# bartelvdh/Navtex

Hardware: AMD Instinct MI355X
Metric: IQ Msamples/s through FIR->FSK->bitsync (higher is better)
Workload: dtype f64

## Files before the change

### navtex_amd/__init__.py

```python
from __future__ import annotations

import ctypes as C
import os
from typing import Callable, Iterable, List, Optional, Sequence, Tuple

import numpy as np

from . import _native as N
from ._native import (CHAIN_490, CHAIN_518, FRAME_BITS, FRAME_IN, FRAME_RAW, FRAME_Y3, RATE_IN, RATE_RAW,
                      SOFT_DECODE, SOFT_KEEP, NvxError, lib)

__all__ = ["Pipeline", "Group", "Capture", "Sitor", "sitor_encode", "make_stream", "synth_host", "synth_device", "device_count",
           "DeviceBuffer", "channelise", "channelise_time_stats", "Store", "wav_write", "wav_read", "NvxError", "lib",
           "CHAIN_518", "CHAIN_490", "SOFT_DECODE", "SOFT_KEEP", "FRAME_BITS", "FRAME_IN", "FRAME_RAW", "FRAME_Y3", "RATE_IN", "RATE_RAW"]


def device_count() -> int:
    return lib.nvx_device_count()


def sitor_encode(text: str, n_phasing: int = 40) -> str:
    t = text.encode("ascii")
    n = lib.nvx_sitor_encode(t, n_phasing, None, 0)
    buf = C.create_string_buffer(n + 1)
# ... 149 lines not shown
        N.check(lib.nvx_cascade_wait_stats(self._h, C.byref(a), C.byref(b), C.byref(c), int(reset)), "nvx_cascade_wait_stats")
        return a.value, b.value, c.value

    def integrity_stats(self, reset: bool = False) -> Tuple[int, int, int]:
        a, b, c = C.c_uint64(), C.c_uint64(), C.c_uint64()
        N.check(lib.nvx_cascade_integrity_stats(self._h, C.byref(a), C.byref(b), C.byref(c), int(reset)), "nvx_cascade_integrity_stats")
        return a.value, b.value, c.value

    def tie_stats(self) -> Tuple[int, int, float]:
        a, b, m = C.c_uint64(), C.c_uint64(), C.c_double()
        N.check(lib.nvx_demod_tie_stats(self._h, C.byref(a), C.byref(b), C.byref(m)), "nvx_demod_tie_stats")
        return a.value, b.value, m.value

    def enable_timing(self, on: bool = True) -> None:
        lib.nvx_enable_timing(self._h, int(on))

    def kernel_ms(self, which: int) -> float:
        return float(lib.nvx_last_kernel_ms(self._h, which))

    def kernel_time_stats(self, which: int, reset: bool = False):
        s, n = C.c_double(), C.c_uint64()
        N.check(lib.nvx_kernel_time_stats(self._h, which, C.byref(s), C.byref(n), int(reset)), "nvx_kernel_time_stats")
        return s.value, n.value

    def enable_signal_report(self, on: bool = True) -> None:
        N.check(lib.nvx_enable_signal_report(self._h, int(on)), "nvx_enable_signal_report")

    def signal_report(self, stream: int = 0, chain: int = 0, reset: bool = False) -> dict:
        r = N.SignalReport()
        N.check(lib.nvx_signal_report_read(self._h, stream, chain, C.byref(r), int(reset)), "nvx_signal_report_read")
        return {f: getattr(r, f) for f, _ in N.SignalReport._fields_}

    def enable_soft(self, mode: int = N.SOFT_DECODE, on_message: Optional[Callable[[int, int, str, str], None]] = None) -> None:
        if not hasattr(self, "soft_messages"):
            self.soft_messages: List[Tuple[int, int, str, str]] = []
        if mode:
            sink = on_message or (lambda s, f, b, t: self.soft_messages.append((s, f, b, t)))
            self._soft_cb = N.MESSAGE_FN(lambda u, s, b, m, f: sink(s, f, b.decode("latin1"), m.decode("latin1")))
            N.check(lib.nvx_set_soft_message_fn(self._h, self._soft_cb, None), "nvx_set_soft_message_fn")
        N.check(lib.nvx_enable_soft(self._h, int(mode)), "nvx_enable_soft")

    def soft_values(self, stream: int = 0, chain: int = 0) -> np.ndarray:
        parts, cap = [], 1 << 14
        while True:
            buf = np.empty(cap, dtype=np.float32)
            n = lib.nvx_poll_soft(self._h, stream, chain, N.as_ptr(buf), cap)
            parts.append(buf[:n])
            if n < cap:
                break
        return np.concatenate(parts)

    def soft_count(self, stream: int = 0, chain: int = 0) -> int:
        return int(lib.nvx_soft_count(self._h, stream, chain))

    def set_carrier(self, stream: int, chain: int, offset_hz: float) -> float:
        applied = C.c_double()
        N.check(lib.nvx_set_carrier(self._h, stream, chain, float(offset_hz), C.byref(applied)), "nvx_set_carrier")
        return applied.value

    def carrier(self, stream: int, chain: int) -> Tuple[float, bool]:
        off, ref = C.c_double(), C.c_int()
        N.check(lib.nvx_get_carrier(self._h, stream, chain, C.byref(off), C.byref(ref)), "nvx_get_carrier")
        return off.value, bool(ref.value)

    def afc_enable(self, stream: int, chain: int, cfg: Optional[N.AfcConfig] = None, **fields) -> None:
        _afc_enable(lib.nvx_afc_enable, self._h, stream, chain, cfg, fields, "nvx_afc_enable")

    def afc_disable(self, stream: int, chain: int, keep: bool = False) -> None:
        N.check(lib.nvx_afc_disable(self._h, stream, chain, int(keep)), "nvx_afc_disable")

    def afc_status(self, stream: int, chain: int) -> dict:
        return _afc_status(lib.nvx_afc_read, self._h, stream, chain, "nvx_afc_read")

    def afc_trace(self, stream: int, chain: int) -> List[int]:
        return _afc_trace(lib.nvx_afc_trace, self._h, stream, chain, "nvx_afc_trace")

    def set_forms(self, independent: int = -1, dynamic_preroll: int = -1, demod_tiles: int = -1) -> None:
        N.check(lib.nvx_debug_set_forms(self._h, independent, dynamic_preroll, demod_tiles), "nvx_debug_set_forms")

    def last_forms(self) -> Tuple[int, int, int]:
        a, b, c = C.c_int(), C.c_int(), C.c_int()
        N.check(lib.nvx_debug_last_forms(self._h, C.byref(a), C.byref(b), C.byref(c)), "nvx_debug_last_forms")
        return a.value, b.value, c.value

    def _apply_forms(self, forms: Optional[Sequence[int]]) -> None:
        if forms is None:
            if not hasattr(lib, "nvx_debug_set_forms"):
                return
            forms = tuple(int(os.environ.get(name, -1)) for name in ("NVX_INDEPENDENT", "NVX_DYNAMIC_PREROLL", "NVX_DEMOD_TILES"))
        if tuple(forms) != (-1, -1, -1):
            self.set_forms(*forms)


class Pipeline(HandleStats):

    def __init__(self, n_streams: int = 1, raw_rate: bool = False, chain_mask: int = CHAIN_518 | CHAIN_490,
                 chain_masks: Optional[Iterable[int]] = None, labels: Optional[Sequence[Sequence[int]]] = None,
                 max_frames: int = 1, char_layer: bool = True, push_mode: bool = False, device: int = 0,
                 wideband: bool = False, bit_history: int = 0, store: "Optional[Store]" = None, stage0_order: int = 1,
                 eager_launch: bool = False, stall_timeout_ms: int = 0, forms: Optional[Sequence[int]] = None):
        self.messages: List[Tuple[int, int, str, str]] = []
        cfg = N.Config()
        lib.nvx_config_default(C.byref(cfg))
        cfg.device, cfg.n_streams, cfg.raw_rate = device, n_streams, int(raw_rate)
        cfg.stage0_order = int(stage0_order)
        cfg.eager_launch = int(eager_launch)
        cfg.stall_timeout_ms = int(stall_timeout_ms)
        cfg.chain_mask, cfg.max_frames, cfg.char_layer, cfg.push_mode = chain_mask, max_frames, int(char_layer), int(push_mode)
        cfg.wideband = int(wideband)
        cfg.bit_history = int(bit_history)
        if chain_masks is not None:
            chain_masks = list(chain_masks)
            self._masks = (C.c_uint8 * len(chain_masks))(*chain_masks)
            cfg.chain_masks = self._masks
        if labels is not None:
            flat = [int(v) for pair in labels for v in pair]
            self._labels = (C.c_int * len(flat))(*flat)
            cfg.labels = self._labels
        self._cb = N.MESSAGE_FN(lambda u, s, b, m, f: self.messages.append((s, f, b.decode("latin1"), m.decode("latin1"))))
        cfg.on_message = self._cb
        if store is not None:
            cfg.on_message = C.cast(lib.nvx_store_on_message, N.MESSAGE_FN)
            cfg.user = store._s
            self._store = store
        self.n_streams, self.raw_rate, self.max_frames, self.device = n_streams, bool(raw_rate), max_frames, device
        self.wideband = bool(wideband)
        self.frame = FRAME_RAW if (raw_rate or wideband) else FRAME_IN
        h = C.c_void_p()
        N.check(lib.nvx_create(C.byref(cfg), C.byref(h)), "nvx_create")
        self._h = h
        self._bits = {}
        self._apply_forms(forms)

    def push(self, stream: int, iq: np.ndarray) -> None:
        iq = np.ascontiguousarray(iq, dtype=np.int16).reshape(-1, 2)
        N.check(lib.nvx_push_iq(self._h, stream, N.as_ptr(iq), iq.shape[0]), "nvx_push_iq")

    def push_planar(self, stream: int, xi: np.ndarray, xq: np.ndarray) -> None:
        xi = np.ascontiguousarray(xi, dtype=np.int16); xq = np.ascontiguousarray(xq, dtype=np.int16)
        N.check(lib.nvx_push_planar(self._h, stream, N.as_ptr(xi), N.as_ptr(xq), xi.size), "nvx_push_planar")

    def flush(self) -> None:
        N.check(lib.nvx_flush(self._h), "nvx_flush")

    def finish(self, stream: Optional[int] = None) -> None:
        if stream is None:
            N.check(lib.nvx_finish(self._h), "nvx_finish")
        else:
            N.check(lib.nvx_stream_finish(self._h, stream), "nvx_stream_finish")

    def poll(self) -> None:
        N.check(lib.nvx_poll(self._h), "nvx_poll")

    def set_active(self, stream: int, active: bool) -> None:
        N.check(lib.nvx_stream_set_active(self._h, stream, int(active)), "nvx_stream_set_active")

    def stream_stats(self, stream: int = 0) -> Tuple[bool, int, int]:
        a, f, p = C.c_int(), C.c_uint64(), C.c_uint64()
        N.check(lib.nvx_stream_stats(self._h, stream, C.byref(a), C.byref(f), C.byref(p)), "nvx_stream_stats")
        return bool(a.value), f.value, p.value

    def set_trace(self, on_text: Optional[Callable[[str], None]]) -> None:
        self._trace_cb = N.SITOR_TRACE_FN(lambda u, t: on_text(t.decode("latin1"))) if on_text else C.cast(None, N.SITOR_TRACE_FN)
        N.check(lib.nvx_set_trace(self._h, self._trace_cb, None), "nvx_set_trace")

    def decode_wav(self, path: str, stream: int = 0) -> int:
# ... 304 lines not shown
```

### navtex_amd/_native.py

```python
from __future__ import annotations

import ctypes as C
import os
from pathlib import Path

import numpy as np

_LIB_PATH = Path(os.environ.get("NAVTEX_AMD_LIB") or (Path(__file__).resolve().parent / "libnavtex_amd.so"))

OK, ERR_ARG, ERR_NODEV, ERR_HIP, ERR_NOMEM, ERR_STATE, ERR_IO = 0, -1, -2, -3, -4, -5, -6
RATE_RAW, RATE_IN = 2016000, 252000
FRAME_BITS, FRAME_IN, FRAME_RAW, FRAME_Y3 = 32, 80640, 645120, 288
CHAIN_518, CHAIN_490 = 1, 2
SOFT_DECODE, SOFT_KEEP = 1, 2
TUNE_N, TUNE_STEP_HZ, TUNE_MAX_HZ, TUNE_NOMINAL_K = 20160, 3.125, 25000.0, 4480

MESSAGE_FN = C.CFUNCTYPE(None, C.c_void_p, C.c_int, C.c_char_p, C.c_char_p, C.c_int)
SITOR_MSG_FN = C.CFUNCTYPE(None, C.c_void_p, C.c_char_p, C.c_char_p, C.c_int)
SITOR_TRACE_FN = C.CFUNCTYPE(None, C.c_void_p, C.c_char_p)


class Config(C.Structure):
    _fields_ = [
        ("struct_size", C.c_uint32), ("device", C.c_int), ("n_streams", C.c_int), ("raw_rate", C.c_int), ("chain_mask", C.c_uint32),
        ("chain_masks", C.POINTER(C.c_uint8)), ("labels", C.POINTER(C.c_int)), ("max_frames", C.c_int),
        ("char_layer", C.c_int), ("on_message", MESSAGE_FN), ("user", C.c_void_p), ("push_mode", C.c_int),
        ("wideband", C.c_int),
        ("bit_history", C.c_int),
        ("host_threads", C.c_int),
        ("stage0_order", C.c_int),
        ("eager_launch", C.c_int),
        ("stall_timeout_ms", C.c_int),
    ]


class Carrier(C.Structure):
    _fields_ = [
        ("freq_hz", C.c_int32), ("shift_hz", C.c_int32), ("amplitude", C.c_int32), ("phase0", C.c_uint32),
        ("bit_offset", C.c_uint32), ("n_bits", C.c_uint32), ("bits", C.c_char_p),
    ]


class SynthStream(C.Structure):
    _fields_ = [("seed", C.c_uint32), ("noise_amp", C.c_int32), ("n_carriers", C.c_int32), ("carrier", Carrier * 16)]


class SignalReport(C.Structure):
    _fields_ = [("samples", C.c_uint64), ("b_samples", C.c_uint64)] + [(f, C.c_double) for f in (
        "sum_power", "sum_dphi_b", "sum_dphi2_b", "sum_dphi_y", "sum_dphi2_y", "sum_mf_hi", "sum_mf_lo",
        "power_db", "b_hz", "y_hz", "offset_hz", "shift_hz", "eye_snr_db", "contrast")]


class AfcConfig(C.Structure):
    _fields_ = [("struct_size", C.c_uint32), ("gain_shift", C.c_int), ("max_step", C.c_int), ("range_k", C.c_int),
                ("min_samples", C.c_int), ("contrast_min", C.c_double)]


class AfcStatus(C.Structure):
    _fields_ = [("enabled", C.c_int), ("centre_k", C.c_int), ("k_last", C.c_int), ("last_step", C.c_int), ("offset_hz", C.c_double),
                ("launches", C.c_uint64), ("updates", C.c_uint64), ("held", C.c_uint64), ("clamped", C.c_uint64)]


AFC_TRACE_KEEP = 1024


def _load() -> C.CDLL:
    if not _LIB_PATH.exists():
        raise ImportError(
            f"{_LIB_PATH} is missing: build it with `python navtex_amd/build.py` "
            "(hipcc, gfx950). navtex_amd has no pure-Python or CPU fallback.")
    lib = C.CDLL(str(_LIB_PATH))
    vp, sz, i, u32 = C.c_void_p, C.c_size_t, C.c_int, C.c_uint32
    sig = {
        "nvx_last_error": (C.c_char_p, []), "nvx_version": (C.c_char_p, []), "nvx_abi_version": (i, []),
        "nvx_sample_to_int16": (i, [C.c_double, C.POINTER(C.c_int16)]), "nvx_shim_stats": (i, [C.POINTER(C.c_uint64), C.POINTER(C.c_uint64)]),
        "nvx_debug_advance_clock": (i, [vp, i, C.c_uint64]),
        "nvx_debug_set_forms": (i, [vp, i, i, i]), "nvx_debug_last_forms": (i, [vp, C.POINTER(i), C.POINTER(i), C.POINTER(i)]),
        "init_fir_filter1": (None, []), "sample_in_1": (None, [C.c_double, C.c_double]), "init_fir2_wrapper": (None, []),
        "nvx_set_trace": (i, [vp, SITOR_TRACE_FN, vp]),
        "nvx_shim_latency": (i, [C.POINTER(C.c_uint64), C.POINTER(C.c_double), C.POINTER(C.c_double), C.POINTER(C.c_double), C.POINTER(C.c_double), i]),
        "nvx_shim_flush": (i, []), "nvx_shim_finish": (i, []), "nvx_shim_bits": (sz, [i, C.c_char_p, sz]),
        "nvx_StreamACallback": (None, [vp, vp, vp, C.c_uint, C.c_uint, vp]),
        "nvx_capture_start": (i, [vp, i, C.c_double, C.POINTER(vp)]), "nvx_capture_callback": (None, [vp, vp, vp, C.c_uint, C.c_uint, vp]),
        "nvx_capture_latency": (i, [vp, C.POINTER(C.c_uint64), C.POINTER(C.c_double), C.POINTER(C.c_double), C.POINTER(C.c_double), C.POINTER(C.c_double), i]),
        "nvx_capture_stop": (i, [vp]), "nvx_capture_record": (i, [vp, C.c_char_p]), "nvx_fsm_selftest": (i, [u32, i]),
        "nvx_cascade_wait_stats": (i, [vp, C.POINTER(C.c_uint64), C.POINTER(C.c_uint64), C.POINTER(C.c_uint64), i]),
        "nvx_debug_cascade_state": (i, [vp, i, vp, sz, i]),
        "nvx_cascade_integrity_stats": (i, [vp, C.POINTER(C.c_uint64), C.POINTER(C.c_uint64), C.POINTER(C.c_uint64), i]), "nvx_capture_pause": (None, [vp, i]),
        "nvx_capture_stats": (None, [vp, C.POINTER(C.c_uint64), C.POINTER(C.c_uint64), C.POINTER(C.c_uint64)]),
        "nvx_config_default": (None, [C.POINTER(Config)]),
        "nvx_create": (i, [C.POINTER(Config), C.POINTER(vp)]), "nvx_destroy": (None, [vp]), "nvx_reset": (i, [vp]), "nvx_stream_reset": (i, [vp, i]),
        "nvx_push_iq": (i, [vp, i, vp, sz]), "nvx_push_planar": (i, [vp, i, vp, vp, sz]), "nvx_flush": (i, [vp]),
        "nvx_finish": (i, [vp]), "nvx_stream_finish": (i, [vp, i]),
        "nvx_poll_bits": (sz, [vp, i, i, C.c_char_p, sz]),
        "nvx_process_resident": (i, [vp, vp, sz, sz, i, vp]), "nvx_fetch_bits": (i, [vp]),
        "nvx_bit_count": (sz, [vp, i, i]),
        "nvx_last_kernel_ms": (C.c_float, [vp, i]), "nvx_enable_timing": (None, [vp, i]), "nvx_enable_debug": (i, [vp, i]),
        "nvx_group_create": (i, [C.POINTER(C.c_int), i, C.POINTER(Config), C.POINTER(vp)]), "nvx_group_destroy": (None, [vp]),
        "nvx_group_reset": (i, [vp]), "nvx_group_size": (i, [vp]),
        "nvx_group_member": (i, [vp, i, C.POINTER(i), C.POINTER(i), C.POINTER(i), C.POINTER(vp)]), "nvx_group_member_of": (i, [vp, i]),
        "nvx_group_process_resident": (i, [vp, C.POINTER(vp), sz, sz, i]), "nvx_group_fetch_bits": (i, [vp]),
        "nvx_group_push_iq": (i, [vp, i, vp, sz]), "nvx_group_flush": (i, [vp]), "nvx_group_finish": (i, [vp]),
        "nvx_group_poll_bits": (sz, [vp, i, i, C.c_char_p, sz]), "nvx_group_bit_count": (sz, [vp, i, i]),
        "nvx_bind_thread_to_device": (i, [i]),
        "nvx_demod_tie_stats": (i, [vp, C.POINTER(C.c_uint64), C.POINTER(C.c_uint64), C.POINTER(C.c_double)]),
        "nvx_capture_error": (i, [vp]),
        "nvx_capture_stalled": (i, [vp, C.POINTER(C.c_uint64)]), "nvx_capture_set_stall_timeout": (None, [vp, C.c_double]),
        "nvx_stream_set_active": (i, [vp, i, i]), "nvx_poll": (i, [vp]),
        "nvx_stream_stats": (i, [vp, i, C.POINTER(i), C.POINTER(C.c_uint64), C.POINTER(C.c_uint64)]),
        "nvx_kernel_time_stats": (i, [vp, i, C.POINTER(C.c_double), C.POINTER(C.c_uint64), i]),
        "nvx_debug_y3": (sz, [vp, i, i, vp, sz]), "nvx_debug_dphi": (sz, [vp, i, i, vp, sz]),
        "nvx_debug_timing": (sz, [vp, i, i, vp, vp, vp, sz]),
        "nvx_enable_signal_report": (i, [vp, i]), "nvx_signal_report_read": (i, [vp, i, i, C.POINTER(SignalReport), i]),
        "nvx_enable_soft": (i, [vp, i]), "nvx_set_soft_message_fn": (i, [vp, MESSAGE_FN, vp]),
        "nvx_poll_soft": (sz, [vp, i, i, vp, sz]), "nvx_soft_count": (C.c_uint64, [vp, i, i]),
        "nvx_sitor_set_soft": (None, [vp, i]), "nvx_sitor_receive_soft": (None, [vp, vp, sz]),
        "nvx_set_carrier": (i, [vp, i, i, C.c_double, C.POINTER(C.c_double)]),
        "nvx_get_carrier": (i, [vp, i, i, C.POINTER(C.c_double), C.POINTER(i)]),
        "nvx_group_set_carrier": (i, [vp, i, i, C.c_double, C.POINTER(C.c_double)]),
        "nvx_group_get_carrier": (i, [vp, i, i, C.POINTER(C.c_double), C.POINTER(i)]),
        "nvx_afc_config_default": (None, [C.POINTER(AfcConfig)]),
        "nvx_afc_enable": (i, [vp, i, i, C.POINTER(AfcConfig)]), "nvx_afc_disable": (i, [vp, i, i, i]),
        "nvx_afc_read": (i, [vp, i, i, C.POINTER(AfcStatus)]), "nvx_afc_trace": (i, [vp, i, i, C.POINTER(C.c_int32), sz]),
        "nvx_group_afc_enable": (i, [vp, i, i, C.POINTER(AfcConfig)]), "nvx_group_afc_disable": (i, [vp, i, i, i]),
        "nvx_group_afc_read": (i, [vp, i, i, C.POINTER(AfcStatus)]), "nvx_group_afc_trace": (i, [vp, i, i, C.POINTER(C.c_int32), sz]),
        "nvx_afc_step_host": (i, [i, i, i, i, C.c_double, i, i, i, C.c_uint, C.c_uint, C.c_double, C.c_double, C.c_double, C.c_double, C.POINTER(C.c_uint)]),
        "nvx_device_count": (i, []), "nvx_device_alloc": (vp, [i, sz]), "nvx_device_free": (None, [i, vp]),
        "nvx_memcpy_h2d": (i, [i, vp, vp, sz]), "nvx_memcpy_d2h": (i, [i, vp, vp, sz]), "nvx_device_sync": (i, [i]),
        "nvx_stream_create": (vp, [i]), "nvx_stream_destroy": (None, [i, vp]),
        "nvx_sitor_new": (vp, [i, SITOR_MSG_FN, vp]), "nvx_sitor_set_trace": (None, [vp, SITOR_TRACE_FN, vp]),
        "nvx_sitor_free": (None, [vp]), "nvx_sitor_reset": (None, [vp]),
        "nvx_sitor_receive_bit": (None, [vp, C.c_char]), "nvx_sitor_receive_bits": (None, [vp, C.c_char_p, sz]),
        "nvx_wav_open": (vp, [C.c_char_p, u32]), "nvx_wav_close": (i, [vp]),
        "nvx_wav_read": (sz, [vp, vp, sz]), "nvx_wav_write": (sz, [vp, vp, sz]),
        "nvx_wav_set_format": (None, [vp, C.c_uint16]), "nvx_wav_set_num_channels": (None, [vp, C.c_uint16]),
        "nvx_wav_set_sample_rate": (None, [vp, u32]), "nvx_wav_set_sample_size": (None, [vp, sz]),
        "nvx_wav_get_format": (C.c_uint16, [vp]), "nvx_wav_get_num_channels": (C.c_uint16, [vp]),
        "nvx_wav_get_sample_rate": (u32, [vp]), "nvx_wav_get_sample_size": (sz, [vp]), "nvx_wav_get_length": (sz, [vp]),
        "nvx_wav_err": (C.c_char_p, []), "nvx_decode_wav": (i, [vp, i, C.c_char_p]),
        "nvx_sitor_encode": (sz, [C.c_char_p, i, C.c_char_p, sz]),
        "nvx_synth_host": (i, [C.POINTER(SynthStream), u32, C.c_uint64, sz, vp]),
        "nvx_synth_device": (i, [i, C.POINTER(SynthStream), i, u32, sz, vp, sz]),
        "nvx_atan2_host": (C.c_double, [C.c_double, C.c_double]),
        "nvx_channelise_resident": (i, [i, vp, sz, sz, i, sz, vp, vp, vp, sz, sz, vp]),
        "nvx_handle_stream": (vp, [vp]), "nvx_channelise_timing": (None, [i]),
        "nvx_channelise_time_stats": (i, [C.POINTER(C.c_double), C.POINTER(C.c_uint64), i]),
        "nvx_store_open": (i, [C.c_char_p, i, C.POINTER(vp)]), "nvx_store_close": (None, [vp]),
        "nvx_store_add_message": (i, [vp, C.c_char_p, C.c_char_p, i]),
        "nvx_store_on_message": (None, [vp, i, C.c_char_p, C.c_char_p, i]),
        "nvx_store_purge": (i, [vp, C.c_long]), "nvx_store_set_time": (None, [vp, C.c_int64]),
        "nvx_store_stats": (None, [vp, C.POINTER(C.c_uint64), C.POINTER(C.c_uint64)]),
    }
    for name, (res, args) in sig.items():
        fn = getattr(lib, name, None)
        if fn is None:
            if os.environ.get("NAVTEX_AMD_LIB"):
                continue
            raise ImportError(f"{_LIB_PATH} does not export {name}: rebuild it (python navtex_amd/build.py)")
        fn.restype, fn.argtypes = res, args
    return lib
# ... 21 lines not shown
```

### navtex_amd/build.py

```python
from __future__ import annotations

import os
import shutil
import subprocess
import sys
from pathlib import Path

PKG = Path(__file__).resolve().parent
ROOT = PKG.parent
CSRC = PKG / "csrc"
OBJ = PKG / "_obj"
LIB = PKG / "libnavtex_amd.so"
ARCH = "gfx950"

C_SOURCES = ["nvx_sitor.c", "nvx_wav.c", "nvx_synth_host.c", "nvx_store.c"]
HIP_SOURCES = ["nvx_cascade.hip", "nvx_fir3.hip", "nvx_demod.hip", "nvx_channelise.hip", "nvx_wideband_fused.hip", "nvx_synth.hip"]
SCAN = PKG / "scan"
SCAN_LIB = PKG / "libnavtex_amd_scan.so"
SCAN_C_SOURCES = ["nvx_scan_find.c"]
SCAN_HIP_SOURCES = ["nvx_scan.hip"]
SCAN_CXX_SOURCES = ["nvx_scan_host.cpp"]
RESAMPLE = PKG / "resample"
RESAMPLE_LIB = PKG / "libnavtex_amd_resample.so"
RESAMPLE_C_SOURCES = ["nvx_resample_design.c"]
RESAMPLE_HIP_SOURCES = ["nvx_resample.hip"]
RESAMPLE_CXX_SOURCES = ["nvx_resample_host.cpp"]
DDC = PKG / "ddc"
DDC_LIB = PKG / "libnavtex_amd_ddc.so"
DDC_HIP_SOURCES = ["nvx_ddc.hip"]
DDC_CXX_SOURCES = ["nvx_ddc_host.cpp"]
DDC_SHARED_C_SOURCES = ["nvx_resample_design.c"]
BLANK = PKG / "blank"
BLANK_LIB = PKG / "libnavtex_amd_blank.so"
BLANK_HIP_SOURCES = ["nvx_blank.hip"]
BLANK_CXX_SOURCES = ["nvx_blank_host.cpp"]
IQC = PKG / "iqc"
IQC_LIB = PKG / "libnavtex_amd_iqc.so"
IQC_HIP_SOURCES = ["nvx_iqc.hip"]
IQC_CXX_SOURCES = ["nvx_iqc_host.cpp"]
REAL = PKG / "real"
REAL_LIB = PKG / "libnavtex_amd_real.so"
REAL_HIP_SOURCES = ["nvx_real.hip"]
REAL_CXX_SOURCES = ["nvx_real_host.cpp"]
NARROW = PKG / "narrow"
NARROW_LIB = PKG / "libnavtex_amd_narrow.so"
NARROW_C_SOURCES = ["nvx_narrow_design.c"]
NARROW_HIP_SOURCES = ["nvx_narrow.hip"]
NARROW_CXX_SOURCES = ["nvx_narrow_host.cpp"]
TAP = PKG / "tap"
TAP_LIB = PKG / "libnavtex_amd_tap.so"
TAP_C_SOURCES = ["nvx_tap_design.c"]
TAP_HIP_SOURCES = ["nvx_tap.hip"]
TAP_CXX_SOURCES = ["nvx_tap_host.cpp"]
ANC = PKG / "anc"
ANC_LIB = PKG / "libnavtex_amd_anc.so"
ANC_HIP_SOURCES = ["nvx_anc.hip"]
ANC_CXX_SOURCES = ["nvx_anc_host.cpp"]
CXX_SOURCES = ["nvx_api.cpp", "nvx_push.cpp", "nvx_shim.cpp", "nvx_capture.cpp", "nvx_wideband.cpp", "nvx_synth_dev.cpp", "nvx_fsm_host.cpp", "nvx_group.cpp",
               "nvx_tune.cpp", "nvx_afc.cpp"]
AFC = PKG / "afc"
AFC_HIP_SOURCES = ["nvx_afc.hip"]

COMMON = ["-O3", "-fPIC", "-ffp-contract=off", "-fvisibility=hidden",
          f"-I{ROOT / 'include'}", f"-I{CSRC}"] + os.environ.get("NVX_EXTRA_CFLAGS", "").split()


def _hipcc() -> str:
    for cand in (os.environ.get("HIPCC"), shutil.which("hipcc"), "/opt/rocm/bin/hipcc"):
        if cand and Path(cand).exists():
            return cand
    raise RuntimeError("hipcc not found: the HIP toolchain is required (there is no CPU build of this library)")


def _run(cmd):
    print(" ".join(str(c) for c in cmd), file=sys.stderr, flush=True)
    subprocess.run([str(c) for c in cmd], check=True, stdout=sys.stderr)


def _stale(out: Path, deps) -> bool:
    if not out.exists():
        return True
    t = out.stat().st_mtime
    return any(Path(d).stat().st_mtime > t for d in deps)


def _companion_jobs(hipcc: str, force: bool, src_dir: Path, c_sources, hip_sources, cxx_sources, also=()):
    headers = list(src_dir.glob("*.h")) + list(CSRC.glob("*.h")) + list((ROOT / "include").glob("*.h")) + [Path(__file__)]
    flags = [*COMMON, f"-I{src_dir}"]
    for d in also:
        headers += list(d.glob("*.h"))
        flags.append(f"-I{d}")
    objs, jobs = [], []
    for srcs, cmd in ((c_sources, [hipcc, "-x", "c", "-std=gnu11", "-Wall", "-Wextra"]),
                      (hip_sources, [hipcc, f"--offload-arch={ARCH}", "-std=c++17"]),
                      (cxx_sources, [hipcc, "-x", "hip", "--offload-arch=" + ARCH, "-std=c++17", "-Wall"])):
        for src in srcs:
            o = OBJ / (src + ".o")
            if force or _stale(o, [src_dir / src] + headers):
                jobs.append([*cmd, *flags, "-c", src_dir / src, "-o", o])
            objs.append(o)
    return objs, jobs


def _scan_jobs(hipcc: str, force: bool):
    return _companion_jobs(hipcc, force, SCAN, SCAN_C_SOURCES, SCAN_HIP_SOURCES, SCAN_CXX_SOURCES)


def _resample_jobs(hipcc: str, force: bool):
    return _companion_jobs(hipcc, force, RESAMPLE, RESAMPLE_C_SOURCES, RESAMPLE_HIP_SOURCES, RESAMPLE_CXX_SOURCES)


def _ddc_jobs(hipcc: str, force: bool):
    objs, jobs = _companion_jobs(hipcc, force, DDC, [], DDC_HIP_SOURCES, DDC_CXX_SOURCES, also=(RESAMPLE,))
    return objs + [OBJ / (src + ".o") for src in DDC_SHARED_C_SOURCES], jobs


def _blank_jobs(hipcc: str, force: bool):
    return _companion_jobs(hipcc, force, BLANK, [], BLANK_HIP_SOURCES, BLANK_CXX_SOURCES, also=(RESAMPLE,))


def _iqc_jobs(hipcc: str, force: bool):
    return _companion_jobs(hipcc, force, IQC, [], IQC_HIP_SOURCES, IQC_CXX_SOURCES, also=(RESAMPLE,))


def _real_jobs(hipcc: str, force: bool):
    return _companion_jobs(hipcc, force, REAL, [], REAL_HIP_SOURCES, REAL_CXX_SOURCES, also=(RESAMPLE,))


def _narrow_jobs(hipcc: str, force: bool):
    return _companion_jobs(hipcc, force, NARROW, NARROW_C_SOURCES, NARROW_HIP_SOURCES, NARROW_CXX_SOURCES, also=(RESAMPLE,))


def _tap_jobs(hipcc: str, force: bool):
    return _companion_jobs(hipcc, force, TAP, TAP_C_SOURCES, TAP_HIP_SOURCES, TAP_CXX_SOURCES, also=(RESAMPLE, DDC))


def _anc_jobs(hipcc: str, force: bool):
    return _companion_jobs(hipcc, force, ANC, [], ANC_HIP_SOURCES, ANC_CXX_SOURCES, also=(RESAMPLE,))


def _link(hipcc: str, lib: Path, objs, libs=()) -> None:
    tmp = lib.with_name(lib.name + f".tmp{os.getpid()}")
    _run([hipcc, "-shared", "-fPIC", f"--offload-arch={ARCH}", *objs, "-o", tmp, *libs])
    os.replace(tmp, lib)


def build_lib(force: bool = False) -> Path:
    from concurrent.futures import ThreadPoolExecutor
    hipcc = _hipcc()
    OBJ.mkdir(exist_ok=True)
    headers = list(CSRC.glob("*.h")) + list((ROOT / "include").glob("*.h")) + [Path(__file__)]
    objs, jobs = [], []
    scan_objs, scan_jobs = _scan_jobs(hipcc, force)
    jobs += scan_jobs
    resample_objs, resample_jobs = _resample_jobs(hipcc, force)
    jobs += resample_jobs
    ddc_objs, ddc_jobs = _ddc_jobs(hipcc, force)
    jobs += ddc_jobs
    blank_objs, blank_jobs = _blank_jobs(hipcc, force)
    jobs += blank_jobs
    iqc_objs, iqc_jobs = _iqc_jobs(hipcc, force)
    jobs += iqc_jobs
    real_objs, real_jobs = _real_jobs(hipcc, force)
    jobs += real_jobs
    narrow_objs, narrow_jobs = _narrow_jobs(hipcc, force)
    jobs += narrow_jobs
    tap_objs, tap_jobs = _tap_jobs(hipcc, force)
    jobs += tap_jobs
    anc_objs, anc_jobs = _anc_jobs(hipcc, force)
    jobs += anc_jobs
    for src in C_SOURCES:
        o = OBJ / (src + ".o")
        if force or _stale(o, [CSRC / src] + headers):
            jobs.append([hipcc, "-x", "c", "-std=gnu11", "-Wall", "-Wextra", *COMMON, "-c", CSRC / src, "-o", o])
        objs.append(o)
    for src in HIP_SOURCES:
        o = OBJ / (src + ".o")
        if force or _stale(o, [CSRC / src] + headers):
            jobs.append([hipcc, f"--offload-arch={ARCH}", "-std=c++17", *COMMON, "-c", CSRC / src, "-o", o])
        objs.append(o)
    for src in AFC_HIP_SOURCES:
        o = OBJ / (src + ".o")
        if force or _stale(o, [AFC / src] + headers):
            jobs.append([hipcc, f"--offload-arch={ARCH}", "-std=c++17", *COMMON, "-c", AFC / src, "-o", o])
        objs.append(o)
    for src in CXX_SOURCES:
        o = OBJ / (src + ".o")
        if force or _stale(o, [CSRC / src] + headers):
            jobs.append([hipcc, "-x", "hip", "--offload-arch=" + ARCH, "-std=c++17", "-Wall", "-Wno-unused-value", "-Wno-unused-result", *COMMON, "-c", CSRC / src, "-o", o])
        objs.append(o)
    with ThreadPoolExecutor(max_workers=min(8, os.cpu_count() or 1)) as pool:
        list(pool.map(_run, jobs))
    if force or _stale(LIB, objs):
        _link(hipcc, LIB, objs, ["-lpthread", "-ldl"])
    if force or _stale(SCAN_LIB, scan_objs):
        _link(hipcc, SCAN_LIB, scan_objs, ["-lpthread", "-lm"])
    if force or _stale(RESAMPLE_LIB, resample_objs):
        _link(hipcc, RESAMPLE_LIB, resample_objs, ["-lpthread", "-lm"])
    if force or _stale(DDC_LIB, ddc_objs):
        _link(hipcc, DDC_LIB, ddc_objs, ["-lpthread", "-lm"])
    if force or _stale(BLANK_LIB, blank_objs):
        _link(hipcc, BLANK_LIB, blank_objs, ["-lpthread"])
    if force or _stale(IQC_LIB, iqc_objs):
        _link(hipcc, IQC_LIB, iqc_objs, ["-lpthread"])
    if force or _stale(REAL_LIB, real_objs):
        _link(hipcc, REAL_LIB, real_objs, ["-lpthread"])
    if force or _stale(NARROW_LIB, narrow_objs):
        _link(hipcc, NARROW_LIB, narrow_objs, ["-lpthread", "-lm"])
    if force or _stale(TAP_LIB, tap_objs):
        _link(hipcc, TAP_LIB, tap_objs, ["-lpthread", "-lm"])
    if force or _stale(ANC_LIB, anc_objs):
        _link(hipcc, ANC_LIB, anc_objs, ["-lpthread"])
    return LIB


def build_variant(name: str, flags, sources=("nvx_cascade.hip", "nvx_wideband_fused.hip")) -> Path:
    hipcc = _hipcc()
    build_lib()
    out_dir = ROOT / "tests" / "_variants"
    out_dir.mkdir(exist_ok=True)
    headers = list(CSRC.glob("*.h")) + list((ROOT / "include").glob("*.h")) + [Path(__file__)]
    objs, jobs = [], []
    for src in C_SOURCES + HIP_SOURCES + CXX_SOURCES:
        if src in sources:
            o = out_dir / f"{src}.{name}.o"
            if _stale(o, [CSRC / src] + headers):
                lang = ["-x", "c", "-std=gnu11"] if src in C_SOURCES else (["-x", "hip"] if src in CXX_SOURCES else []) + [f"--offload-arch={ARCH}", "-std=c++17"]
                jobs.append([hipcc, *lang, *COMMON, *flags, "-c", CSRC / src, "-o", o])
            objs.append(o)
        else:
            objs.append(OBJ / (src + ".o"))
    objs += [OBJ / (src + ".o") for src in AFC_HIP_SOURCES]
    from concurrent.futures import ThreadPoolExecutor
    with ThreadPoolExecutor(max_workers=2) as pool:
        list(pool.map(_run, jobs))
    lib = out_dir / f"libnavtex_amd_{name}.so"
    if _stale(lib, objs):
        tmp = lib.with_name(lib.name + f".tmp{os.getpid()}")
        _run([hipcc, "-shared", "-fPIC", f"--offload-arch={ARCH}", *objs, "-o", tmp, "-lpthread", "-ldl"])
        os.replace(tmp, lib)
    return lib


INJECT_FLAGS = ["-DNVX_INJECT_STALE=5"]


def build_oracle() -> None:
    _run(["make", "-s", "-C", ROOT / "oracle", "oracle"])
    if os.path.isdir("/root/reference/receiver"):
        _run(["make", "-s", "-C", ROOT / "oracle", "ref"])


if __name__ == "__main__":
    build_lib(force="--force" in sys.argv)
    if "--oracle" in sys.argv:
        build_oracle()
    if "--inject" in sys.argv or (ROOT / "tests" / "_variants" / "libnavtex_amd_inject.so").exists():
        build_variant("inject", INJECT_FLAGS)
    if "--variant" in sys.argv:
        rest = sys.argv[sys.argv.index("--variant") + 1:]
        srcs = ("nvx_cascade.hip", "nvx_wideband_fused.hip")
        if "--sources" in rest:
            k = rest.index("--sources"); srcs = tuple(rest[k + 1].split(",")); rest = rest[:k] + rest[k + 2:]
        print(build_variant(rest[0], rest[1:], srcs))
```

### navtex_amd/csrc/nvx_api.cpp

```cpp
#include "nvx_handle.h"
#include <chrono>
#include <cmath>
#include "navtex_amd_afc.h"
#include "navtex_amd_signal.h"
#include "navtex_amd_soft.h"
#include "navtex_amd_tune.h"
#include "nvx_fsm.h"

extern "C" hipError_t nvx_launch_afc_update(const nvx_afc_args *a, hipStream_t s) __attribute__((weak));
static_assert(NVX_AFC_LAW_C == NVX_AFC_C && NVX_AFC_K_MAX * NVX_TUNE_STEP_HZ == NVX_TUNE_MAX_HZ, "the law's constants are the header's");
static_assert(sizeof(nvx_afc_note) == 8 && sizeof(nvx_afc_par) == 32, "layouts of nvx_afc_law.h");

static thread_local char g_err[512] = "";
extern "C" void nvx_set_error(const char *fmt, ...)
{
    va_list ap; va_start(ap, fmt);
    vsnprintf(g_err, sizeof g_err, fmt, ap);
    va_end(ap);
}
extern "C" const char *nvx_last_error(void) { return g_err; }
int64_t nvx_now_ns()
{
    return std::chrono::duration_cast<std::chrono::nanoseconds>(std::chrono::steady_clock::now().time_since_epoch()).count();
}
#define NVX_STR2(x) #x
#define NVX_STR(x) NVX_STR2(x)
extern "C" const char *nvx_version(void) { return "navtex_amd " NVX_STR(NVX_ABI_VERSION) ".0 (gfx950)"; }
extern "C" int nvx_abi_version(void) { return NVX_ABI_VERSION; }

int nvx_select_device(int device)
{
    int n = 0;
    hipError_t e = hipGetDeviceCount(&n);
    if (e != hipSuccess || n == 0) {
        nvx_set_error("no HIP device available (%s); libnavtex_amd has no CPU path",
                      e == hipSuccess ? "device count 0" : hipGetErrorString(e));
        return NVX_ERR_NODEV;
    }
    if (device < 0 || device >= n) { nvx_set_error("device %d out of range (0..%d)", device, n - 1); return NVX_ERR_ARG; }
    HIP_TRY(hipSetDevice(device));
    return NVX_OK;
}


int nvx_check_device_span(const void *p, size_t bytes, const char *what)
{
    hipDeviceptr_t base = nullptr; size_t size = 0;
    if (hipMemGetAddressRange(&base, &size, (hipDeviceptr_t)p) != hipSuccess) { (void)hipGetLastError(); return NVX_OK; }
    const size_t off = (size_t)((const char *)p - (const char *)base);
    if (off > size || bytes > size - off) {
        nvx_set_error("%s: %zu bytes from %p leave the allocation they lie in (%zu bytes from %p): the launch would fault", what, bytes, p, size, (void *)base);
        return NVX_ERR_ARG;
    }
    return NVX_OK;
}

static void sitor_sink(void *user, const char *bbbb, const char *message, int freq);

static void deliver_outbox(nvx_handle *h, int stream, Slot &s);

static void sitor_sink_impl(nvx_handle *h, int slot, const char *bbbb, const char *message, int freq);

static void sitor_sink(void *user, const char *bbbb, const char *message, int freq)
{
    SinkCtx *c = (SinkCtx *)user;
    if (c->soft) c->h->slots[c->slot].soft_outbox.push_back(Message{ bbbb, message, freq });
    else sitor_sink_impl(c->h, c->slot, bbbb, message, freq);
}

extern "C" void nvx_config_default(nvx_config *c)
{
    memset(c, 0, sizeof *c);
    c->struct_size = (uint32_t)sizeof *c;
    c->device = 0; c->n_streams = 1; c->raw_rate = 0;
    c->chain_mask = NVX_CHAIN_518 | NVX_CHAIN_490;
    c->max_frames = 1; c->char_layer = 1; c->push_mode = 0;
}

static int drain(nvx_handle *h)
{
    if (h->launch_done_valid) HIP_TRY(hipEventSynchronize(h->launch_done));
    if (h->stream) HIP_TRY(hipStreamSynchronize(h->stream));
    if (h->stream2) HIP_TRY(hipStreamSynchronize(h->stream2));
    return NVX_OK;
}

// ... 326 lines not shown
    return NVX_OK;
}

int nvx_launch_locked(nvx_handle *h, const void *d_iq, size_t pitch, size_t first_sample, int n_frames, hipStream_t st,
                      const int *part, int n_part, const int *tail_n3)
{
    if (h->poisoned) return nvx_poisoned_error(h);
    if (n_frames < 1 || n_frames > h->cfg.max_frames) { nvx_set_error("n_frames %d outside 1..max_frames %d", n_frames, h->cfg.max_frames); return NVX_ERR_ARG; }
    if ((pitch & 3) || (first_sample & 3)) { nvx_set_error("pitch and first sample must be multiples of 4 samples"); return NVX_ERR_ARG; }
    if (part && (n_part < 1 || n_part > h->n_in)) { nvx_set_error("launch with %d of %d streams", n_part, h->n_in); return NVX_ERR_ARG; }
    if (part && n_part == h->n_in && !tail_n3) part = nullptr;
    for (int i = 0; part && i < n_part; i++)
        if (part[i] < 0 || part[i] >= h->n_in || (i > 0 && part[i] <= part[i - 1])) { nvx_set_error("launch list: stream %d out of order or range", part[i]); return NVX_ERR_ARG; }
    const int n_named = part ? n_part : h->n_in;
    for (int i = 0; i < n_named; i++) {
        const int s = part ? part[i] : i;
        if (h->ended[s]) { nvx_set_error("stream %d has ended (nvx_finish): nvx_stream_reset or nvx_reset starts a new one", s); return NVX_ERR_STATE; }
        if (tail_n3 && (tail_n3[i] < 1 || tail_n3[i] >= n_frames * NVX_FRAME_Y3)) { nvx_set_error("launch list: %d samples at 900 S/s in the tail of stream %d", tail_n3[i], s); return NVX_ERR_ARG; }
    }
    Result &r = h->res[h->launched % RESULT_SLOTS];
    if (r.pending) { int rc = nvx_collect_locked(h, h->launched - RESULT_SLOTS + 1); if (rc != NVX_OK) return rc; }
    { int rc = nvx_collect_ready_locked(h); if (rc != NVX_OK) return rc; }

    if (h->launch_done_valid && st != h->last_launch_stream) HIP_TRY(hipStreamWaitEvent(st, h->launch_done, 0));

    const bool fused = h->cfg.wideband != 0;
    const int yb = (int)(h->launched & 1);
    hipStream_t sd = h->stream2;
    const int n3_full = n_frames * NVX_FRAME_Y3;
    const bool with_list = h->diverged || part != nullptr || tail_n3 != nullptr;
    r.n_part = 0;
    const nvx_part *d_list = nullptr;
    if (with_list) {
        r.n_part = n_named;
        for (int i = 0; i < r.n_part; i++) {
            const int s = part ? part[i] : i;
            r.h_part[i] = nvx_part{ s, (int)h->parity[s], h->g0s[s], tail_n3 ? tail_n3[i] : n3_full, 0 };
        }
        HIP_TRY(hipMemcpyAsync(r.d_part, r.h_part, (size_t)r.n_part * sizeof(nvx_part), hipMemcpyHostToDevice, st));
        d_list = r.d_part;
    }
    const int n_here = with_list ? r.n_part : h->n_in;
    const int p0 = d_list ? 0 : (int)h->parity[0];
    const unsigned third0 = (unsigned)(h->g0s[0] / (NVX_FRAME_Y3 / 3));
    double2 *const y2_bufs[2] = { h->d_y2[d_list ? 0 : p0], h->d_y2[d_list ? 1 : p0 ^ 1] };
    nvx_demod_args da{};
    da.y3 = h->d_y3[yb]; da.y3_cap = (size_t)h->y3_cap; da.y3_base = 0; da.n3 = n3_full;
    da.n_slots = h->n_slots; da.slot_active = h->d_active;
    da.g0 = h->g0s[0]; da.part = d_list; da.n_part = r.n_part; da.per_part = h->per_in;
    da.dstate[0] = h->d_dd[p0]; da.dstate[1] = h->d_dd[p0 ^ 1];
    da.state_i = h->d_di; da.fsm_table = h->d_fsm_tab; da.words = h->d_words;
    da.bits = r.d_bits; da.bits_cap = h->bits_cap; da.nbits = r.d_nbits; da.dphi = h->d_dphi; da.ties = h->d_ties;
    da.corr = h->d_corr; da.csum = h->d_csum;
    const bool afc = h->afc_tracking > 0;
    da.sig = (h->sig_on || afc) ? r.d_sig : nullptr; da.sig_part = h->d_sig_part; da.sig_stride = h->sig_stride;
    da.soft = h->soft_mode ? r.d_soft : nullptr; da.soft_cap = std::min(h->soft_cap, n3_full / 8 + 8); da.soft_pos = h->d_soft_pos;
    nvx_forms forms = h->forms_req;
    forms.demod_tiles = nvx_front_tile_wgs(&da, forms.demod_tiles);
    da.sig_parts = 1 + forms.demod_tiles;

    if (h->demod_pending[yb]) HIP_TRY(hipStreamWaitEvent(st, h->demod_done[yb], 0));
    r.timed = h->timing;
    if (r.timed) HIP_TRY(hipEventRecord(r.ev[0], st));
    if (fused) {
        nvx_wideband_args wa{};
        wa.raw = (const uint32_t *)d_iq; wa.pitch = pitch; wa.first_sample = first_sample;
        wa.n_wide = n_here; wa.n_frames = n_frames; wa.chain_masks = h->d_masks;
        wa.part = d_list;
        wa.state[0] = h->d_cstate[p0]; wa.state[1] = h->d_cstate[p0 ^ 1];
        wa.hist[0] = h->d_whist[p0]; wa.hist[1] = h->d_whist[p0 ^ 1];
        wa.y3 = h->d_y3[yb]; wa.y3_cap = (size_t)h->y3_cap; wa.y3_base = 0;
        wa.queue = h->d_ctrl; wa.status = h->d_ctrl + 1; wa.done = h->d_ctrl + NVX_CASCADE_CTRL_INTS; wa.third0 = third0;
        wa.y2[0] = y2_bufs[0]; wa.y2[1] = y2_bufs[1]; wa.y2_pitch = h->y2_pitch; wa.y2_row = h->d_y2row;
        HIP_TRY(nvx_launch_wideband_fused(&wa, &forms, st));
    } else {
        nvx_cascade_args ca{};
        ca.iq = (const uint32_t *)d_iq; ca.pitch = pitch; ca.first_sample = first_sample;
        ca.n_frames = n_frames; ca.n_streams = n_here; ca.chain_masks = h->d_masks;
        ca.part = d_list;
        ca.state[0] = h->d_cstate[p0]; ca.state[1] = h->d_cstate[p0 ^ 1]; ca.y3 = h->d_y3[yb]; ca.y3_cap = (size_t)h->y3_cap; ca.y3_base = 0;
        ca.queue = h->d_ctrl; ca.status = h->d_ctrl + 1; ca.done = h->d_ctrl + NVX_CASCADE_CTRL_INTS;
        ca.stage0_order = h->cfg.stage0_order;
        ca.third0 = third0;
        ca.tune_k = afc ? h->d_afc_k[h->launched & 1] : h->d_tune_k;
        ca.max_waves_per_cu = -1;
        HIP_TRY(nvx_launch_cascade(&ca, h->cascade_raw, h->nch, &forms, st));
    }
    if (r.timed) HIP_TRY(hipEventRecord(r.ev[1], st));
    HIP_TRY(hipMemcpyAsync(h->h_status + NVX_STATUS_INTS * (h->launched % RESULT_SLOTS), h->d_ctrl + 1, NVX_STATUS_INTS * sizeof(int), hipMemcpyDeviceToHost, st));
    HIP_TRY(hipEventRecord(h->casc_done[yb], st));
    HIP_TRY(hipStreamWaitEvent(sd, h->casc_done[yb], 0));
    if (fused) {
        nvx_fir3_args fa{};
        fa.y2[0] = y2_bufs[0]; fa.y2[1] = y2_bufs[1]; fa.y2_pitch = h->y2_pitch; fa.y2_row = h->d_y2row;
        fa.y3 = h->d_y3[yb]; fa.y3_cap = (size_t)h->y3_cap; fa.y3_base = 0; fa.n_frames = n_frames; fa.n_slots = h->n_slots;
        fa.part = d_list; fa.n_part = r.n_part; fa.per_part = h->per_in;
        if (r.timed) HIP_TRY(hipEventRecord(r.ev[6], sd));
        HIP_TRY(nvx_launch_fir3(&fa, sd));
        if (r.timed) HIP_TRY(hipEventRecord(r.ev[7], sd));
    }
    if (r.timed) HIP_TRY(hipEventRecord(r.ev[2], sd));
    HIP_TRY(nvx_launch_demod_front(&da, sd));
    if (r.timed) HIP_TRY(hipEventRecord(r.ev[3], sd));
    if (!da.soft && !afc) HIP_TRY(hipEventRecord(h->demod_done[yb], sd));
    h->demod_pending[yb] = true;
    if (r.timed) HIP_TRY(hipEventRecord(r.ev[4], sd));
    HIP_TRY(nvx_launch_demod_fsm(&da, sd));
    if (r.timed) HIP_TRY(hipEventRecord(r.ev[5], sd));
    if (afc) {
        nvx_afc_args aa{};
        aa.sig = r.d_sig; aa.par = h->d_afc_par; aa.k_rw = h->d_afc_k[h->launched & 1]; aa.k_next = h->d_afc_k[(h->launched + 1) & 1];
        aa.note = r.d_note; aa.n_slots = h->n_slots; aa.part = d_list; aa.n_part = r.n_part;
        if (r.timed) HIP_TRY(hipEventRecord(r.ev[8], sd));
        HIP_TRY(nvx_launch_afc_update(&aa, sd));
        if (r.timed) HIP_TRY(hipEventRecord(r.ev[9], sd));
    }
    if (da.soft || afc) HIP_TRY(hipEventRecord(h->demod_done[yb], sd));
    HIP_TRY(hipMemcpyAsync(h->h_ties, h->d_ties, sizeof(nvx_tie_stats), hipMemcpyDeviceToHost, sd));
    HIP_TRY(hipMemcpyAsync(r.h_nbits, r.d_nbits, (size_t)h->n_slots * sizeof(int), hipMemcpyDeviceToHost, sd));
    HIP_TRY(hipMemcpyAsync(r.h_bits, r.d_bits, (size_t)h->n_slots * h->bits_cap, hipMemcpyDeviceToHost, sd));
    if (h->sig_on) HIP_TRY(hipMemcpyAsync(r.h_sig, r.d_sig, (size_t)h->n_slots * sizeof(nvx_sig_rec), hipMemcpyDeviceToHost, sd));
    r.sig = h->sig_on;
    if (afc) HIP_TRY(hipMemcpyAsync(r.h_note, r.d_note, (size_t)h->n_slots * sizeof(nvx_afc_note), hipMemcpyDeviceToHost, sd));
    r.afc = afc;
    if (da.soft) HIP_TRY(hipMemcpyAsync(r.h_soft, r.d_soft, (size_t)h->n_slots * da.soft_cap * sizeof(float), hipMemcpyDeviceToHost, sd));
    r.soft_pitch = da.soft_cap;
    r.soft = da.soft != nullptr;
    HIP_TRY(hipEventRecord(r.done, sd));
    HIP_TRY(hipEventRecord(h->launch_done, sd));
    h->launch_done_valid = true; h->last_launch_stream = st;
    r.pending = true;
    r.n3 = n3_full;
    r.g0_all = h->g0s[0];
    h->launched++;
    h->last_n3 = n3_full;
    h->forms_last = forms; h->forms_known = true;
    for (int i = 0; i < n_here; i++) {
        const int s = with_list ? r.h_part[i].stream : i;
        h->parity[s] ^= 1; h->g0s[s] += (unsigned long long)(tail_n3 ? tail_n3[i] : n3_full);
        if (tail_n3) h->ended[s] = 1;
    }
    if (part) h->partial_launches++;
    h->diverged = with_list && !streams_together(h);
    return NVX_OK;
}

int nvx_collect_ready_locked(nvx_handle *h)
{
    while (h->collected < h->launched) {
        Result &o = h->res[h->collected % RESULT_SLOTS];
        if (o.pending) {
            const hipError_t q = hipEventQuery(o.done);
            if (q == hipErrorNotReady) { (void)hipGetLastError(); break; }
            if (q != hipSuccess) { nvx_set_error("hipEventQuery: %s", hipGetErrorString(q)); return NVX_ERR_HIP; }
        }
        int rc = nvx_collect_locked(h, h->collected + 1);
        if (rc != NVX_OK) return rc;
    }
    return NVX_OK;
}

int nvx_poisoned_error(nvx_handle *h)
{
    nvx_set_error("a launch of this handle failed (%s): nvx_reset it", h->poison_why.c_str());
    return NVX_ERR_STATE;
}

// ... 287 lines not shown
extern "C" int nvx_enable_signal_report(nvx_handle *h, int on)
{
    if (!h) { nvx_set_error("nvx_enable_signal_report: null handle"); return NVX_ERR_ARG; }
    std::lock_guard<std::mutex> lk(h->mu);
    HIP_TRY(hipSetDevice(h->cfg.device));
    { int rc = drain(h); if (rc != NVX_OK) return rc; }
    if (!on) { free_signal(h); return NVX_OK; }
    if (h->sig_on) return NVX_OK;
    { int rc = make_signal_buffers(h, "nvx_enable_signal_report"); if (rc != NVX_OK) return rc; }
    h->sig_on = true;
    return NVX_OK;
}

extern "C" int nvx_enable_soft(nvx_handle *h, int mode)
{
    if (!h) { nvx_set_error("nvx_enable_soft: null handle"); return NVX_ERR_ARG; }
    if (mode != 0 && mode != NVX_SOFT_DECODE && mode != (NVX_SOFT_DECODE | NVX_SOFT_KEEP)) { nvx_set_error("nvx_enable_soft: mode %d (0, NVX_SOFT_DECODE, NVX_SOFT_DECODE | NVX_SOFT_KEEP)", mode); return NVX_ERR_ARG; }
    std::lock_guard<std::mutex> lk(h->mu);
    if (h->poisoned) return nvx_poisoned_error(h);
    HIP_TRY(hipSetDevice(h->cfg.device));
    { int rc = drain(h); if (rc != NVX_OK) return rc; }
    if (!mode) { free_soft(h); return NVX_OK; }
    if (!h->soft_mode) {
        const int cap = h->bits_cap * 8;
        const size_t row_bytes = (size_t)h->n_slots * cap * sizeof(float);
        hipError_t e = hipMalloc(&h->d_soft_pos, (size_t)(h->y3_cap / 9) * h->n_slots * sizeof(unsigned short));
        for (auto &r : h->res) {
            if (e == hipSuccess) e = hipMalloc(&r.d_soft, row_bytes);
            if (e == hipSuccess) e = hipHostMalloc((void **)&r.h_soft, row_bytes, hipHostMallocDefault);
        }
        if (e != hipSuccess) {
            free_soft(h);
            nvx_set_error("nvx_enable_soft: allocation failed: %s", hipGetErrorString(e));
            return e == hipErrorOutOfMemory ? NVX_ERR_NOMEM : NVX_ERR_HIP;
        }
        h->soft_cap = cap;
        if (h->cfg.char_layer)
            for (int i = 0; i < h->n_slots; i++) {
                Slot &s = h->slots[i];
                if (!s.active) continue;
                SinkCtx *ctx = new SinkCtx{ h, i / 2, i, true };
                h->sinks.push_back(ctx);
                s.soft_sitor = nvx_sitor_new(s.label, sitor_sink, ctx);
                nvx_sitor_set_soft(s.soft_sitor, 1);
            }
    }
    if (!(mode & NVX_SOFT_KEEP))
        for (auto &s : h->slots) { s.soft_base += s.soft.size(); std::vector<float>().swap(s.soft); }
    else if (!(h->soft_mode & NVX_SOFT_KEEP))
        for (auto &s : h->slots) { s.soft_base = (size_t)s.soft_count; s.soft_polled = s.soft_base; }
    h->soft_mode = mode;
    return NVX_OK;
}

extern "C" int nvx_set_soft_message_fn(nvx_handle *h, nvx_message_fn fn, void *user)
{
    if (!h) { nvx_set_error("nvx_set_soft_message_fn: null handle"); return NVX_ERR_ARG; }
    std::lock_guard<std::mutex> lk(h->mu);
    if (h->poisoned) return nvx_poisoned_error(h);
    h->soft_fn = fn; h->soft_user = user;
    return NVX_OK;
}

extern "C" size_t nvx_poll_soft(nvx_handle *h, int stream, int chain, float *out, size_t cap)
{
    if (!h || !out || stream < 0 || stream >= h->n_streams || chain < 0 || chain > 1) return 0;
    std::lock_guard<std::mutex> lk(h->mu);
    if (!(h->soft_mode & NVX_SOFT_KEEP)) return 0;
    Slot &s = h->slots[2 * stream + chain];
    if (s.soft_polled < s.soft_base) s.soft_polled = s.soft_base;
    const size_t n = std::min(cap, s.soft_base + s.soft.size() - s.soft_polled);
    if (n) memcpy(out, s.soft.data() + (s.soft_polled - s.soft_base), n * sizeof(float));
    s.soft_polled += n;
    return n;
}

extern "C" uint64_t nvx_soft_count(nvx_handle *h, int stream, int chain)
{
    if (!h || stream < 0 || stream >= h->n_streams || chain < 0 || chain > 1) return 0;
    std::lock_guard<std::mutex> lk(h->mu);
    return h->slots[2 * stream + chain].soft_count;
}

static int afc_write_centre(nvx_handle *h, int slot, int k)
{
    for (int i = 0; i < 2; i++) HIP_TRY(hipMemcpy(h->d_afc_k[i] + slot, &k, sizeof(int), hipMemcpyHostToDevice));
    h->slots[slot].afc.par.kc = k;
    HIP_TRY(hipMemcpy(h->d_afc_par + slot, &h->slots[slot].afc.par, sizeof(nvx_afc_par), hipMemcpyHostToDevice));
    return NVX_OK;
}

extern "C" int nvx_set_carrier(nvx_handle *h, int stream, int chain, double offset_hz, double *applied_hz)
{
    if (!h) { nvx_set_error("nvx_set_carrier: null handle"); return NVX_ERR_ARG; }
    if (h->cfg.wideband) { nvx_set_error("nvx_set_carrier: not for wideband handles (the channeliser fixes their sub-bands)"); return NVX_ERR_STATE; }
    if (stream < 0 || stream >= h->n_streams || chain < 0 || chain > 1) { nvx_set_error("nvx_set_carrier: bad stream or chain"); return NVX_ERR_ARG; }
    if (!((h->masks[stream] >> chain) & 1)) { nvx_set_error("nvx_set_carrier: chain %d is not in stream %d's mask", chain, stream); return NVX_ERR_ARG; }
    if (!std::isfinite(offset_hz) || std::fabs(offset_hz) > NVX_TUNE_MAX_HZ) { nvx_set_error("nvx_set_carrier: offset %g Hz outside +-%g Hz", offset_hz, NVX_TUNE_MAX_HZ); return NVX_ERR_ARG; }
    const int k = (int)std::rint(offset_hz / NVX_TUNE_STEP_HZ);
    std::lock_guard<std::mutex> lk(h->mu);
    HIP_TRY(hipSetDevice(h->cfg.device));
    const int slot = 2 * stream + chain;
    if (h->slots[slot].afc.on) { int rc = nvx_collect_locked(h); if (rc != NVX_OK) return rc; }
    { int rc = drain(h); if (rc != NVX_OK) return rc; }
    HIP_TRY(hipMemcpyAsync(h->d_tune_k + slot, &k, sizeof(int), hipMemcpyHostToDevice, h->stream));
    if (h->afc_tracking) { int rc = afc_write_centre(h, slot, k); if (rc != NVX_OK) return rc; }
    HIP_TRY(hipStreamSynchronize(h->stream));
    h->tune_k[slot] = k;
    afc_restart(h, slot);
    if (applied_hz) *applied_hz = k * NVX_TUNE_STEP_HZ;
    return NVX_OK;
}

extern "C" int nvx_get_carrier(nvx_handle *h, int stream, int chain, double *offset_hz, int *reference_mixer)
{
    if (!h) { nvx_set_error("nvx_get_carrier: null handle"); return NVX_ERR_ARG; }
    if (h->cfg.wideband) { nvx_set_error("nvx_get_carrier: not for wideband handles"); return NVX_ERR_STATE; }
    if (stream < 0 || stream >= h->n_streams || chain < 0 || chain > 1) { nvx_set_error("nvx_get_carrier: bad stream or chain"); return NVX_ERR_ARG; }
    std::lock_guard<std::mutex> lk(h->mu);
    const int k = h->tune_k[2 * stream + chain];
    if (offset_hz) *offset_hz = k * NVX_TUNE_STEP_HZ;
    if (reference_mixer) *reference_mixer = k == (chain ? -NVX_TUNE_NOMINAL_K : NVX_TUNE_NOMINAL_K);
    return NVX_OK;
}

extern "C" void nvx_afc_config_default(nvx_afc_config *c)
{
    if (!c) return;
    memset(c, 0, sizeof *c);
    c->struct_size = (uint32_t)sizeof *c;
    c->gain_shift = 1; c->max_step = 8; c->range_k = 48; c->min_samples = 256; c->contrast_min = 0.7;
}

static int afc_args(nvx_handle *h, int stream, int chain, const char *what, int *slot)
{
    if (!h) { nvx_set_error("%s: null handle", what); return NVX_ERR_ARG; }
    if (h->cfg.wideband) { nvx_set_error("%s: not for wideband handles (the channeliser fixes their sub-bands)", what); return NVX_ERR_STATE; }
    if (stream < 0 || stream >= h->n_streams || chain < 0 || chain > 1) { nvx_set_error("%s: bad stream or chain", what); return NVX_ERR_ARG; }
    if (!((h->masks[stream] >> chain) & 1)) { nvx_set_error("%s: chain %d is not in stream %d's mask", what, chain, stream); return NVX_ERR_ARG; }
    *slot = 2 * stream + chain;
    return NVX_OK;
}

static int make_afc(nvx_handle *h)
{
    if (h->d_afc_par) return NVX_OK;
    const size_t n = (size_t)h->n_slots;
    hipError_t e = hipMalloc(&h->d_afc_par, n * sizeof(nvx_afc_par));
    if (e != hipSuccess) h->d_afc_par = nullptr;
    for (int i = 0; i < 2; i++) if (e == hipSuccess) e = hipMalloc(&h->d_afc_k[i], n * sizeof(int));
    for (auto &r : h->res) {
        if (e == hipSuccess) e = hipMalloc(&r.d_note, n * sizeof(nvx_afc_note));
        if (e == hipSuccess) e = hipHostMalloc((void **)&r.h_note, n * sizeof(nvx_afc_note), hipHostMallocDefault);
    }
    if (e == hipSuccess) {
        std::vector<nvx_afc_par> par(n);
        for (size_t i = 0; i < n; i++) { par[i] = h->slots[i].afc.par; par[i].track = 0; par[i].kc = h->tune_k[i]; }
        e = hipMemcpy(h->d_afc_par, par.data(), n * sizeof(nvx_afc_par), hipMemcpyHostToDevice);
    }
    if (e != hipSuccess) {
        free_afc(h);
        nvx_set_error("nvx_afc_enable: allocation failed: %s", hipGetErrorString(e));
        return e == hipErrorOutOfMemory ? NVX_ERR_NOMEM : NVX_ERR_HIP;
    }
    return NVX_OK;
}

extern "C" int nvx_afc_enable(nvx_handle *h, int stream, int chain, const nvx_afc_config *cfg)
{
    int slot = 0;
    { int rc = afc_args(h, stream, chain, "nvx_afc_enable", &slot); if (rc != NVX_OK) return rc; }
    nvx_afc_config c;
    nvx_afc_config_default(&c);
    if (cfg) {
        if (cfg->struct_size != sizeof(nvx_afc_config)) { nvx_set_error("nvx_afc_enable: nvx_afc_config.struct_size is %u, this library's has %zu bytes", cfg->struct_size, sizeof(nvx_afc_config)); return NVX_ERR_ARG; }
        c = *cfg;
    }
    if (c.gain_shift < 0 || c.gain_shift > 4 || c.max_step < 1 || c.max_step > 64 || c.range_k < 1 || c.range_k > 320 || c.min_samples < 0 ||
        !(c.contrast_min >= 0.0 && c.contrast_min <= 1.0)) {
        nvx_set_error("nvx_afc_enable: a field out of range (gain_shift 0..4, max_step 1..64, range_k 1..320, min_samples >= 0, contrast_min 0..1)");
        return NVX_ERR_ARG;
    }
    if (!nvx_launch_afc_update) { nvx_set_error("nvx_afc_enable: this build holds no update kernel"); return NVX_ERR_STATE; }
    std::lock_guard<std::mutex> lk(h->mu);
    if (h->poisoned) return nvx_poisoned_error(h);
    HIP_TRY(hipSetDevice(h->cfg.device));
    { int rc = nvx_collect_locked(h); if (rc != NVX_OK) return rc; }
    { int rc = drain(h); if (rc != NVX_OK) return rc; }
    { int rc = make_signal_buffers(h, "nvx_afc_enable"); if (rc != NVX_OK) return rc; }
    { int rc = make_afc(h); if (rc != NVX_OK) { if (!h->sig_on && !h->afc_tracking) free_signal_buffers(h); return rc; } }
    AfcHost &a = h->slots[slot].afc;
    if (!h->afc_tracking)
        for (int i = 0; i < 2; i++) HIP_TRY(hipMemcpy(h->d_afc_k[i], h->tune_k.data(), (size_t)h->n_slots * sizeof(int), hipMemcpyHostToDevice));
    a.par.track = 1;
    a.par.gain_shift = c.gain_shift; a.par.max_step = c.max_step; a.par.range_k = c.range_k; a.par.min_samples = c.min_samples;
    a.par.contrast_min = c.contrast_min;
    { int rc = afc_write_centre(h, slot, h->tune_k[slot]); if (rc != NVX_OK) { a.par.track = a.on ? 1 : 0; return rc; } }
    if (a.ring.empty()) a.ring.assign(NVX_AFC_TRACE_KEEP, 0);
    if (!a.on) { a.on = true; h->afc_tracking++; }
    afc_restart(h, slot);
    return NVX_OK;
}

extern "C" int nvx_afc_disable(nvx_handle *h, int stream, int chain, int keep)
{
    int slot = 0;
    { int rc = afc_args(h, stream, chain, "nvx_afc_disable", &slot); if (rc != NVX_OK) return rc; }
    std::lock_guard<std::mutex> lk(h->mu);
    if (h->poisoned) return nvx_poisoned_error(h);
    AfcHost &a = h->slots[slot].afc;
    if (!a.on) return NVX_OK;
    HIP_TRY(hipSetDevice(h->cfg.device));
    { int rc = nvx_collect_locked(h); if (rc != NVX_OK) return rc; }
    { int rc = drain(h); if (rc != NVX_OK) return rc; }
    int k = h->tune_k[slot];
    if (keep) {
        HIP_TRY(hipMemcpy(&k, h->d_afc_k[h->launched & 1] + slot, sizeof(int), hipMemcpyDeviceToHost));
        HIP_TRY(hipMemcpy(h->d_tune_k + slot, &k, sizeof(int), hipMemcpyHostToDevice));
        h->tune_k[slot] = k;
    }
    a.par.track = 0;
    { int rc = afc_write_centre(h, slot, k); if (rc != NVX_OK) return rc; }
    a.on = false; h->afc_tracking--;
    afc_restart(h, slot);
    if (!h->afc_tracking && !h->sig_on) free_signal_buffers(h);
    return NVX_OK;
}

static int afc_take_in(nvx_handle *h)
{
    if (h->poisoned) return nvx_poisoned_error(h);
    if (h->collected != h->launched) {
        HIP_TRY(hipSetDevice(h->cfg.device));
        return nvx_collect_ready_locked(h);
    }
    return NVX_OK;
}

extern "C" int nvx_afc_read(nvx_handle *h, int stream, int chain, nvx_afc_status *out)
{
    int slot = 0;
    { int rc = afc_args(h, stream, chain, "nvx_afc_read", &slot); if (rc != NVX_OK) return rc; }
    if (!out) { nvx_set_error("nvx_afc_read: null argument"); return NVX_ERR_ARG; }
    std::lock_guard<std::mutex> lk(h->mu);
    { int rc = afc_take_in(h); if (rc != NVX_OK) return rc; }
    const AfcHost &a = h->slots[slot].afc;
    memset(out, 0, sizeof *out);
    out->enabled = a.on; out->centre_k = h->tune_k[slot];
    out->k_last = a.on ? a.k_last : h->tune_k[slot]; out->last_step = a.on ? a.last_step : 0;
    out->offset_hz = out->k_last * NVX_TUNE_STEP_HZ;
    out->launches = a.launches; out->updates = a.updates; out->held = a.held; out->clamped = a.clamped;
    return NVX_OK;
}

extern "C" int nvx_afc_trace(nvx_handle *h, int stream, int chain, int32_t *k, size_t cap)
{
    int slot = 0;
    { int rc = afc_args(h, stream, chain, "nvx_afc_trace", &slot); if (rc != NVX_OK) return rc; }
    if (!k && cap) { nvx_set_error("nvx_afc_trace: null argument"); return NVX_ERR_ARG; }
    std::lock_guard<std::mutex> lk(h->mu);
    { int rc = afc_take_in(h); if (rc != NVX_OK) return rc; }
    AfcHost &a = h->slots[slot].afc;
    if (!a.on) return 0;
    if (a.ring_w - a.ring_r > NVX_AFC_TRACE_KEEP) a.ring_r = a.ring_w - NVX_AFC_TRACE_KEEP;
    int n = 0;
    while (a.ring_r < a.ring_w && (size_t)n < cap) k[n++] = a.ring[a.ring_r++ % NVX_AFC_TRACE_KEEP];
    return n;
}

static void signal_derive(nvx_signal_report *o)
{
    const double nan = std::nan(""), hz = 900.0 / (2.0 * M_PI);
    const uint64_t ny = o->samples - o->b_samples;
    o->power_db = o->samples ? 10.0 * std::log10(o->sum_power / (double)o->samples) : nan;
    const double mb = o->b_samples ? o->sum_dphi_b / (double)o->b_samples : nan;
    const double my = ny ? o->sum_dphi_y / (double)ny : nan;
    o->b_hz = mb * hz; o->y_hz = my * hz;
    o->offset_hz = (o->b_hz + o->y_hz) / 2.0;
    o->shift_hz = o->b_hz - o->y_hz;
    const double vb = std::max(0.0, o->sum_dphi2_b / (double)o->b_samples - mb * mb);
    const double vy = std::max(0.0, o->sum_dphi2_y / (double)ny - my * my);
    const double half = (mb - my) / 2.0, noise = (vb + vy) / 2.0;
    o->eye_snr_db = (o->b_samples && ny && noise > 0.0) ? 10.0 * std::log10(half * half / noise) : nan;
    const double mf = o->sum_mf_hi + o->sum_mf_lo;
    o->contrast = mf != 0.0 ? (o->sum_mf_hi - o->sum_mf_lo) / mf : nan;
}

extern "C" int nvx_signal_report_read(nvx_handle *h, int stream, int chain, nvx_signal_report *out, int reset)
{
    if (!h || !out) { nvx_set_error("nvx_signal_report_read: null argument"); return NVX_ERR_ARG; }
    if (stream < 0 || stream >= h->n_streams || chain < 0 || chain > 1) { nvx_set_error("nvx_signal_report_read: bad stream or chain"); return NVX_ERR_ARG; }
    std::lock_guard<std::mutex> lk(h->mu);
    if (h->poisoned) return nvx_poisoned_error(h);
    if (!h->sig_on) { nvx_set_error("nvx_signal_report_read: signal reports are off (nvx_enable_signal_report)"); return NVX_ERR_STATE; }
    if (h->collected != h->launched) {
        HIP_TRY(hipSetDevice(h->cfg.device));
        int rc = nvx_collect_ready_locked(h);
        if (rc != NVX_OK) return rc;
    }
    SigSums &g = h->slots[2 * stream + chain].sig;
    memset(out, 0, sizeof *out);
    out->samples = g.samples; out->b_samples = g.b_samples;
    out->sum_power = g.power; out->sum_dphi_b = g.dphi_b; out->sum_dphi2_b = g.dphi2_b;
    out->sum_dphi_y = g.dphi_y; out->sum_dphi2_y = g.dphi2_y; out->sum_mf_hi = g.hi; out->sum_mf_lo = g.lo;
    signal_derive(out);
    if (reset) g = SigSums{};
    return NVX_OK;
}

static_assert(NVX_STATE_BLOCK_BYTES == NVX_CASCADE_STATE_BYTES, "public size of a state block");
extern "C" int nvx_debug_cascade_state(nvx_handle *h, int stream, void *buf, size_t bytes, int write)
{
    if (!h || !buf || stream < 0 || stream >= h->n_streams || bytes != (size_t)NVX_CASCADE_STATE_BYTES) { nvx_set_error("nvx_debug_cascade_state: bad argument (a block is %d bytes)", NVX_CASCADE_STATE_BYTES); return NVX_ERR_ARG; }
    std::lock_guard<std::mutex> lk(h->mu);
    HIP_TRY(hipSetDevice(h->cfg.device));
    { int rc = drain(h); if (rc != NVX_OK) return rc; }
    const int in = stream / h->per_in;
    uint8_t *blk = h->d_cstate[h->parity[in]] + (size_t)stream * NVX_CASCADE_STATE_BYTES;
    if (write) HIP_TRY(hipMemcpy(blk, buf, bytes, hipMemcpyHostToDevice));
    else HIP_TRY(hipMemcpy(buf, blk, bytes, hipMemcpyDeviceToHost));
    return NVX_OK;
}

static unsigned long long seal_tag_host(int stream, unsigned third)
{
    unsigned long long t = ((unsigned long long)(unsigned)stream << 32) | third;
    t *= 0x9E3779B97F4A7C15ull; t ^= t >> 29; t *= 0xBF58476D1CE4E5B9ull; t ^= t >> 32;
    return t;
}

static_assert(NVX_CLOCK_PERIOD % NVX_FRAME_Y3 == 0 && NVX_CLOCK_PERIOD % (9 * 567) == 0, "the clock's period");
extern "C" int nvx_debug_advance_clock(nvx_handle *h, int stream, uint64_t periods)
{
    if (!h || stream < 0 || stream >= h->n_in) { nvx_set_error("nvx_debug_advance_clock: bad stream"); return NVX_ERR_ARG; }
    if (h->cfg.wideband) { nvx_set_error("nvx_debug_advance_clock: not for wideband handles"); return NVX_ERR_STATE; }
    std::unique_lock<std::mutex> lk(h->mu);
    if (h->poisoned) return nvx_poisoned_error(h);
    if (h->ended[stream]) { nvx_set_error("nvx_debug_advance_clock: stream %d has ended", stream); return NVX_ERR_STATE; }
    HIP_TRY(hipSetDevice(h->cfg.device));
    { int rc = nvx_collect_locked(h); if (rc != NVX_OK) return rc; }
    { int rc = drain(h); if (rc != NVX_OK) return rc; }
    const unsigned long long g_old = h->g0s[stream];
    if (g_old < 3 * NVX_FRAME_Y3) { nvx_set_error("nvx_debug_advance_clock: stream %d is still priming (%llu samples at 900 S/s; the timing filter is primed at 582)", stream, g_old); return NVX_ERR_STATE; }
    if (periods > (~0ull - g_old) / (unsigned long long)NVX_CLOCK_PERIOD) { nvx_set_error("nvx_debug_advance_clock: the clock would pass 2^64"); return NVX_ERR_ARG; }
    const unsigned long long g_new = g_old + periods * (unsigned long long)NVX_CLOCK_PERIOD;
    const unsigned third_old = (unsigned)(g_old / (NVX_FRAME_Y3 / 3)), third_new = (unsigned)(g_new / (NVX_FRAME_Y3 / 3));
    unsigned long long seal[2];
    uint8_t *entry = h->d_cstate[h->parity[stream]] + (size_t)stream * NVX_CASCADE_STATE_BYTES + (size_t)NVX_STATE_SEAL * 16;
    HIP_TRY(hipMemcpy(seal, entry, sizeof seal, hipMemcpyDeviceToHost));
    seal[0] ^= seal_tag_host(stream, third_old) ^ seal_tag_host(stream, third_new);
    seal[1] = ((unsigned long long)(unsigned)stream << 32) | third_new;
    HIP_TRY(hipMemcpy(entry, seal, sizeof seal, hipMemcpyHostToDevice));
    h->g0s[stream] = g_new;
    h->diverged = !streams_together(h);
    return NVX_OK;
}

extern "C" int nvx_debug_set_forms(nvx_handle *h, int independent, int dynamic_preroll, int demod_tiles)
{
    const auto bad = [](int v) { return v < -1 || v > 1; };
    if (!h || bad(independent) || bad(dynamic_preroll) || bad(demod_tiles)) { nvx_set_error("nvx_debug_set_forms: null handle, or a value outside -1 (automatic), 0, 1"); return NVX_ERR_ARG; }
    std::lock_guard<std::mutex> lk(h->mu);
    h->forms_req = nvx_forms{ independent, dynamic_preroll, demod_tiles };
    return NVX_OK;
}

extern "C" int nvx_debug_last_forms(nvx_handle *h, int *independent, int *dynamic_preroll, int *front_tile_wgs)
{
    if (!h) { nvx_set_error("nvx_debug_last_forms: null handle"); return NVX_ERR_ARG; }
    std::lock_guard<std::mutex> lk(h->mu);
    if (!h->forms_known) { nvx_set_error("nvx_debug_last_forms: the handle has launched nothing yet"); return NVX_ERR_STATE; }
    if (independent) *independent = h->forms_last.independent;
    if (dynamic_preroll) *dynamic_preroll = h->forms_last.dynamic_preroll;
    if (front_tile_wgs) *front_tile_wgs = h->forms_last.demod_tiles;
    return NVX_OK;
}

extern "C" size_t nvx_debug_y3(nvx_handle *h, int stream, int chain, double *out, size_t cap_pairs)
{
    if (!h || !out || stream < 0 || stream >= h->n_streams || chain < 0 || chain > 1) return 0;
    std::lock_guard<std::mutex> lk(h->mu);
    hipSetDevice(h->cfg.device);
    hipDeviceSynchronize();
    size_t n = std::min(cap_pairs, (size_t)h->last_n3);
    const int in = stream / h->per_in;
    if (h->ended[in]) n = std::min(n, (size_t)(h->g0s[in] % NVX_FRAME_Y3));
    if (hipMemcpy(out, h->d_y3[(h->launched + 1) & 1] + (size_t)(2 * stream + chain) * h->y3_cap, n * sizeof(double2), hipMemcpyDeviceToHost) != hipSuccess) return 0;
    return n;
}

extern "C" size_t nvx_debug_dphi(nvx_handle *h, int stream, int chain, double *out, size_t cap)
{
    if (!h || !out || !h->d_dphi || stream < 0 || stream >= h->n_streams || chain < 0 || chain > 1) return 0;
    std::lock_guard<std::mutex> lk(h->mu);
    hipSetDevice(h->cfg.device);
    hipDeviceSynchronize();
    size_t n = std::min(cap, (size_t)h->last_n3);
    if (hipMemcpy(out, h->d_dphi + (size_t)(2 * stream + chain) * h->y3_cap, n * sizeof(double), hipMemcpyDeviceToHost) != hipSuccess) return 0;
    return n;
}

extern "C" size_t nvx_debug_timing(nvx_handle *h, int stream, int chain, double *corr, double *csum, uint16_t *words, size_t cap)
{
    if (!h || stream < 0 || stream >= h->n_streams || chain < 0 || chain > 1) return 0;
    std::lock_guard<std::mutex> lk(h->mu);
    if ((corr || csum) && !h->d_corr) return 0;
    hipSetDevice(h->cfg.device);
    hipDeviceSynchronize();
    size_t n = std::min(cap, (size_t)h->last_n3);
    const int in = stream / h->per_in;
    if (h->ended[in]) n = std::min(n, (size_t)(h->g0s[in] % NVX_FRAME_Y3));
    const size_t slot = (size_t)(2 * stream + chain);
    if (corr && hipMemcpy(corr, h->d_corr + slot * h->y3_cap, n * sizeof(double), hipMemcpyDeviceToHost) != hipSuccess) return 0;
    if (csum && hipMemcpy(csum, h->d_csum + slot * h->y3_cap, n * sizeof(double), hipMemcpyDeviceToHost) != hipSuccess) return 0;
    if (words && hipMemcpy(words, h->d_words + slot * (h->y3_cap / 9), (n + 8) / 9 * sizeof(uint16_t), hipMemcpyDeviceToHost) != hipSuccess) return 0;
    return n;
}

extern "C" int nvx_device_count(void) { int n = 0; return hipGetDeviceCount(&n) == hipSuccess ? n : 0; }
extern "C" void *nvx_device_alloc(int device, size_t bytes)
{
    if (nvx_select_device(device) != NVX_OK) return nullptr;
    void *p = nullptr;
    hipError_t e = hipMalloc(&p, bytes);
    if (e != hipSuccess) { nvx_set_error("hipMalloc(%zu) failed: %s", bytes, hipGetErrorString(e)); return nullptr; }
    return p;
}
extern "C" void nvx_device_free(int device, void *p) { if (p && nvx_select_device(device) == NVX_OK) hipFree(p); }
extern "C" int nvx_memcpy_h2d(int device, void *d, const void *s, size_t n)
{
    int rc = nvx_select_device(device); if (rc != NVX_OK) return rc;
    HIP_TRY(hipMemcpy(d, s, n, hipMemcpyHostToDevice)); return NVX_OK;
}
extern "C" int nvx_memcpy_d2h(int device, void *d, const void *s, size_t n)
{
    int rc = nvx_select_device(device); if (rc != NVX_OK) return rc;
    HIP_TRY(hipMemcpy(d, s, n, hipMemcpyDeviceToHost)); return NVX_OK;
}
extern "C" int nvx_device_sync(int device)
{
    int rc = nvx_select_device(device); if (rc != NVX_OK) return rc;
    HIP_TRY(hipDeviceSynchronize()); return NVX_OK;
}
extern "C" void *nvx_stream_create(int device)
{
    if (nvx_select_device(device) != NVX_OK) return nullptr;
    hipStream_t s = nullptr;
    hipError_t e = hipStreamCreateWithFlags(&s, hipStreamNonBlocking);
    if (e != hipSuccess) { nvx_set_error("hipStreamCreate failed: %s", hipGetErrorString(e)); return nullptr; }
    return (void *)s;
}
extern "C" void nvx_stream_destroy(int device, void *hip_stream)
{
    if (hip_stream && nvx_select_device(device) == NVX_OK) { hipStreamSynchronize((hipStream_t)hip_stream); hipStreamDestroy((hipStream_t)hip_stream); }
}
```

### navtex_amd/csrc/nvx_cascade.hip

```cpp
#include <hip/hip_runtime.h>
#include <stdint.h>
#include <stdlib.h>
#include <mutex>

#include "nvx_cascade_wave.h"
#include "nvx_tune_table.h"

__device__ double2 nvx_tune_tab[NVX_TUNE_TAB_ENTRIES];

__device__ __forceinline__ int add_low_halves(unsigned a, unsigned b)
{
    int r;
    asm("v_add_u32_sdwa %0, sext(%1), sext(%2) dst_sel:DWORD dst_unused:UNUSED_PAD src0_sel:WORD_0 src1_sel:WORD_0"
        : "=v"(r) : "v"(a), "v"(b));
    return r;
}
__device__ __forceinline__ int add_high_halves(unsigned a, unsigned b)
{
    int r;
    asm("v_add_u32_sdwa %0, sext(%1), sext(%2) dst_sel:DWORD dst_unused:UNUSED_PAD src0_sel:WORD_1 src1_sel:WORD_1"
        : "=v"(r) : "v"(a), "v"(b));
    return r;
}
__device__ __forceinline__ double stage0_component(u32x4 v, bool odd)
{
    const int sI = add_low_halves(v.x, v.y) + add_low_halves(v.z, v.w);
    const int sQ = add_high_halves(v.x, v.y) + add_high_halves(v.z, v.w);
    int mine = (odd ? sQ : sI) + 4;
    const int other = odd ? sI : sQ;
    asm("" : "+v"(mine));
    const int tot = mine + dpp_swap_pairs(other);
    return (double)(tot >> 3);
}

struct Stage0Cic3 {
    unsigned sel_mine, sel_other;
    unsigned wa0, wa1, wb0, wb1, wc0, wc1;
    int c_prev, t_prev;
    bool last_pair;

    __device__ __forceinline__ void init(int lane)
    {
        const bool odd = lane & 1;
        sel_mine = odd ? 0x07060302u : 0x05040100u;
        sel_other = odd ? 0x05040100u : 0x07060302u;
        wa0 = odd ? (10u | 6u << 16) : (36u | 28u << 16);  wa1 = odd ? (3u | 1u << 16) : (21u | 15u << 16);
        wb0 = odd ? (48u | 48u << 16) : (28u | 36u << 16); wb1 = odd ? (46u | 42u << 16) : (42u | 46u << 16);
        wc0 = odd ? (6u | 10u << 16) : 0u;                 wc1 = odd ? (15u | 21u << 16) : (1u | 3u << 16);
        last_pair = lane >= 62;
        c_prev = 0; t_prev = 0;
    }
    __device__ __forceinline__ static int rot1(int v) { return __builtin_amdgcn_mov_dpp(v, 0x13C, 0xF, 0xF, false); }
    __device__ __forceinline__ static void dot2_first(nvx_short2 a, unsigned wb, unsigned wc, int &b, int &c)
    {
        asm("v_dot2_i32_i16 %0, %2, %3, 0\n\t"
            "v_dot2_i32_i16 %1, %2, %4, 0\n\t"
            "s_nop 2"
            : "=&v"(b), "=v"(c) : "v"(a), "v"(wb), "v"(wc));
    }
    __device__ __forceinline__ double step(u32x4 v)
    {
        const nvx_short2 m01 = as_short2(__builtin_amdgcn_perm(v.y, v.x, sel_mine)), m23 = as_short2(__builtin_amdgcn_perm(v.w, v.z, sel_mine));
        const nvx_short2 o01 = as_short2(__builtin_amdgcn_perm(v.y, v.x, sel_other)), o23 = as_short2(__builtin_amdgcn_perm(v.w, v.z, sel_other));
        int oa = __builtin_amdgcn_sdot2(o01, as_short2(wa0), 256, false); oa = __builtin_amdgcn_sdot2(o23, as_short2(wa1), oa, false);
        int ob, oc;
        dot2_first(o01, wb0, wc0, ob, oc);
        ob = __builtin_amdgcn_sdot2(o23, as_short2(wb1), ob, false); oc = __builtin_amdgcn_sdot2(o23, as_short2(wc1), oc, false);
        int A = dpp_swap_pairs(oa); A = __builtin_amdgcn_sdot2(m01, as_short2(wa0), A, false); A = __builtin_amdgcn_sdot2(m23, as_short2(wa1), A, false);
        int B = dpp_swap_pairs(ob); B = __builtin_amdgcn_sdot2(m01, as_short2(wb0), B, false); B = __builtin_amdgcn_sdot2(m23, as_short2(wb1), B, false);
        int C = dpp_swap_pairs(oc); C = __builtin_amdgcn_sdot2(m01, as_short2(wc0), C, false); C = __builtin_amdgcn_sdot2(m23, as_short2(wc1), C, false);
        const int t = B + rot1(rot1(last_pair ? c_prev : C));
        const int y = A + rot1(rot1(last_pair ? t_prev : t));
        c_prev = C; t_prev = t;
        return (double)(y >> 9);
    }
};

template <bool RAW>
__device__ __forceinline__ void load_pass(u32x4 (&pf)[RAW ? 8 : 1], const u32x4 *src)
{
    if (RAW) {
#pragma unroll
        for (int j = 0; j < 8; j++) pf[j] = __builtin_nontemporal_load(src + 64 * j);
    } else {
        pf[0] = __builtin_nontemporal_load(src);
    }
}

#define NVX_SPIN_LIMIT (1 << 22)

template <bool RAW, int NCH, int S0, typename ARGS, bool LIST = false>
__device__ __forceinline__ void cascade_wave_main(ARGS a)
{
    __shared__ CascadeLds<NCH> lds;
    const int lane = threadIdx.x;
    CascadeWave<NCH> cw;
    cw.init(&lds, lane);

    const size_t pass_words = RAW ? 2048 : 256;
    const size_t pass_stride = pass_words / 4;
    constexpr int NPF = RAW ? 8 : 1;
    const int half = lane >> 1, comp = lane & 1;
    const bool odd = lane & 1;
    double *xw = (double *)&lds.X[(half & 7) * XS + XH + (lane >> 4)] + comp;
    double2 *xw4 = &lds.X[(lane & 1) * 4 * XS + XH + half];
    static_assert(S0 == 1 || (S0 == 3 && RAW), "the third-order stage 0 belongs to the raw-rate kernels");
    Stage0Cic3 s0;
    if (S0 == 3) s0.init(lane);
    const int n_full = a.n_streams * a.split_from;
    const int n_units = n_full + 3 * a.n_streams * (a.n_frames - a.split_from);

    for (;;) {
        int u = 0;
        if (lane == 0) u = __hip_atomic_fetch_add(a.queue, 1, __ATOMIC_RELAXED, __HIP_MEMORY_SCOPE_AGENT);
        u = __builtin_amdgcn_readfirstlane(u);
        if (u >= n_units) break;
        int tpart, thirds, entry;
        if (u < n_full) { const int frame = u / a.n_streams; entry = u - frame * a.n_streams; tpart = 3 * frame; thirds = 3; }
        else { const int v = u - n_full, q = v / a.n_streams; entry = v - q * a.n_streams; tpart = 3 * a.split_from + q; thirds = 1; }
        const int part = tpart;
        int stream = entry;
        const uint8_t *state_rd = a.state[0];
        uint8_t *state_wr = a.state[1];
        unsigned third0 = a.third0;
        if (LIST) {
            const unsigned long long e = nvx_load_const_u64(a.part + entry);
            stream = (int)(unsigned)e;
            if (e >> 32) { state_rd = a.state[1]; state_wr = a.state[0]; }
            third0 = (unsigned)(nvx_load_const_u64(&a.part[entry].g0) / NVX_THIRD_Y3);
        }
        int *const done = a.done + entry;
        const unsigned mask = a.chain_masks[stream];

        bool preroll = a.independent && part > 0;
        bool late_publish = false;
        const u32x4 *unit0 = (const u32x4 *)(a.iq + ((size_t)stream * a.pitch + a.first_sample)) + (size_t)part * NVX_THIRD_PASSES * pass_stride + lane;
        u32x4 pfA[NPF];
        if (!preroll) load_pass<RAW>(pfA, unit0);

        if (part > 0 && !a.independent) {
            int spins = 0, ok = 0;
            do {
                int d = 0;
                if (lane == 0) d = __hip_atomic_load(done, __ATOMIC_RELAXED, __HIP_MEMORY_SCOPE_AGENT);
                d = __builtin_amdgcn_readfirstlane(d);
                ok = d >= part;
                if (!ok && a.dynamic_preroll) break;
                if (!ok) __builtin_amdgcn_s_sleep(32);
            } while (!ok && ++spins < NVX_SPIN_LIMIT);
            if (!ok && a.dynamic_preroll) {
                preroll = true; late_publish = true;
                if (lane == 0) __hip_atomic_fetch_add(a.status + 2, 1, __ATOMIC_RELAXED, __HIP_MEMORY_SCOPE_AGENT);
            } else {
                if (spins > 0 && lane == 0) {
                    __hip_atomic_fetch_add(a.status + 1, spins, __ATOMIC_RELAXED, __HIP_MEMORY_SCOPE_AGENT);
                    __hip_atomic_fetch_add(a.status + 2, 1, __ATOMIC_RELAXED, __HIP_MEMORY_SCOPE_AGENT);
                }
                if (!ok) {
                    if (lane == 0) __hip_atomic_store(a.status, NVX_STATUS_TIMEOUT, __ATOMIC_RELAXED, __HIP_MEMORY_SCOPE_AGENT);
                    break;
                }
                asm volatile("" ::: "memory");
            }
        }

        double2 *st = (double2 *)(state_wr + (size_t)stream * NVX_CASCADE_STATE_BYTES);
        const double2 *st_in = (part == 0) ? (const double2 *)(state_rd + (size_t)stream * NVX_CASCADE_STATE_BYTES) : st;
#ifdef NVX_INJECT_STALE
        if (part > 0 && !preroll && (u % NVX_INJECT_STALE) == 0) st_in = (const double2 *)(state_rd + (size_t)stream * NVX_CASCADE_STATE_BYTES);
#endif
        cw.set_mask(mask);
        unsigned long long ct = 0;
        if (!preroll) {
            NVX_WAVE_LDS_FENCE();
            const unsigned long long sealed = seal_load(st_in);
            unsigned long long fold = cw.state_in(st_in);
            if (S0 == 3 && s0.last_pair) {
                ct = __hip_atomic_load((const unsigned long long *)(st_in + NVX_STATE_CIC3) + (lane & 1), __ATOMIC_RELAXED, __HIP_MEMORY_SCOPE_AGENT);
                fold ^= seal_rotc<37>(ct);
            }
            const unsigned third_in = third0 + (unsigned)part;
            if (third_in != 0 && !seal_ok(sealed, wave_fold64(fold), stream, third_in)) {
                if (part == 0) {
                    if (lane == 0) __hip_atomic_store(a.status, NVX_STATUS_INTEGRITY, __ATOMIC_RELAXED, __HIP_MEMORY_SCOPE_AGENT);
                } else {
                    preroll = true; ct = 0;
                    if (lane == 0) __hip_atomic_fetch_add(a.status + 3, 1, __ATOMIC_RELAXED, __HIP_MEMORY_SCOPE_AGENT);
                }
            }
        }
        const int pre = preroll ? NVX_PREROLL_PASSES : 0;
        const int n_pass = pre + thirds * NVX_THIRD_PASSES;
        const u32x4 *src = unit0 - (size_t)pre * pass_stride;
        if (preroll) load_pass<RAW>(pfA, src);
        const u32x4 *nxt = src + pass_stride;
        cw.begin_unit(mask, a.y3, (size_t)(stream * 2) * a.y3_cap + a.y3_base + (size_t)part * NVX_THIRD_Y3, a.y3_cap,
                      ((part % 3) * (NVX_THIRD_PASSES * 64)) % NVX_MIX_N,
                      preroll ? NVX_PREROLL_U : 0, preroll ? NVX_PREROLL_Y2 : 0, !preroll);
        NVX_WAVE_LDS_FENCE();
        if (preroll) cw.state_zero();
        NVX_WAVE_LDS_FENCE();
        if (S0 == 3) { s0.c_prev = (int)(unsigned)ct; s0.t_prev = (int)(unsigned)(ct >> 32); }
        {
            const unsigned long long k01 = nvx_load_const_u64(a.tune_k + 2 * stream);
            int o_first = (part % 3) * (NVX_THIRD_PASSES * 64) - pre * 64;
            if (o_first < 0) o_first += NVX_PASSES_PER_FRAME * 64;
            cw.begin_table_mix((int)(unsigned)k01, (int)(unsigned)(k01 >> 32), o_first);
        }

        auto body = [&](u32x4 (&pf)[NPF], const int pass) {
            cw.tune_fetch(nvx_tune_tab);
            if (RAW) {
#pragma unroll
                for (int j = 0; j < 8; j++) xw[j * 8] = (S0 == 3) ? s0.step(pf[j]) : stage0_component(pf[j], odd);
            } else {
                const uint32_t w[4] = { pf[0].x, pf[0].y, pf[0].z, pf[0].w };
#pragma unroll
                for (int r = 0; r < 4; r++) {
                    double2 v;
                    v.x = (double)(int)(short)(w[r] & 0xffffu);
                    v.y = (double)((int)w[r] >> 16);
                    xw4[r * XS] = v;
                }
            }
            cw.tune_ready();
            if (pass + 1 < n_pass) load_pass<RAW>(pf, nxt);
            nxt += pass_stride;
            NVX_WAVE_LDS_FENCE();
            cw.compute_pass(true);
        };

        for (int pass = 0; pass < n_pass; pass++) {
            if (pass == pre) { cw.emit = true; cw.n3_done = 0; }
            body(pfA, pass);
        }

        NVX_WAVE_LDS_FENCE();
        if (late_publish) {
            int spins = 0, ok = 0;
            do {
                int d = 0;
                if (lane == 0) d = __hip_atomic_load(done, __ATOMIC_RELAXED, __HIP_MEMORY_SCOPE_AGENT);
                d = __builtin_amdgcn_readfirstlane(d);
                ok = d >= part;
                if (!ok) __builtin_amdgcn_s_sleep(32);
            } while (!ok && ++spins < NVX_SPIN_LIMIT);
            if (spins > 0 && lane == 0) __hip_atomic_fetch_add(a.status + 1, spins, __ATOMIC_RELAXED, __HIP_MEMORY_SCOPE_AGENT);
            if (!ok) {
                if (lane == 0) __hip_atomic_store(a.status, NVX_STATUS_TIMEOUT, __ATOMIC_RELAXED, __HIP_MEMORY_SCOPE_AGENT);
                break;
            }
            asm volatile("" ::: "memory");
        }
        if (!a.independent || part + thirds == 3 * a.n_frames) {
            unsigned long long fold = cw.state_out(st);
            if (S0 == 3 && s0.last_pair) {
                const unsigned long long ct_out = (unsigned long long)(unsigned)s0.c_prev | ((unsigned long long)(unsigned)s0.t_prev << 32);
                __hip_atomic_store((unsigned long long *)(st + NVX_STATE_CIC3) + (lane & 1), ct_out, __ATOMIC_RELAXED, __HIP_MEMORY_SCOPE_AGENT);
                fold ^= seal_rotc<37>(ct_out);
            }
            fold = wave_fold64(fold);
            if (lane == 0) seal_store(st, fold, stream, third0 + (unsigned)(part + thirds));
        }
        asm volatile("s_waitcnt vmcnt(0)" ::: "memory");
        if (lane == 0 && !a.independent) __hip_atomic_store(done, part + thirds, __ATOMIC_RELAXED, __HIP_MEMORY_SCOPE_AGENT);
    }
}

template <bool RAW, int NCH>
__global__ __launch_bounds__(64) void nvx_fir_cascade(nvx_cascade_args a)
{
    if (RAW) cascade_wave_main<RAW, NCH, 1, const nvx_cascade_args &>(a);
    else cascade_wave_main<RAW, NCH, 1, const nvx_cascade_args>(a);
}

__global__ __launch_bounds__(64) __attribute__((amdgpu_waves_per_eu(3, 3))) void nvx_fir_cascade_cic3_1(nvx_cascade_args a) { cascade_wave_main<true, 1, 3, const nvx_cascade_args &>(a); }
__global__ __launch_bounds__(64) void nvx_fir_cascade_cic3_2(nvx_cascade_args a) { cascade_wave_main<true, 2, 3, const nvx_cascade_args &>(a); }

template <bool RAW, int NCH, int S0>
__global__ __launch_bounds__(64) void nvx_fir_cascade_list(nvx_cascade_args a)
{
    if (RAW) cascade_wave_main<RAW, NCH, S0, const nvx_cascade_args &, true>(a);
    else cascade_wave_main<RAW, NCH, S0, const nvx_cascade_args, true>(a);
}

template <bool RAW, int NCH, int S0, bool LIST> struct CascadeKernel { static constexpr auto fn = nvx_fir_cascade_list<RAW, NCH, S0>; };
template <bool RAW, int NCH> struct CascadeKernel<RAW, NCH, 1, false> { static constexpr auto fn = nvx_fir_cascade<RAW, NCH>; };
template <> struct CascadeKernel<true, 1, 3, false> { static constexpr auto fn = nvx_fir_cascade_cic3_1; };
template <> struct CascadeKernel<true, 2, 3, false> { static constexpr auto fn = nvx_fir_cascade_cic3_2; };

#define NVX_MAX_DEVICES 64
template <bool RAW, int NCH, int S0 = 1, bool LIST = false>
static hipError_t launch_cascade_as(const nvx_cascade_args *a, nvx_forms *f, hipStream_t s)
{
    static std::mutex mu;
    static int cus_of[NVX_MAX_DEVICES], fit_of[NVX_MAX_DEVICES];
    int n_cus = 0, fit_per_cu = 0;
    {
        int dev = 0;
        hipError_t e = hipGetDevice(&dev);
        if (e != hipSuccess) return e;
        std::lock_guard<std::mutex> lk(mu);
        const bool cached = dev >= 0 && dev < NVX_MAX_DEVICES && cus_of[dev] > 0;
        if (!cached) {
            int cus = 0, per_cu = 0;
            e = hipDeviceGetAttribute(&cus, hipDeviceAttributeMultiprocessorCount, dev);
            if (e == hipSuccess) e = hipOccupancyMaxActiveBlocksPerMultiprocessor(&per_cu, CascadeKernel<RAW, NCH, S0, LIST>::fn, 64, 0);
            if (e != hipSuccess) return e;
            n_cus = cus; fit_per_cu = per_cu > 0 ? per_cu : 1;
            if (dev >= 0 && dev < NVX_MAX_DEVICES) { cus_of[dev] = n_cus; fit_of[dev] = fit_per_cu; }
        } else {
            n_cus = cus_of[dev]; fit_per_cu = fit_of[dev];
        }
    }
    int per_cu = fit_per_cu;
    if (a->max_waves_per_cu > 0 && a->max_waves_per_cu < per_cu) per_cu = a->max_waves_per_cu;
    if (a->max_waves_per_cu < 0 && per_cu + a->max_waves_per_cu >= 4) per_cu += a->max_waves_per_cu;
    const int resident = n_cus * per_cu;
    nvx_cascade_args args = *a;
    args.independent = f->independent >= 0 ? f->independent : (a->n_streams < resident && a->n_frames > 1);
    const long long whole_units = (long long)a->n_streams * a->n_frames;
    const int split_frames = whole_units > resident ? 1 : ((args.independent && 3 * whole_units <= resident) ? a->n_frames : 0);
    args.split_from = a->n_frames - split_frames;
    const long long units = (long long)a->n_streams * (args.split_from + 3LL * split_frames);
    const unsigned grid = (unsigned)(units < resident ? units : resident);
    args.dynamic_preroll = f->dynamic_preroll != 0;
    f->independent = args.independent; f->dynamic_preroll = args.dynamic_preroll;
    hipLaunchKernelGGL((CascadeKernel<RAW, NCH, S0, LIST>::fn), dim3(grid), dim3(64), 0, s, args);
    return hipGetLastError();
}

static hipError_t tune_table_ready()
{
    static std::mutex mu;
    static bool done[NVX_MAX_DEVICES];
    int dev = 0;
    hipError_t e = hipGetDevice(&dev);
    if (e != hipSuccess) return e;
    if (dev < 0 || dev >= NVX_MAX_DEVICES) return hipErrorInvalidDevice;
    std::lock_guard<std::mutex> lk(mu);
    if (done[dev]) return hipSuccess;
    double2 *tab = (double2 *)calloc(NVX_TUNE_TAB_ENTRIES, sizeof(double2));
    if (!tab) return hipErrorOutOfMemory;
    for (int j = 0; j < NVX_TUNE_TAB_N; j++) nvx_tune_entry(j, &tab[j].x, &tab[j].y);
    for (int o = 0; o < NVX_MIX_N; o++) {
        const int j = (NVX_TUNE_NOMINAL_K * o) % NVX_TUNE_TAB_N;
        tab[NVX_TUNE_TAB_N + j] = double2{ NVX_MIX_CR[o], NVX_MIX_CI[o] };
        tab[2 * NVX_TUNE_TAB_N + (NVX_TUNE_TAB_N - j) % NVX_TUNE_TAB_N] = double2{ NVX_MIX_CR[o], -NVX_MIX_CI[o] };
    }
    e = hipMemcpyToSymbol(HIP_SYMBOL(nvx_tune_tab), tab, NVX_TUNE_TAB_ENTRIES * sizeof(double2), 0, hipMemcpyHostToDevice);
    free(tab);
    if (e == hipSuccess) done[dev] = true;
    return e;
}

extern "C" hipError_t nvx_launch_cascade(const nvx_cascade_args *a, int raw, int nch, nvx_forms *f, hipStream_t s)
{
    { hipError_t e = tune_table_ready(); if (e != hipSuccess) return e; }
    hipError_t e = hipMemsetAsync(a->queue, 0, (size_t)(NVX_CASCADE_CTRL_INTS + a->n_streams) * sizeof(int), s);
    if (e != hipSuccess) return e;
    const bool cic3 = raw && a->stage0_order == 3;
    if (a->part) {
        if (cic3) return nch == 1 ? launch_cascade_as<true, 1, 3, true>(a, f, s) : launch_cascade_as<true, 2, 3, true>(a, f, s);
        if (raw) return nch == 1 ? launch_cascade_as<true, 1, 1, true>(a, f, s) : launch_cascade_as<true, 2, 1, true>(a, f, s);
        return nch == 1 ? launch_cascade_as<false, 1, 1, true>(a, f, s) : launch_cascade_as<false, 2, 1, true>(a, f, s);
    }
    if (cic3) return nch == 1 ? launch_cascade_as<true, 1, 3>(a, f, s) : launch_cascade_as<true, 2, 3>(a, f, s);
    if (raw) return nch == 1 ? launch_cascade_as<true, 1>(a, f, s) : launch_cascade_as<true, 2>(a, f, s);
    return nch == 1 ? launch_cascade_as<false, 1>(a, f, s) : launch_cascade_as<false, 2>(a, f, s);
}
```

### navtex_amd/csrc/nvx_cascade_wave.h

```cpp
#ifndef NVX_CASCADE_WAVE_H
#define NVX_CASCADE_WAVE_H

#include <hip/hip_runtime.h>
#include <stdint.h>

#include "nvx_tables.h"
#include "nvx_kernels.h"
#include "nvx_device.h"

#define XPH 8
#define XH 5
#define XS 37
#define X_ENTRIES (XPH * XS)
#define NVX_Y2_RUN 160

template <int NCH> struct Geo;
template <> struct Geo<1> { static constexpr int U_RUN = 224, Y2_PER_RUN = 32, Y2_RUN = NVX_Y2_RUN, Y3_PER_RUN = NVX_Y2_RUN / 10, U_PEND_MAX = 256, U_LEFT_MAX = 32; };
template <> struct Geo<2> { static constexpr int U_RUN = 112, Y2_PER_RUN = 16, Y2_RUN = 80, Y3_PER_RUN = 8, U_PEND_MAX = 160, U_LEFT_MAX = 48; };
template <int NCH> struct GeoSizes {
    static constexpr int U_ENTRIES = ((46 + Geo<NCH>::U_PEND_MAX) + 7) / 8 * 8;
    static constexpr int Y2_ENTRIES = ((70 + Geo<NCH>::Y2_RUN) + 7) / 8 * 8;
};
static_assert(Geo<1>::Y2_RUN % Geo<1>::Y2_PER_RUN == 0 && Geo<2>::Y2_RUN % Geo<2>::Y2_PER_RUN == 0, "NVX_Y2_RUN: a whole number of FIR2 runs (160)");
static_assert(Geo<1>::U_RUN % 32 == 0 && Geo<2>::U_RUN % 16 == 0 && 46 + Geo<1>::U_LEFT_MAX <= 128 && 46 + Geo<2>::U_LEFT_MAX <= 128, "slide covers two rows of 64");
// ... 22 lines not shown
__device__ __forceinline__ constexpr int f1_offset(int j)
{
    const int t = 7 - j, r = t & 7, fl = (t - r) / 8;
    return 2 * (r * XS + fl);
}

template <int N> struct TapIndex {
    int first[N];
    constexpr TapIndex(const double (&h)[N]) : first{}
    {
        for (int i = 0; i < N; i++) {
            int f = i;
            for (int k = 0; k < i; k++) if (h[k] == h[i]) { f = k; break; }
            first[i] = f;
        }
    }
};
static constexpr TapIndex<NVX_T1> NVX_H1_FIRST(NVX_H1);

__device__ __forceinline__ double2 state_load(const double2 *p)
{
    double2 r;
    r.x = __hip_atomic_load(&p->x, __ATOMIC_RELAXED, __HIP_MEMORY_SCOPE_AGENT);
    r.y = __hip_atomic_load(&p->y, __ATOMIC_RELAXED, __HIP_MEMORY_SCOPE_AGENT);
    return r;
}
__device__ __forceinline__ void state_store(double2 *p, double2 v)
{
    __hip_atomic_store(&p->x, v.x, __ATOMIC_RELAXED, __HIP_MEMORY_SCOPE_AGENT);
    __hip_atomic_store(&p->y, v.y, __ATOMIC_RELAXED, __HIP_MEMORY_SCOPE_AGENT);
}

template <int R> __device__ __forceinline__ unsigned long long seal_rotc(unsigned long long v)
{
    constexpr int r = R & 63;
    if constexpr (r == 0) return v;
    else return (v << r) | (v >> (64 - r));
}
template <int SLOT> __device__ __forceinline__ unsigned long long seal_pair(double2 v)
{
    return seal_rotc<14 * SLOT + 3>((unsigned long long)__double_as_longlong(v.x)) ^ seal_rotc<14 * SLOT + 10>((unsigned long long)__double_as_longlong(v.y));
}
__device__ __forceinline__ unsigned long long seal_tag(int stream, unsigned third)
{
    unsigned long long t = ((unsigned long long)(unsigned)stream << 32) | third;
    t *= 0x9E3779B97F4A7C15ull; t ^= t >> 29; t *= 0xBF58476D1CE4E5B9ull; t ^= t >> 32;
    return t;
}
template <int CTRL, int R> __device__ __forceinline__ unsigned long long seal_step(unsigned long long v)
{
    const unsigned lo = (unsigned)__builtin_amdgcn_mov_dpp((int)(unsigned)v, CTRL, 0xF, 0xF, true);
    const unsigned hi = (unsigned)__builtin_amdgcn_mov_dpp((int)(unsigned)(v >> 32), CTRL, 0xF, 0xF, true);
    return v ^ seal_rotc<R>(((unsigned long long)hi << 32) | lo);
}
__device__ __forceinline__ unsigned long long seal_row(unsigned lo, unsigned hi, int lane0)
{
    return ((unsigned long long)(unsigned)__builtin_amdgcn_readlane((int)hi, lane0) << 32) | (unsigned)__builtin_amdgcn_readlane((int)lo, lane0);
}
__device__ __forceinline__ unsigned long long wave_fold64(unsigned long long v)
{
    v = seal_step<0xB1, 1>(v);
    v = seal_step<0x4E, 2>(v);
    v = seal_step<0x141, 4>(v);
    v = seal_step<0x140, 8>(v);
    const unsigned lo = (unsigned)v, hi = (unsigned)(v >> 32);
    return seal_row(lo, hi, 0) ^ seal_rotc<16>(seal_row(lo, hi, 16)) ^ seal_rotc<32>(seal_row(lo, hi, 32)) ^ seal_rotc<48>(seal_row(lo, hi, 48));
}
__device__ __forceinline__ void seal_store(double2 *st, unsigned long long fold, int stream, unsigned third)
{
    unsigned long long *p = (unsigned long long *)(st + NVX_STATE_SEAL);
    __hip_atomic_store(p, fold ^ seal_tag(stream, third), __ATOMIC_RELAXED, __HIP_MEMORY_SCOPE_AGENT);
    __hip_atomic_store(p + 1, ((unsigned long long)(unsigned)stream << 32) | third, __ATOMIC_RELAXED, __HIP_MEMORY_SCOPE_AGENT);
}
__device__ __forceinline__ unsigned long long seal_load(const double2 *st_in)
{
    return __hip_atomic_load((const unsigned long long *)(st_in + NVX_STATE_SEAL), __ATOMIC_RELAXED, __HIP_MEMORY_SCOPE_AGENT);
}
__device__ __forceinline__ bool seal_ok(unsigned long long got, unsigned long long fold, int stream, unsigned third)
{
    const unsigned long long d = got ^ fold ^ seal_tag(stream, third);
    return __builtin_amdgcn_readfirstlane((int)((unsigned)d | (unsigned)(d >> 32))) == 0;
}

template <int NCH, bool F3IN = true>
struct CascadeWave {
    CascadeLds<NCH, F3IN> *lds;
    int lane, half, comp;
    const lds_vdouble *xrv;
    const lds_vd2 *mixrow;
    int lane_mod9;
    double h1v[NVX_T1];
    unsigned mask;
    int chain_of_slot0;
    int n_u, n_y2, n3_done, mixbase;
    nvx_d2 mix_next;
    bool emit;
    double2 *y3; size_t y3_row0, y3_cap;
    double2 *y2_lane; int n2_done;
    int toff[NCH], tk[NCH], tidx[NCH];
    nvx_d2 tc[NCH];

    __device__ __forceinline__ void init(CascadeLds<NCH, F3IN> *l, int lane_)
    {
        lds = l; lane = lane_; half = lane >> 1; comp = lane & 1;
        xrv = (const lds_vdouble *)((const double *)&lds->X[XH + half] + comp);
        lane_mod9 = (2 * half) % 9;
        if (!F3IN && lane < 4 * NVX_MIX_N) {
            const int j9 = lane % NVX_MIX_N;
            double cr = 0.0, ci = 0.0;
#pragma unroll
            for (int j = 0; j < NVX_MIX_N; j++) if (j9 == j) { cr = NVX_MIX_CR[j]; ci = NVX_MIX_CI[j]; }
            lds->mix[0][lane % (2 * NVX_MIX_N)] = double2{ cr, ci };
            lds->mix[1][lane % (2 * NVX_MIX_N)] = double2{ cr, -ci };
        }
#pragma unroll
        for (int i = 0; i < NVX_T1; i++)
            if (NVX_H1_FIRST.first[i] == i) { h1v[i] = NVX_H1[i]; asm volatile("" : "+v"(h1v[i])); }
    }

    __device__ __forceinline__ void set_mask(unsigned chain_mask)
    {
        mask = chain_mask;
        chain_of_slot0 = (NCH == 1) ? ((mask & 1u) ? 0 : 1) : 0;
    }
    __device__ __forceinline__ void begin_unit(unsigned chain_mask, double2 *y3_, size_t row0, size_t cap, int mixbase0, int n_u0, int n_y20, bool emit0)
    {
        set_mask(chain_mask);
        mixrow = (const lds_vd2 *)&lds->mix[(comp ^ (NCH == 1 ? chain_of_slot0 : 0)) ? 0 : 1][lane_mod9];
        y3 = y3_; y3_row0 = row0; y3_cap = cap;
        mixbase = mixbase0; n_u = n_u0; n_y2 = n_y20; n3_done = 0; n2_done = 0; emit = emit0;
        if (!F3IN) mix_next = mixrow[mixbase];
    }

    __device__ __forceinline__ void begin_table_mix(int k0, int k1, int o_first)
    {
        int o = o_first + lane;
        if (o >= NVX_TUNE_TAB_N) o -= NVX_TUNE_TAB_N;
#pragma unroll
        for (int c = 0; c < NCH; c++) {
            const int ch = __builtin_amdgcn_readfirstlane((NCH == 1) ? chain_of_slot0 : c);
            const int k = ch ? k1 : k0;
            const bool nominal = k == (ch ? -NVX_TUNE_NOMINAL_K : NVX_TUNE_NOMINAL_K);
            tk[c] = ((k % NVX_TUNE_TAB_N) + NVX_TUNE_TAB_N) % NVX_TUNE_TAB_N;
            toff[c] = nominal ? NVX_TUNE_TAB_N * (1 + ch) : 0;
            tidx[c] = (tk[c] * o) % NVX_TUNE_TAB_N;
        }
    }
    __device__ __forceinline__ void tune_fetch(const double2 *tab)
    {
#pragma unroll
        for (int c = 0; c < NCH; c++) {
            tc[c] = *(const nvx_d2 *)(tab + toff[c] + tidx[c]);
            tidx[c] += (64 * tk[c]) % NVX_TUNE_TAB_N;
            if (tidx[c] >= NVX_TUNE_TAB_N) tidx[c] -= NVX_TUNE_TAB_N;
        }
    }

    __device__ __forceinline__ void tune_ready()
    {
#pragma unroll
        for (int c = 0; c < NCH; c++) asm volatile("" :: "v"(tc[c].x), "v"(tc[c].y));
    }

    __device__ __forceinline__ void begin_unit_y2(double2 *y2buf, size_t pitch, int row0, int row1, size_t first)
    {
        const int ch = (NCH == 1) ? chain_of_slot0 : (lane >> 5);
        const int row = ch ? row1 : row0;
        y2_lane = row < 0 ? nullptr : y2buf + ((size_t)row * pitch + NVX_Y2_PREFIX + first);
    }

    __device__ __forceinline__ unsigned long long state_in(const double2 *st_in)
    {
        unsigned long long f = 0;
        if (lane < 36) {
            const int v = lane + 4;
            const double2 x = state_load(st_in + lane);
            f ^= seal_pair<0>(x);
            lds->X[(v & 7) * XS + (v >> 3)] = x;
        }
#pragma unroll
        for (int c = 0; c < NCH; c++) {
            const int ch = (NCH == 1) ? chain_of_slot0 : c;
            const double2 *su = st_in + 36 + ch * (46 + 70);
            if (lane < 46) { const double2 u = state_load(su + lane); f ^= (c ? seal_pair<4>(u) : seal_pair<1>(u)); lds->U[c][lane] = u; }
            if constexpr (F3IN) {
                const double2 y = state_load(su + 46 + lane);
                f ^= (c ? seal_pair<5>(y) : seal_pair<2>(y));
                lds->Y2[c][lane] = y;
                if (lane < 6) { const double2 t = state_load(su + 46 + 64 + lane); f ^= (c ? seal_pair<6>(t) : seal_pair<3>(t)); lds->Y2[c][64 + lane] = t; }
            }
        }
        return f;
    }
    __device__ __forceinline__ void state_zero()
    {
        const double2 zero = { 0.0, 0.0 };
        if (lane < XPH * XH) lds->X[(lane & 7) * XS + (lane >> 3)] = zero;
#pragma unroll
        for (int c = 0; c < NCH; c++) {
            for (int i = lane; i < 46 + NVX_PREROLL_U; i += 64) lds->U[c][i] = zero;
            if constexpr (F3IN) for (int i = lane; i < 70 + NVX_PREROLL_Y2; i += 64) lds->Y2[c][i] = zero;
        }
    }
    __device__ __forceinline__ unsigned long long state_out(double2 *st)
    {
        unsigned long long f = 0;
        if (lane < 36) {
            const int v = lane + 4;
            const double2 x = lds->X[(v & 7) * XS + (v >> 3)];
            f ^= seal_pair<0>(x);
            state_store(st + lane, x);
        }
#pragma unroll
        for (int c = 0; c < NCH; c++) {
            const int ch = (NCH == 1) ? chain_of_slot0 : c;
            double2 *su = st + 36 + ch * (46 + 70);
            if (lane < 46) { const double2 u = lds->U[c][lane]; f ^= (c ? seal_pair<4>(u) : seal_pair<1>(u)); state_store(su + lane, u); }
            if constexpr (F3IN) {
                const double2 y = lds->Y2[c][lane];
                f ^= (c ? seal_pair<5>(y) : seal_pair<2>(y));
                state_store(su + 46 + lane, y);
                if (lane < 6) { const double2 t = lds->Y2[c][64 + lane]; f ^= (c ? seal_pair<6>(t) : seal_pair<3>(t)); state_store(su + 46 + 64 + lane, t); }
            }
        }
        return f;
    }

    __device__ __forceinline__ void compute_pass(const bool table_mix = false)
    {
        nvx_d2 c0 = { 0.0, 0.0 }, c1 = { 0.0, 0.0 };
        if (!table_mix) { c0 = mix_next; c1 = mixrow[mixbase + 1]; mix_next = c1; }
        nvx_d2 tail = { 0.0, 0.0 };
        if (lane < XPH * XH) tail = *(const lds_vd2 *)&lds->X[(lane & 7) * XS + 32 + (lane >> 3)];
        double xs[NVX_T1 + 4];
        constexpr int F1N = NVX_T1 + 4, F1NG = (F1N + NVX_F1_GROUP - 1) / NVX_F1_GROUP;
#pragma unroll
        for (int j = 0; j < NVX_F1_AHEAD * NVX_F1_GROUP; j++) xs[j] = xrv[f1_offset(j)];
        double a0 = 0.0, a1 = 0.0;
#pragma unroll
        for (int g = 0; g < F1NG; g++) {
            if (g + NVX_F1_AHEAD < F1NG) {
                NVX_PIN_AFTER(a1);
#pragma unroll
                for (int j = (g + NVX_F1_AHEAD) * NVX_F1_GROUP; j < (g + NVX_F1_AHEAD + 1) * NVX_F1_GROUP && j < F1N; j++) xs[j] = xrv[f1_offset(j)];
            }
            const int lo = g * NVX_F1_GROUP, hi = (lo + NVX_F1_GROUP < F1N ? lo + NVX_F1_GROUP : F1N) - 1;
            if (hi > lo) asm volatile("" : "+v"(xs[lo]) : "v"(xs[hi]));
#pragma unroll
            for (int j = lo; j <= hi; j++) {
                if (j < NVX_T1) a1 += h1v[NVX_H1_FIRST.first[j]] * xs[j];
                if (j >= 4) a0 += h1v[NVX_H1_FIRST.first[j - 4]] * xs[j];
            }
        }
        if (table_mix) {
            const double o0 = dpp_swap_pairs_f64(a0), o1 = dpp_swap_pairs_f64(a1);
#pragma unroll
            for (int c = 0; c < NCH; c++) {
                const nvx_d2 tp = { dpp_swap_pairs_f64(tc[c].x), dpp_swap_pairs_f64(tc[c].y) };
                const nvx_d2 c0t = comp ? tp : tc[c], c1t = comp ? tc[c] : tp;
                const double A0 = a0 * c0t.x, A1 = a1 * c1t.x;
                const double B0 = o0 * c0t.y, B1 = o1 * c1t.y;
                double *uw = (double *)&lds->U[c][46 + n_u + 2 * half] + comp;
                uw[0] = comp ? A0 + B0 : A0 - B0;
                uw[2] = comp ? A1 + B1 : A1 - B1;
            }
        } else {
            const double o0 = dpp_swap_pairs_f64(a0), o1 = dpp_swap_pairs_f64(a1);
            const double A0 = a0 * c0.x, A1 = a1 * c1.x;
            const double B0 = o0 * c0.y, B1 = o1 * c1.y;
#pragma unroll
            for (int c = 0; c < NCH; c++) {
                const int ch = (NCH == 1) ? chain_of_slot0 : c;
                double *uw = (double *)&lds->U[c][46 + n_u + 2 * half] + comp;
                uw[0] = (NCH == 1 || ch == 0) ? A0 + B0 : A0 - B0;
                uw[2] = (NCH == 1 || ch == 0) ? A1 + B1 : A1 - B1;
            }
        }
        n_u += 64;
        if (!table_mix) { mixbase += 1; if (mixbase == NVX_MIX_N) mixbase = 0; }
        NVX_WAVE_LDS_FENCE();
        if (lane < XPH * XH) *(lds_vd2 *)&lds->X[(lane & 7) * XS + (lane >> 3)] = tail;
        NVX_WAVE_LDS_FENCE();

        constexpr int U_RUN = Geo<NCH>::U_RUN, Y2_PER_RUN = Geo<NCH>::Y2_PER_RUN;
        constexpr int Y2_RUN = Geo<NCH>::Y2_RUN, Y3_PER_RUN = Geo<NCH>::Y3_PER_RUN;
        const int f2c = (NCH == 2) ? (lane >> 5) : 0;
        const int f2o = (NCH == 2) ? ((lane >> 1) & 15) : half;
        constexpr int UT1 = 46 + Geo<NCH>::U_LEFT_MAX - 64;
        while (n_u >= U_RUN) {
            nvx_d2 ut0[NCH], ut1[NCH];
#pragma unroll
            for (int c = 0; c < NCH; c++) {
                ut0[c] = *(const lds_vd2 *)&lds->U[c][U_RUN + lane];
                ut1[c] = *(const lds_vd2 *)&lds->U[c][U_RUN + 64 + (lane < UT1 ? lane : UT1 - 1)];
            }
            {
                const lds_vdouble *ub = (const lds_vdouble *)((const double *)&lds->U[f2c][7 * f2o] + comp);
                double xs2[NVX_T2], acc = 0.0;
#pragma unroll
                for (int i = 0; i < NVX_F23_AHEAD; i++) xs2[i] = ub[2 * (52 - i)];
                nvx_static_for<0, NVX_T2>([&](auto ic) {
                    constexpr int i = decltype(ic)::value;
                    if constexpr (i + NVX_F23_AHEAD < NVX_T2) { NVX_PIN_AFTER(acc); xs2[i + NVX_F23_AHEAD] = ub[2 * (52 - (i + NVX_F23_AHEAD))]; }
                    acc += NVX_H2[i] * xs2[i];
                });
                if constexpr (F3IN) {
                    if (NCH == 1 || ((mask >> f2c) & 1u)) ((double *)&lds->Y2[f2c][70 + n_y2 + f2o])[comp] = acc;
                } else {
                    if (emit && y2_lane) ((double *)(y2_lane + n2_done + f2o))[comp] = acc;
                }
            }
            NVX_WAVE_LDS_FENCE();
            const int keep = 46 + n_u - U_RUN;
#pragma unroll
            for (int c = 0; c < NCH; c++) {
                if (lane < keep) *(lds_vd2 *)&lds->U[c][lane] = ut0[c];
                if (lane + 64 < keep) *(lds_vd2 *)&lds->U[c][64 + lane] = ut1[c];
            }
            NVX_WAVE_LDS_FENCE();
            n_u -= U_RUN;
            if constexpr (!F3IN) { if (emit) n2_done += Y2_PER_RUN; continue; }
            n_y2 += Y2_PER_RUN;

            if constexpr (F3IN) if (n_y2 >= Y2_RUN) {
                const int f3c = (NCH == 2) ? ((lane >> 4) & 1) : 0;
                const int f3o = half & (Y3_PER_RUN - 1);
                const bool f3live = lane < 2 * Y3_PER_RUN * NCH;
                nvx_d2 yt0[NCH], yt1[NCH];
#pragma unroll
                for (int c = 0; c < NCH; c++) {
                    yt0[c] = *(const lds_vd2 *)&lds->Y2[c][Y2_RUN + lane];
                    yt1[c] = *(const lds_vd2 *)&lds->Y2[c][Y2_RUN + 64 + (lane < 6 ? lane : 5)];
                }
                {
                    const int ch = (NCH == 1) ? chain_of_slot0 : f3c;
                    const lds_vdouble *yb = (const lds_vdouble *)((const double *)&lds->Y2[f3c][10 * f3o] + comp);
                    double xs3[NVX_T3], acc = 0.0;
#pragma unroll
                    for (int i = 0; i < NVX_F23_AHEAD; i++) xs3[i] = yb[2 * (79 - i)];
                    nvx_static_for<0, NVX_T3>([&](auto ic) {
                        constexpr int i = decltype(ic)::value;
                        if constexpr (i + NVX_F23_AHEAD < NVX_T3) { NVX_PIN_AFTER(acc); xs3[i + NVX_F23_AHEAD] = yb[2 * (79 - (i + NVX_F23_AHEAD))]; }
                        acc += NVX_H3[i] * xs3[i];
                    });
                    if (emit && f3live && (NCH == 1 || ((mask >> f3c) & 1u))) {
                        double *out = (double *)(y3 + (y3_row0 + (size_t)ch * y3_cap + n3_done + f3o));
                        out[comp] = acc;
                    }
                }
                NVX_WAVE_LDS_FENCE();
                const int keep3 = 70 + n_y2 - Y2_RUN;
#pragma unroll
                for (int c = 0; c < NCH; c++) {
                    if (lane < keep3) *(lds_vd2 *)&lds->Y2[c][lane] = yt0[c];
                    if (lane + 64 < keep3) *(lds_vd2 *)&lds->Y2[c][64 + lane] = yt1[c];
                }
                NVX_WAVE_LDS_FENCE();
                n_y2 -= Y2_RUN;
                n3_done += Y3_PER_RUN;
            }
        }
    }
// ... 4 lines not shown
```

### navtex_amd/csrc/nvx_handle.h

```cpp
#ifndef NVX_HANDLE_H
#define NVX_HANDLE_H

#include <hip/hip_runtime.h>

#include <algorithm>
#include <atomic>
#include <condition_variable>
#include <cstdarg>
#include <cstdio>
#include <cstdlib>
#include <cstring>
#include <mutex>
#include <string>
#include <thread>
#include <vector>

#include "navtex_amd.h"
#include "nvx_internal.h"
#include "nvx_kernels.h"
#include "nvx_afc_law.h"
#include "nvx_pool.h"

#define HIP_TRY(expr)                                                                      \
    do {                                                                                   \
// ... 50 lines not shown
    int n3 = 0;
    unsigned long long g0_all = 0;
    hipEvent_t copied = nullptr;
    hipEvent_t done = nullptr;
    hipEvent_t ev[10] = { nullptr, nullptr, nullptr, nullptr, nullptr, nullptr, nullptr, nullptr, nullptr, nullptr };
    bool timed = false;
    bool pending = false;
    nvx_sig_rec *d_sig = nullptr, *h_sig = nullptr;
    bool sig = false;
    float *d_soft = nullptr, *h_soft = nullptr;
    bool soft = false;
    int soft_pitch = 0;
    nvx_afc_note *d_note = nullptr, *h_note = nullptr;
    bool afc = false;
};

struct ArrivalClock {
    static const int RING = 512;
    static const int KEEP = 8192;
    std::mutex mu;
    int64_t t_ns[RING];
    uint64_t stamped = 0;
    uint64_t base = 0;
    std::vector<float> lat_ms;
    uint64_t booked = 0;
    float max_ms = 0.f, last_ms = 0.f;
    void stamp(uint64_t frame, int64_t ns)
    {
        std::lock_guard<std::mutex> lk(mu);
        t_ns[frame % RING] = ns;
        if (frame + 1 > stamped) stamped = frame + 1;
    }
    void book(uint64_t handle_frame, int64_t now_ns)
    {
        std::lock_guard<std::mutex> lk(mu);
        if (handle_frame < base) return;
        const uint64_t f = handle_frame - base;
        if (f >= stamped || stamped - f > RING) return;
        const float ms = (float)((double)(now_ns - t_ns[f % RING]) * 1e-6);
        if (lat_ms.size() < (size_t)KEEP) lat_ms.push_back(ms); else lat_ms[booked % KEEP] = ms;
        booked++; last_ms = ms; if (ms > max_ms) max_ms = ms;
    }
};
int64_t nvx_now_ns();
void nvx_clock_report(ArrivalClock &c, uint64_t *frames, double *p50_ms, double *p99_ms, double *max_ms, double *last_ms, int reset);

enum class HipRes : uint8_t { stream, event, device, pinned };

struct nvx_handle {
    nvx_config cfg{};
    int n_streams = 0, n_slots = 0, nch = 1;
    int n_in = 0;
    int per_in = 1;
    size_t bit_history = NVX_BIT_HISTORY;
    bool cascade_raw = false;
    size_t frame_in = 0;
    uint32_t *d_whist[2] = { nullptr, nullptr };
    int y3_cap = 0, bits_cap = 0;
    hipStream_t stream = nullptr;
    hipStream_t stream2 = nullptr;
    hipEvent_t casc_done[2] = { nullptr, nullptr };
    hipEvent_t demod_done[2] = { nullptr, nullptr };
    hipEvent_t launch_done = nullptr; bool launch_done_valid = false;
    hipStream_t last_launch_stream = nullptr;
    bool demod_pending[2] = { false, false };
    uint8_t *d_masks = nullptr, *d_active = nullptr;
    uint8_t *d_cstate[2] = { nullptr, nullptr };
    double2 *d_y3[2] = { nullptr, nullptr };
    double2 *d_y2[2] = { nullptr, nullptr };
    int *d_y2row = nullptr;
    std::vector<int> y2row;
    size_t y2_pitch = 0; int y2_rows = 0;
    double *d_dd[2] = { nullptr, nullptr };
    double *d_dphi = nullptr;
    double *d_corr = nullptr, *d_csum = nullptr;
    bool sig_on = false;
    nvx_sig_rec *d_sig_part = nullptr;
    int sig_stride = 0;
    int soft_mode = 0;
    int soft_cap = 0;
    unsigned short *d_soft_pos = nullptr;
    nvx_message_fn soft_fn = nullptr; void *soft_user = nullptr;
    std::vector<int> tune_k;
    int *d_tune_k = nullptr;
    int *d_afc_k[2] = { nullptr, nullptr };
    nvx_afc_par *d_afc_par = nullptr;
    int afc_tracking = 0;
    int *d_di = nullptr;
    uint32_t *d_fsm_tab = nullptr;
    unsigned short *d_words = nullptr;
    nvx_tie_stats *d_ties = nullptr;
    nvx_tie_stats *h_ties = nullptr;
    int *d_ctrl = nullptr;
    int *h_status = nullptr;
    uint64_t wait_polls = 0, wait_units = 0, wait_launches = 0;
    uint64_t stale_repaired = 0, integrity_failures = 0;
    std::vector<uint8_t> parity;
    std::vector<unsigned long long> g0s;
    bool diverged = false;
    uint64_t partial_launches = 0;
    std::vector<uint8_t> ended;
    bool poisoned = false;
    std::string poison_why;
    Result res[RESULT_SLOTS];
    std::vector<ArrivalClock *> arrival;
    int n_arrival = 0;
    uint64_t launched = 0, collected = 0;
    int last_n3 = 0;
    nvx_forms forms_req = { -1, -1, -1 }, forms_last = { -1, -1, -1 };
    bool forms_known = false;
    bool timing = false;
    float ms[5] = { 0.f, 0.f, 0.f, 0.f, 0.f };
    double ms_sum[5] = { 0.0, 0.0, 0.0, 0.0, 0.0 };
    uint64_t ms_count = 0;
    std::vector<uint8_t> masks;
    std::vector<Slot> slots;
    std::vector<struct SinkCtx *> sinks;
    HostPool pool;
    std::vector<std::pair<HipRes, void *>> made;
    std::mutex mu;
    uint32_t *h_stage[2] = { nullptr, nullptr };
    std::vector<uint8_t> cur;
    std::vector<uint64_t> set_launch[2];
    uint64_t copies_synced = 0;
    std::vector<uint8_t> active;
    size_t stage_cap = 0;
    std::vector<size_t> fill;
    uint32_t *d_in = nullptr;
    std::vector<uint8_t> writing;
    std::vector<uint8_t> pushing;
    std::vector<uint8_t> closing;
    std::vector<int64_t> last_push_ns;
    std::vector<int64_t> stall_ns;
    int writers = 0, quiesce = 0;
    std::condition_variable wr_cv;
};

struct SinkCtx { nvx_handle *h; int stream; int slot; bool soft = false; };

struct StagingQuiesce {
    nvx_handle *h; std::unique_lock<std::mutex> &lk;
    StagingQuiesce(nvx_handle *h_, std::unique_lock<std::mutex> &lk_) : h(h_), lk(lk_)
    {
        h->quiesce++;
        h->wr_cv.wait(lk, [&] { return h->writers == 0; });
    }
    ~StagingQuiesce() { h->quiesce--; h->wr_cv.notify_all(); }
};

struct StreamClose {
    nvx_handle *h; int first, last;
    StreamClose(nvx_handle *h_, std::unique_lock<std::mutex> &lk, int first_, int last_) : h(h_), first(first_), last(last_)
    {
        if (h->pushing.empty()) { first = last = 0; return; }
        for (int s = first; s < last; s++) h->closing[s]++;
        h->wr_cv.wait(lk, [&] { for (int s = first; s < last; s++) if (h->pushing[s]) return false; return true; });
    }
    ~StreamClose() { for (int s = first; s < last; s++) h->closing[s]--; if (first != last) h->wr_cv.notify_all(); }
};

int nvx_launch_locked(nvx_handle *h, const void *d_iq, size_t pitch, size_t first_sample, int n_frames, hipStream_t st,
                      const int *part = nullptr, int n_part = 0, const int *tail_n3 = nullptr);
int nvx_push_iq_partial(nvx_handle *h, int stream, const int16_t *iq, size_t n, size_t *accepted);
int nvx_collect_locked(nvx_handle *h, uint64_t upto = UINT64_MAX);
int nvx_collect_ready_locked(nvx_handle *h);
int nvx_poisoned_error(nvx_handle *h);
int nvx_launches_in_flight(nvx_handle *h);
uint64_t nvx_launch_count(nvx_handle *h);
const uint32_t *nvx_fsm_table_host();

#endif
```

### navtex_amd/csrc/nvx_kernels.h

```cpp
#ifndef NVX_KERNELS_H
#define NVX_KERNELS_H

#include <hip/hip_runtime.h>
#include <stdint.h>
#include "nvx_synth.h"

#define NVX_PASSES_PER_FRAME 315
#define NVX_Y3_PER_FRAME 288
#define NVX_THIRD_PASSES (NVX_PASSES_PER_FRAME / 3)
#define NVX_THIRD_Y3 (NVX_Y3_PER_FRAME / 3)
#define NVX_Y2_PER_FRAME 2880
#define NVX_THIRD_Y2 (NVX_Y2_PER_FRAME / 3)
#define NVX_Y2_PREFIX 80
#define NVX_PREROLL_PASSES 9
#define NVX_PREROLL_U 96
#define NVX_PREROLL_Y2 64
#define NVX_CASCADE_CTRL_INTS 8
#define NVX_STATUS_TIMEOUT 1
#define NVX_STATUS_INTEGRITY 2
#define NVX_STATUS_INTS 4
#define NVX_STATE_DATA_ENTRIES (36 + 2 * (46 + 70))
#define NVX_STATE_CIC3 NVX_STATE_DATA_ENTRIES
#define NVX_STATE_SEAL (NVX_STATE_DATA_ENTRIES + 1)
#ifndef NVX_CASCADE_STATE_ENTRIES
#define NVX_CASCADE_STATE_ENTRIES 272
#endif
#define NVX_CASCADE_STATE_BYTES   (NVX_CASCADE_STATE_ENTRIES * 16)
#define NVX_DEMOD_DOUBLES (8 + 8 + 8 + 567)
#define NVX_DEMOD_INTS    5
#define NVX_DI_PHASE       3
#define NVX_DI_PREV_OFFSET 4

typedef struct {
    int stream;
    int parity;
    unsigned long long g0;
    int n3;
    int reserved;
} nvx_part;

typedef struct {
    const uint32_t *iq;
    size_t pitch;
    size_t first_sample;
    int n_frames;
    int n_streams;
    const nvx_part *part;
    const uint8_t *chain_masks;
    uint8_t *state[2];
    double2 *y3;
    size_t y3_cap, y3_base;
    int *queue;
    int *status;
    int *done;
    int independent;
    int max_waves_per_cu;
    int stage0_order;
    int dynamic_preroll;
    int split_from;
    unsigned third0;
    const int *tune_k;
} nvx_cascade_args;
#define NVX_TUNE_NOMINAL_K 4480
#define NVX_TUNE_TAB_N 20160
#define NVX_TUNE_TAB_ENTRIES (3 * NVX_TUNE_TAB_N)
#define NVX_TUNE_K_OFFSET(n_streams) ((((size_t)(n_streams)) + 7) / 8 * 8)

typedef struct {
    double2 *y2[2];
    size_t y2_pitch;
    const int *y2_row;
    double2 *y3; size_t y3_cap, y3_base;
    int n_frames;
    int n_slots;
    const nvx_part *part; int n_part, per_part;
} nvx_fir3_args;

typedef struct {
    unsigned long long near_ties;
    unsigned long long evaluations;
    unsigned int min_margin_bits;
    unsigned int pad;
} nvx_tie_stats;

typedef struct {
    double sum_power;
    double sum_dphi_b, sum_dphi2_b;
    double sum_dphi_y, sum_dphi2_y;
    double sum_mf_hi, sum_mf_lo;
    unsigned samples, b_samples;
} nvx_sig_rec;
#define NVX_FRONT_TILE 432

typedef struct {
    const double2 *y3;
    size_t y3_cap, y3_base;
    int n3;
    int n_slots;
    const uint8_t *slot_active;
    unsigned long long g0;
    const nvx_part *part;
    int n_part;
    int per_part;
    double *dstate[2];
    int *state_i;
    const uint32_t *fsm_table;
    unsigned short *words;
    uint8_t *bits; int bits_cap; int *nbits;
    double *dphi;
    double *corr, *csum;
    nvx_tie_stats *ties;
    nvx_sig_rec *sig;
    nvx_sig_rec *sig_part;
    int sig_stride;
    int sig_parts;
    float *soft;
    int soft_cap;
    unsigned short *soft_pos;
} nvx_demod_args;

typedef struct nvx_afc_par nvx_afc_par;
typedef struct nvx_afc_note nvx_afc_note;
typedef struct {
    const nvx_sig_rec *sig;
    const nvx_afc_par *par;
    int *k_rw;
    const int *k_next;
    nvx_afc_note *note;
    int n_slots;
    const nvx_part *part;
    int n_part;
} nvx_afc_args;

typedef struct {
    const nvx_synth_desc *desc;
    const nvx_period *pool;
    uint32_t *out; size_t pitch; size_t n; uint32_t spb;
} nvx_synth_args;

typedef struct {
    const uint32_t *raw;
    size_t pitch_raw, first_sample;
    int n_wide;
    size_t n_out;
    const uint32_t *hist_in;
    uint32_t *hist_out;
    uint32_t *sub;
    size_t pitch_sub, sub_first;
    int chunks_per_block;
} nvx_channelise_args;

#define NVX_WB_SUBBANDS_K 8
#define NVX_WB_HALO 40
typedef struct {
    const uint32_t *raw;
    size_t pitch, first_sample;
    int n_wide, n_frames;
    const nvx_part *part;
    const uint8_t *chain_masks;
    uint8_t *state[2];
    uint32_t *hist[2];
    double2 *y3; size_t y3_cap, y3_base;
    int *queue, *status, *done;
    int independent;
    int thirds;
    unsigned third0;
    double2 *y2[2]; size_t y2_pitch; const int *y2_row;
} nvx_wideband_args;

typedef struct {
    int independent;
    int dynamic_preroll;
    int demod_tiles;
} nvx_forms;

#ifdef __cplusplus
extern "C" {
#endif
hipError_t nvx_launch_wideband_fused(const nvx_wideband_args *a, nvx_forms *f, hipStream_t s);
hipError_t nvx_launch_channelise(const nvx_channelise_args *a, hipStream_t s);
hipError_t nvx_launch_cascade(const nvx_cascade_args *a, int raw, int nch, nvx_forms *f, hipStream_t s);
hipError_t nvx_launch_fir3(const nvx_fir3_args *a, hipStream_t s);
int nvx_front_tile_wgs(const nvx_demod_args *a, int request);
hipError_t nvx_launch_demod_front(const nvx_demod_args *a, hipStream_t s);
hipError_t nvx_launch_demod_fsm(const nvx_demod_args *a, hipStream_t s);
hipError_t nvx_launch_synth(const nvx_synth_args *a, int n_streams, hipStream_t s);
double nvx_atan2_host(double y, double x);
hipError_t nvx_launch_afc_update(const nvx_afc_args *a, hipStream_t s);
int nvx_afc_step_host(int gain_shift, int max_step, int range_k, int min_samples, double contrast_min, int kc, int k0, int k1,
                      unsigned samples, unsigned b_samples, double sum_dphi_b, double sum_dphi_y, double sum_mf_hi, double sum_mf_lo,
                      unsigned *flags);
#ifdef __cplusplus
}
#endif
#endif
```

Baseline: 1.542 million.

## Split cascade into LDS-mixer and table-mixer kernels chosen by tuning state

Splits the cascade kernel into two compile-time variants. The default one mixes with the fixed LDS mixer row. A separate tuned variant in its own translation unit reads the frequency table and is used only when AFC is active or some slot is retuned away from nominal. The host tracks how many slots are tuned and passes a null tune pointer otherwise, so the untuned path no longer carries table fetches, per-channel index bookkeeping or the runtime table_mix branch. This adds a second set of kernels and extra build complexity.

```diff
diff --git a/include/navtex_amd_mixer.h b/include/navtex_amd_mixer.h
--- /dev/null
+++ b/include/navtex_amd_mixer.h
@@ -0,0 +1,18 @@
+#ifndef NAVTEX_AMD_MIXER_H
+#define NAVTEX_AMD_MIXER_H
+
+#include "navtex_amd.h"
+
+#ifdef __cplusplus
+extern "C" {
+#endif
+
+#define NVX_MIXER_LDS   1
+#define NVX_MIXER_TABLE 2
+
+NVX_API int nvx_debug_last_mixer(nvx_handle *h, int *mixer);
+
+#ifdef __cplusplus
+}
+#endif
+#endif
diff --git a/navtex_amd/__init__.py b/navtex_amd/__init__.py
--- a/navtex_amd/__init__.py
+++ b/navtex_amd/__init__.py
@@ -255,6 +255,11 @@
         a, b, c = C.c_int(), C.c_int(), C.c_int()
         N.check(lib.nvx_debug_last_forms(self._h, C.byref(a), C.byref(b), C.byref(c)), "nvx_debug_last_forms")
         return a.value, b.value, c.value
+
+    def last_mixer(self) -> str:
+        m = C.c_int()
+        N.check(lib.nvx_debug_last_mixer(self._h, C.byref(m)), "nvx_debug_last_mixer")
+        return {1: "lds", 2: "table"}[m.value]
 
     def _apply_forms(self, forms: Optional[Sequence[int]]) -> None:
         if forms is None:
diff --git a/navtex_amd/_native.py b/navtex_amd/_native.py
--- a/navtex_amd/_native.py
+++ b/navtex_amd/_native.py
@@ -76,6 +76,7 @@
         "nvx_sample_to_int16": (i, [C.c_double, C.POINTER(C.c_int16)]), "nvx_shim_stats": (i, [C.POINTER(C.c_uint64), C.POINTER(C.c_uint64)]),
         "nvx_debug_advance_clock": (i, [vp, i, C.c_uint64]),
         "nvx_debug_set_forms": (i, [vp, i, i, i]), "nvx_debug_last_forms": (i, [vp, C.POINTER(i), C.POINTER(i), C.POINTER(i)]),
+        "nvx_debug_last_mixer": (i, [vp, C.POINTER(i)]),
         "init_fir_filter1": (None, []), "sample_in_1": (None, [C.c_double, C.c_double]), "init_fir2_wrapper": (None, []),
         "nvx_set_trace": (i, [vp, SITOR_TRACE_FN, vp]),
         "nvx_shim_latency": (i, [C.POINTER(C.c_uint64), C.POINTER(C.c_double), C.POINTER(C.c_double), C.POINTER(C.c_double), C.POINTER(C.c_double), i]),
diff --git a/navtex_amd/build.py b/navtex_amd/build.py
--- a/navtex_amd/build.py
+++ b/navtex_amd/build.py
@@ -60,6 +60,8 @@
                "nvx_tune.cpp", "nvx_afc.cpp"]
 AFC = PKG / "afc"
 AFC_HIP_SOURCES = ["nvx_afc.hip"]
+TUNE = PKG / "tune"
+TUNE_HIP_SOURCES = ["nvx_cascade_tune.hip"]
 
 COMMON = ["-O3", "-fPIC", "-ffp-contract=off", "-fvisibility=hidden",
           f"-I{ROOT / 'include'}", f"-I{CSRC}"] + os.environ.get("NVX_EXTRA_CFLAGS", "").split()
@@ -184,6 +186,11 @@
         if force or _stale(o, [AFC / src] + headers):
             jobs.append([hipcc, f"--offload-arch={ARCH}", "-std=c++17", *COMMON, "-c", AFC / src, "-o", o])
         objs.append(o)
+    for src in TUNE_HIP_SOURCES:
+        o = OBJ / (src + ".o")
+        if force or _stale(o, [TUNE / src] + headers):
+            jobs.append([hipcc, f"--offload-arch={ARCH}", "-std=c++17", *COMMON, "-c", TUNE / src, "-o", o])
+        objs.append(o)
     for src in CXX_SOURCES:
         o = OBJ / (src + ".o")
         if force or _stale(o, [CSRC / src] + headers):
@@ -231,8 +238,16 @@
         else:
             objs.append(OBJ / (src + ".o"))
     objs += [OBJ / (src + ".o") for src in AFC_HIP_SOURCES]
+    for src in TUNE_HIP_SOURCES:
+        if "nvx_cascade.hip" in sources:
+            o = out_dir / f"{src}.{name}.o"
+            if _stale(o, [TUNE / src] + headers):
+                jobs.append([hipcc, f"--offload-arch={ARCH}", "-std=c++17", *COMMON, *flags, "-c", TUNE / src, "-o", o])
+            objs.append(o)
+        else:
+            objs.append(OBJ / (src + ".o"))
     from concurrent.futures import ThreadPoolExecutor
-    with ThreadPoolExecutor(max_workers=2) as pool:
+    with ThreadPoolExecutor(max_workers=3) as pool:
         list(pool.map(_run, jobs))
     lib = out_dir / f"libnavtex_amd_{name}.so"
     if _stale(lib, objs):
diff --git a/navtex_amd/csrc/nvx_api.cpp b/navtex_amd/csrc/nvx_api.cpp
--- a/navtex_amd/csrc/nvx_api.cpp
+++ b/navtex_amd/csrc/nvx_api.cpp
@@ -2,6 +2,7 @@
 #include <chrono>
 #include <cmath>
 #include "navtex_amd_afc.h"
+#include "navtex_amd_mixer.h"
 #include "navtex_amd_signal.h"
 #include "navtex_amd_soft.h"
 #include "navtex_amd_tune.h"
@@ -494,7 +495,8 @@
         ca.queue = h->d_ctrl; ca.status = h->d_ctrl + 1; ca.done = h->d_ctrl + NVX_CASCADE_CTRL_INTS;
         ca.stage0_order = h->cfg.stage0_order;
         ca.third0 = third0;
-        ca.tune_k = afc ? h->d_afc_k[h->launched & 1] : h->d_tune_k;
+        ca.tune_k = afc ? h->d_afc_k[h->launched & 1] : (h->tuned_slots > 0 ? h->d_tune_k : nullptr);
+        h->mixer_last = ca.tune_k ? NVX_MIXER_TABLE : NVX_MIXER_LDS;
         ca.max_waves_per_cu = -1;
         HIP_TRY(nvx_launch_cascade(&ca, h->cascade_raw, h->nch, &forms, st));
     }
@@ -948,6 +950,13 @@
     return h->slots[2 * stream + chain].soft_count;
 }
 
+static void set_tune_k(nvx_handle *h, int slot, int k)
+{
+    const int nominal = (slot & 1) ? -NVX_TUNE_NOMINAL_K : NVX_TUNE_NOMINAL_K;
+    h->tuned_slots += (k != nominal) - (h->tune_k[slot] != nominal);
+    h->tune_k[slot] = k;
+}
+
 static int afc_write_centre(nvx_handle *h, int slot, int k)
 {
     for (int i = 0; i < 2; i++) HIP_TRY(hipMemcpy(h->d_afc_k[i] + slot, &k, sizeof(int), hipMemcpyHostToDevice));
@@ -972,7 +981,7 @@
     HIP_TRY(hipMemcpyAsync(h->d_tune_k + slot, &k, sizeof(int), hipMemcpyHostToDevice, h->stream));
     if (h->afc_tracking) { int rc = afc_write_centre(h, slot, k); if (rc != NVX_OK) return rc; }
     HIP_TRY(hipStreamSynchronize(h->stream));
-    h->tune_k[slot] = k;
+    set_tune_k(h, slot, k);
     afc_restart(h, slot);
     if (applied_hz) *applied_hz = k * NVX_TUNE_STEP_HZ;
     return NVX_OK;
@@ -1083,7 +1092,7 @@
     if (keep) {
         HIP_TRY(hipMemcpy(&k, h->d_afc_k[h->launched & 1] + slot, sizeof(int), hipMemcpyDeviceToHost));
         HIP_TRY(hipMemcpy(h->d_tune_k + slot, &k, sizeof(int), hipMemcpyHostToDevice));
-        h->tune_k[slot] = k;
+        set_tune_k(h, slot, k);
     }
     a.par.track = 0;
     { int rc = afc_write_centre(h, slot, k); if (rc != NVX_OK) return rc; }
@@ -1242,6 +1251,15 @@
     return NVX_OK;
 }
 
+extern "C" int nvx_debug_last_mixer(nvx_handle *h, int *mixer)
+{
+    if (!h || !mixer) { nvx_set_error("nvx_debug_last_mixer: null handle or pointer"); return NVX_ERR_ARG; }
+    std::lock_guard<std::mutex> lk(h->mu);
+    if (!h->mixer_last) { nvx_set_error("nvx_debug_last_mixer: the handle has launched no single-wave cascade yet"); return NVX_ERR_STATE; }
+    *mixer = h->mixer_last;
+    return NVX_OK;
+}
+
 extern "C" size_t nvx_debug_y3(nvx_handle *h, int stream, int chain, double *out, size_t cap_pairs)
 {
     if (!h || !out || stream < 0 || stream >= h->n_streams || chain < 0 || chain > 1) return 0;
diff --git a/navtex_amd/csrc/nvx_cascade.hip b/navtex_amd/csrc/nvx_cascade.hip
--- a/navtex_amd/csrc/nvx_cascade.hip
+++ b/navtex_amd/csrc/nvx_cascade.hip
@@ -1,287 +1,20 @@
-#include <hip/hip_runtime.h>
-#include <stdint.h>
-#include <stdlib.h>
-#include <mutex>
+#include "nvx_cascade_main.h"
 
-#include "nvx_cascade_wave.h"
-#include "nvx_tune_table.h"
-
-__device__ double2 nvx_tune_tab[NVX_TUNE_TAB_ENTRIES];
-
-__device__ __forceinline__ int add_low_halves(unsigned a, unsigned b)
+template <bool RAW, int NCH>
+__global__ __launch_bounds__(64) void nvx_fir_cascade(nvx_cascade_core_args a)
 {
-    int r;
-    asm("v_add_u32_sdwa %0, sext(%1), sext(%2) dst_sel:DWORD dst_unused:UNUSED_PAD src0_sel:WORD_0 src1_sel:WORD_0"
-        : "=v"(r) : "v"(a), "v"(b));
-    return r;
-}
-__device__ __forceinline__ int add_high_halves(unsigned a, unsigned b)
-{
-    int r;
-    asm("v_add_u32_sdwa %0, sext(%1), sext(%2) dst_sel:DWORD dst_unused:UNUSED_PAD src0_sel:WORD_1 src1_sel:WORD_1"
-        : "=v"(r) : "v"(a), "v"(b));
-    return r;
-}
-__device__ __forceinline__ double stage0_component(u32x4 v, bool odd)
-{
-    const int sI = add_low_halves(v.x, v.y) + add_low_halves(v.z, v.w);
-    const int sQ = add_high_halves(v.x, v.y) + add_high_halves(v.z, v.w);
-    int mine = (odd ? sQ : sI) + 4;
-    const int other = odd ? sI : sQ;
-    asm("" : "+v"(mine));
-    const int tot = mine + dpp_swap_pairs(other);
-    return (double)(tot >> 3);
+    if (RAW) cascade_wave_main<RAW, NCH, 1, const nvx_cascade_core_args &, false, false>(a, nullptr);
+    else cascade_wave_main<RAW, NCH, 1, const nvx_cascade_core_args, false, false>(a, nullptr);
 }
 
-struct Stage0Cic3 {
-    unsigned sel_mine, sel_other;
-    unsigned wa0, wa1, wb0, wb1, wc0, wc1;
-    int c_prev, t_prev;
-    bool last_pair;
-
-    __device__ __forceinline__ void init(int lane)
-    {
-        const bool odd = lane & 1;
-        sel_mine = odd ? 0x07060302u : 0x05040100u;
-        sel_other = odd ? 0x05040100u : 0x07060302u;
-        wa0 = odd ? (10u | 6u << 16) : (36u | 28u << 16);  wa1 = odd ? (3u | 1u << 16) : (21u | 15u << 16);
-        wb0 = odd ? (48u | 48u << 16) : (28u | 36u << 16); wb1 = odd ? (46u | 42u << 16) : (42u | 46u << 16);
-        wc0 = odd ? (6u | 10u << 16) : 0u;                 wc1 = odd ? (15u | 21u << 16) : (1u | 3u << 16);
-        last_pair = lane >= 62;
-        c_prev = 0; t_prev = 0;
-    }
-    __device__ __forceinline__ static int rot1(int v) { return __builtin_amdgcn_mov_dpp(v, 0x13C, 0xF, 0xF, false); }
-    __device__ __forceinline__ static void dot2_first(nvx_short2 a, unsigned wb, unsigned wc, int &b, int &c)
-    {
-        asm("v_dot2_i32_i16 %0, %2, %3, 0\n\t"
-            "v_dot2_i32_i16 %1, %2, %4, 0\n\t"
-            "s_nop 2"
-            : "=&v"(b), "=v"(c) : "v"(a), "v"(wb), "v"(wc));
-    }
-    __device__ __forceinline__ double step(u32x4 v)
-    {
-        const nvx_short2 m01 = as_short2(__builtin_amdgcn_perm(v.y, v.x, sel_mine)), m23 = as_short2(__builtin_amdgcn_perm(v.w, v.z, sel_mine));
-        const nvx_short2 o01 = as_short2(__builtin_amdgcn_perm(v.y, v.x, sel_other)), o23 = as_short2(__builtin_amdgcn_perm(v.w, v.z, sel_other));
-        int oa = __builtin_amdgcn_sdot2(o01, as_short2(wa0), 256, false); oa = __builtin_amdgcn_sdot2(o23, as_short2(wa1), oa, false);
-        int ob, oc;
-        dot2_first(o01, wb0, wc0, ob, oc);
-        ob = __builtin_amdgcn_sdot2(o23, as_short2(wb1), ob, false); oc = __builtin_amdgcn_sdot2(o23, as_short2(wc1), oc, false);
-        int A = dpp_swap_pairs(oa); A = __builtin_amdgcn_sdot2(m01, as_short2(wa0), A, false); A = __builtin_amdgcn_sdot2(m23, as_short2(wa1), A, false);
-        int B = dpp_swap_pairs(ob); B = __builtin_amdgcn_sdot2(m01, as_short2(wb0), B, false); B = __builtin_amdgcn_sdot2(m23, as_short2(wb1), B, false);
-        int C = dpp_swap_pairs(oc); C = __builtin_amdgcn_sdot2(m01, as_short2(wc0), C, false); C = __builtin_amdgcn_sdot2(m23, as_short2(wc1), C, false);
-        const int t = B + rot1(rot1(last_pair ? c_prev : C));
-        const int y = A + rot1(rot1(last_pair ? t_prev : t));
-        c_prev = C; t_prev = t;
-        return (double)(y >> 9);
-    }
-};
-
-template <bool RAW>
-__device__ __forceinline__ void load_pass(u32x4 (&pf)[RAW ? 8 : 1], const u32x4 *src)
-{
-    if (RAW) {
-#pragma unroll
-        for (int j = 0; j < 8; j++) pf[j] = __builtin_nontemporal_load(src + 64 * j);
-    } else {
-        pf[0] = __builtin_nontemporal_load(src);
-    }
-}
-
-#define NVX_SPIN_LIMIT (1 << 22)
-
-template <bool RAW, int NCH, int S0, typename ARGS, bool LIST = false>
-__device__ __forceinline__ void cascade_wave_main(ARGS a)
-{
-    __shared__ CascadeLds<NCH> lds;
-    const int lane = threadIdx.x;
-    CascadeWave<NCH> cw;
-    cw.init(&lds, lane);
-
-    const size_t pass_words = RAW ? 2048 : 256;
-    const size_t pass_stride = pass_words / 4;
-    constexpr int NPF = RAW ? 8 : 1;
-    const int half = lane >> 1, comp = lane & 1;
-    const bool odd = lane & 1;
-    double *xw = (double *)&lds.X[(half & 7) * XS + XH + (lane >> 4)] + comp;
-    double2 *xw4 = &lds.X[(lane & 1) * 4 * XS + XH + half];
-    static_assert(S0 == 1 || (S0 == 3 && RAW), "the third-order stage 0 belongs to the raw-rate kernels");
-    Stage0Cic3 s0;
-    if (S0 == 3) s0.init(lane);
-    const int n_full = a.n_streams * a.split_from;
-    const int n_units = n_full + 3 * a.n_streams * (a.n_frames - a.split_from);
-
-    for (;;) {
-        int u = 0;
-        if (lane == 0) u = __hip_atomic_fetch_add(a.queue, 1, __ATOMIC_RELAXED, __HIP_MEMORY_SCOPE_AGENT);
-        u = __builtin_amdgcn_readfirstlane(u);
-        if (u >= n_units) break;
-        int tpart, thirds, entry;
-        if (u < n_full) { const int frame = u / a.n_streams; entry = u - frame * a.n_streams; tpart = 3 * frame; thirds = 3; }
-        else { const int v = u - n_full, q = v / a.n_streams; entry = v - q * a.n_streams; tpart = 3 * a.split_from + q; thirds = 1; }
-        const int part = tpart;
-        int stream = entry;
-        const uint8_t *state_rd = a.state[0];
-        uint8_t *state_wr = a.state[1];
-        unsigned third0 = a.third0;
-        if (LIST) {
-            const unsigned long long e = nvx_load_const_u64(a.part + entry);
-            stream = (int)(unsigned)e;
-            if (e >> 32) { state_rd = a.state[1]; state_wr = a.state[0]; }
-            third0 = (unsigned)(nvx_load_const_u64(&a.part[entry].g0) / NVX_THIRD_Y3);
-        }
-        int *const done = a.done + entry;
-        const unsigned mask = a.chain_masks[stream];
-
-        bool preroll = a.independent && part > 0;
-        bool late_publish = false;
-        const u32x4 *unit0 = (const u32x4 *)(a.iq + ((size_t)stream * a.pitch + a.first_sample)) + (size_t)part * NVX_THIRD_PASSES * pass_stride + lane;
-        u32x4 pfA[NPF];
-        if (!preroll) load_pass<RAW>(pfA, unit0);
-
-        if (part > 0 && !a.independent) {
-            int spins = 0, ok = 0;
-            do {
-                int d = 0;
-                if (lane == 0) d = __hip_atomic_load(done, __ATOMIC_RELAXED, __HIP_MEMORY_SCOPE_AGENT);
-                d = __builtin_amdgcn_readfirstlane(d);
-                ok = d >= part;
-                if (!ok && a.dynamic_preroll) break;
-                if (!ok) __builtin_amdgcn_s_sleep(32);
-            } while (!ok && ++spins < NVX_SPIN_LIMIT);
-            if (!ok && a.dynamic_preroll) {
-                preroll = true; late_publish = true;
-                if (lane == 0) __hip_atomic_fetch_add(a.status + 2, 1, __ATOMIC_RELAXED, __HIP_MEMORY_SCOPE_AGENT);
-            } else {
-                if (spins > 0 && lane == 0) {
-                    __hip_atomic_fetch_add(a.status + 1, spins, __ATOMIC_RELAXED, __HIP_MEMORY_SCOPE_AGENT);
-                    __hip_atomic_fetch_add(a.status + 2, 1, __ATOMIC_RELAXED, __HIP_MEMORY_SCOPE_AGENT);
-                }
-                if (!ok) {
-                    if (lane == 0) __hip_atomic_store(a.status, NVX_STATUS_TIMEOUT, __ATOMIC_RELAXED, __HIP_MEMORY_SCOPE_AGENT);
-                    break;
-                }
-                asm volatile("" ::: "memory");
-            }
-        }
-
-        double2 *st = (double2 *)(state_wr + (size_t)stream * NVX_CASCADE_STATE_BYTES);
-        const double2 *st_in = (part == 0) ? (const double2 *)(state_rd + (size_t)stream * NVX_CASCADE_STATE_BYTES) : st;
-#ifdef NVX_INJECT_STALE
-        if (part > 0 && !preroll && (u % NVX_INJECT_STALE) == 0) st_in = (const double2 *)(state_rd + (size_t)stream * NVX_CASCADE_STATE_BYTES);
-#endif
-        cw.set_mask(mask);
-        unsigned long long ct = 0;
-        if (!preroll) {
-            NVX_WAVE_LDS_FENCE();
-            const unsigned long long sealed = seal_load(st_in);
-            unsigned long long fold = cw.state_in(st_in);
-            if (S0 == 3 && s0.last_pair) {
-                ct = __hip_atomic_load((const unsigned long long *)(st_in + NVX_STATE_CIC3) + (lane & 1), __ATOMIC_RELAXED, __HIP_MEMORY_SCOPE_AGENT);
-                fold ^= seal_rotc<37>(ct);
-            }
-            const unsigned third_in = third0 + (unsigned)part;
-            if (third_in != 0 && !seal_ok(sealed, wave_fold64(fold), stream, third_in)) {
-                if (part == 0) {
-                    if (lane == 0) __hip_atomic_store(a.status, NVX_STATUS_INTEGRITY, __ATOMIC_RELAXED, __HIP_MEMORY_SCOPE_AGENT);
-                } else {
-                    preroll = true; ct = 0;
-                    if (lane == 0) __hip_atomic_fetch_add(a.status + 3, 1, __ATOMIC_RELAXED, __HIP_MEMORY_SCOPE_AGENT);
-                }
-            }
-        }
-        const int pre = preroll ? NVX_PREROLL_PASSES : 0;
-        const int n_pass = pre + thirds * NVX_THIRD_PASSES;
-        const u32x4 *src = unit0 - (size_t)pre * pass_stride;
-        if (preroll) load_pass<RAW>(pfA, src);
-        const u32x4 *nxt = src + pass_stride;
-        cw.begin_unit(mask, a.y3, (size_t)(stream * 2) * a.y3_cap + a.y3_base + (size_t)part * NVX_THIRD_Y3, a.y3_cap,
-                      ((part % 3) * (NVX_THIRD_PASSES * 64)) % NVX_MIX_N,
-                      preroll ? NVX_PREROLL_U : 0, preroll ? NVX_PREROLL_Y2 : 0, !preroll);
-        NVX_WAVE_LDS_FENCE();
-        if (preroll) cw.state_zero();
-        NVX_WAVE_LDS_FENCE();
-        if (S0 == 3) { s0.c_prev = (int)(unsigned)ct; s0.t_prev = (int)(unsigned)(ct >> 32); }
-        {
-            const unsigned long long k01 = nvx_load_const_u64(a.tune_k + 2 * stream);
-            int o_first = (part % 3) * (NVX_THIRD_PASSES * 64) - pre * 64;
-            if (o_first < 0) o_first += NVX_PASSES_PER_FRAME * 64;
-            cw.begin_table_mix((int)(unsigned)k01, (int)(unsigned)(k01 >> 32), o_first);
-        }
-
-        auto body = [&](u32x4 (&pf)[NPF], const int pass) {
-            cw.tune_fetch(nvx_tune_tab);
-            if (RAW) {
-#pragma unroll
-                for (int j = 0; j < 8; j++) xw[j * 8] = (S0 == 3) ? s0.step(pf[j]) : stage0_component(pf[j], odd);
-            } else {
-                const uint32_t w[4] = { pf[0].x, pf[0].y, pf[0].z, pf[0].w };
-#pragma unroll
-                for (int r = 0; r < 4; r++) {
-                    double2 v;
-                    v.x = (double)(int)(short)(w[r] & 0xffffu);
-                    v.y = (double)((int)w[r] >> 16);
-                    xw4[r * XS] = v;
-                }
-            }
-            cw.tune_ready();
-            if (pass + 1 < n_pass) load_pass<RAW>(pf, nxt);
-            nxt += pass_stride;
-            NVX_WAVE_LDS_FENCE();
-            cw.compute_pass(true);
-        };
-
-        for (int pass = 0; pass < n_pass; pass++) {
-            if (pass == pre) { cw.emit = true; cw.n3_done = 0; }
-            body(pfA, pass);
-        }
-
-        NVX_WAVE_LDS_FENCE();
-        if (late_publish) {
-            int spins = 0, ok = 0;
-            do {
-                int d = 0;
-                if (lane == 0) d = __hip_atomic_load(done, __ATOMIC_RELAXED, __HIP_MEMORY_SCOPE_AGENT);
-                d = __builtin_amdgcn_readfirstlane(d);
-                ok = d >= part;
-                if (!ok) __builtin_amdgcn_s_sleep(32);
-            } while (!ok && ++spins < NVX_SPIN_LIMIT);
-            if (spins > 0 && lane == 0) __hip_atomic_fetch_add(a.status + 1, spins, __ATOMIC_RELAXED, __HIP_MEMORY_SCOPE_AGENT);
-            if (!ok) {
-                if (lane == 0) __hip_atomic_store(a.status, NVX_STATUS_TIMEOUT, __ATOMIC_RELAXED, __HIP_MEMORY_SCOPE_AGENT);
-                break;
-            }
-            asm volatile("" ::: "memory");
-        }
-        if (!a.independent || part + thirds == 3 * a.n_frames) {
-            unsigned long long fold = cw.state_out(st);
-            if (S0 == 3 && s0.last_pair) {
-                const unsigned long long ct_out = (unsigned long long)(unsigned)s0.c_prev | ((unsigned long long)(unsigned)s0.t_prev << 32);
-                __hip_atomic_store((unsigned long long *)(st + NVX_STATE_CIC3) + (lane & 1), ct_out, __ATOMIC_RELAXED, __HIP_MEMORY_SCOPE_AGENT);
-                fold ^= seal_rotc<37>(ct_out);
-            }
-            fold = wave_fold64(fold);
-            if (lane == 0) seal_store(st, fold, stream, third0 + (unsigned)(part + thirds));
-        }
-        asm volatile("s_waitcnt vmcnt(0)" ::: "memory");
-        if (lane == 0 && !a.independent) __hip_atomic_store(done, part + thirds, __ATOMIC_RELAXED, __HIP_MEMORY_SCOPE_AGENT);
-    }
-}
-
-template <bool RAW, int NCH>
-__global__ __launch_bounds__(64) void nvx_fir_cascade(nvx_cascade_args a)
-{
-    if (RAW) cascade_wave_main<RAW, NCH, 1, const nvx_cascade_args &>(a);
-    else cascade_wave_main<RAW, NCH, 1, const nvx_cascade_args>(a);
-}
-
-__global__ __launch_bounds__(64) __attribute__((amdgpu_waves_per_eu(3, 3))) void nvx_fir_cascade_cic3_1(nvx_cascade_args a) { cascade_wave_main<true, 1, 3, const nvx_cascade_args &>(a); }
-__global__ __launch_bounds__(64) void nvx_fir_cascade_cic3_2(nvx_cascade_args a) { cascade_wave_main<true, 2, 3, const nvx_cascade_args &>(a); }
+__global__ __launch_bounds__(64) __attribute__((amdgpu_waves_per_eu(3, 3))) void nvx_fir_cascade_cic3_1(nvx_cascade_core_args a) { cascade_wave_main<true, 1, 3, const nvx_cascade_core_args &, false, false>(a, nullptr); }
+__global__ __launch_bounds__(64) void nvx_fir_cascade_cic3_2(nvx_cascade_core_args a) { cascade_wave_main<true, 2, 3, const nvx_cascade_core_args &, false, false>(a, nullptr); }
 
 template <bool RAW, int NCH, int S0>
-__global__ __launch_bounds__(64) void nvx_fir_cascade_list(nvx_cascade_args a)
+__global__ __launch_bounds__(64) void nvx_fir_cascade_list(nvx_cascade_core_args a)
 {
-    if (RAW) cascade_wave_main<RAW, NCH, S0, const nvx_cascade_args &, true>(a);
-    else cascade_wave_main<RAW, NCH, S0, const nvx_cascade_args, true>(a);
+    if (RAW) cascade_wave_main<RAW, NCH, S0, const nvx_cascade_core_args &, true, false>(a, nullptr);
+    else cascade_wave_main<RAW, NCH, S0, const nvx_cascade_core_args, true, false>(a, nullptr);
 }
 
 template <bool RAW, int NCH, int S0, bool LIST> struct CascadeKernel { static constexpr auto fn = nvx_fir_cascade_list<RAW, NCH, S0>; };
@@ -289,83 +22,8 @@
 template <> struct CascadeKernel<true, 1, 3, false> { static constexpr auto fn = nvx_fir_cascade_cic3_1; };
 template <> struct CascadeKernel<true, 2, 3, false> { static constexpr auto fn = nvx_fir_cascade_cic3_2; };
 
-#define NVX_MAX_DEVICES 64
-template <bool RAW, int NCH, int S0 = 1, bool LIST = false>
-static hipError_t launch_cascade_as(const nvx_cascade_args *a, nvx_forms *f, hipStream_t s)
-{
-    static std::mutex mu;
-    static int cus_of[NVX_MAX_DEVICES], fit_of[NVX_MAX_DEVICES];
-    int n_cus = 0, fit_per_cu = 0;
-    {
-        int dev = 0;
-        hipError_t e = hipGetDevice(&dev);
-        if (e != hipSuccess) return e;
-        std::lock_guard<std::mutex> lk(mu);
-        const bool cached = dev >= 0 && dev < NVX_MAX_DEVICES && cus_of[dev] > 0;
-        if (!cached) {
-            int cus = 0, per_cu = 0;
-            e = hipDeviceGetAttribute(&cus, hipDeviceAttributeMultiprocessorCount, dev);
-            if (e == hipSuccess) e = hipOccupancyMaxActiveBlocksPerMultiprocessor(&per_cu, CascadeKernel<RAW, NCH, S0, LIST>::fn, 64, 0);
-            if (e != hipSuccess) return e;
-            n_cus = cus; fit_per_cu = per_cu > 0 ? per_cu : 1;
-            if (dev >= 0 && dev < NVX_MAX_DEVICES) { cus_of[dev] = n_cus; fit_of[dev] = fit_per_cu; }
-        } else {
-            n_cus = cus_of[dev]; fit_per_cu = fit_of[dev];
-        }
-    }
-    int per_cu = fit_per_cu;
-    if (a->max_waves_per_cu > 0 && a->max_waves_per_cu < per_cu) per_cu = a->max_waves_per_cu;
-    if (a->max_waves_per_cu < 0 && per_cu + a->max_waves_per_cu >= 4) per_cu += a->max_waves_per_cu;
-    const int resident = n_cus * per_cu;
-    nvx_cascade_args args = *a;
-    args.independent = f->independent >= 0 ? f->independent : (a->n_streams < resident && a->n_frames > 1);
-    const long long whole_units = (long long)a->n_streams * a->n_frames;
-    const int split_frames = whole_units > resident ? 1 : ((args.independent && 3 * whole_units <= resident) ? a->n_frames : 0);
-    args.split_from = a->n_frames - split_frames;
-    const long long units = (long long)a->n_streams * (args.split_from + 3LL * split_frames);
-    const unsigned grid = (unsigned)(units < resident ? units : resident);
-    args.dynamic_preroll = f->dynamic_preroll != 0;
-    f->independent = args.independent; f->dynamic_preroll = args.dynamic_preroll;
-    hipLaunchKernelGGL((CascadeKernel<RAW, NCH, S0, LIST>::fn), dim3(grid), dim3(64), 0, s, args);
-    return hipGetLastError();
-}
-
-static hipError_t tune_table_ready()
-{
-    static std::mutex mu;
-    static bool done[NVX_MAX_DEVICES];
-    int dev = 0;
-    hipError_t e = hipGetDevice(&dev);
-    if (e != hipSuccess) return e;
-    if (dev < 0 || dev >= NVX_MAX_DEVICES) return hipErrorInvalidDevice;
-    std::lock_guard<std::mutex> lk(mu);
-    if (done[dev]) return hipSuccess;
-    double2 *tab = (double2 *)calloc(NVX_TUNE_TAB_ENTRIES, sizeof(double2));
-    if (!tab) return hipErrorOutOfMemory;
-    for (int j = 0; j < NVX_TUNE_TAB_N; j++) nvx_tune_entry(j, &tab[j].x, &tab[j].y);
-    for (int o = 0; o < NVX_MIX_N; o++) {
-        const int j = (NVX_TUNE_NOMINAL_K * o) % NVX_TUNE_TAB_N;
-        tab[NVX_TUNE_TAB_N + j] = double2{ NVX_MIX_CR[o], NVX_MIX_CI[o] };
-        tab[2 * NVX_TUNE_TAB_N + (NVX_TUNE_TAB_N - j) % NVX_TUNE_TAB_N] = double2{ NVX_MIX_CR[o], -NVX_MIX_CI[o] };
-    }
-    e = hipMemcpyToSymbol(HIP_SYMBOL(nvx_tune_tab), tab, NVX_TUNE_TAB_ENTRIES * sizeof(double2), 0, hipMemcpyHostToDevice);
-    free(tab);
-    if (e == hipSuccess) done[dev] = true;
-    return e;
-}
-
 extern "C" hipError_t nvx_launch_cascade(const nvx_cascade_args *a, int raw, int nch, nvx_forms *f, hipStream_t s)
 {
-    { hipError_t e = tune_table_ready(); if (e != hipSuccess) return e; }
-    hipError_t e = hipMemsetAsync(a->queue, 0, (size_t)(NVX_CASCADE_CTRL_INTS + a->n_streams) * sizeof(int), s);
-    if (e != hipSuccess) return e;
-    const bool cic3 = raw && a->stage0_order == 3;
-    if (a->part) {
-        if (cic3) return nch == 1 ? launch_cascade_as<true, 1, 3, true>(a, f, s) : launch_cascade_as<true, 2, 3, true>(a, f, s);
-        if (raw) return nch == 1 ? launch_cascade_as<true, 1, 1, true>(a, f, s) : launch_cascade_as<true, 2, 1, true>(a, f, s);
-        return nch == 1 ? launch_cascade_as<false, 1, 1, true>(a, f, s) : launch_cascade_as<false, 2, 1, true>(a, f, s);
-    }
-    if (cic3) return nch == 1 ? launch_cascade_as<true, 1, 3>(a, f, s) : launch_cascade_as<true, 2, 3>(a, f, s);
-    if (raw) return nch == 1 ? launch_cascade_as<true, 1>(a, f, s) : launch_cascade_as<true, 2>(a, f, s);
-    return nch == 1 ? launch_cascade_as<false, 1>(a, f, s) : launch_cascade_as<false, 2>(a, f, s);
+    if (a->tune_k) return nvx_launch_cascade_tuned(a, raw, nch, f, s);
+    return launch_cascade_family<CascadeKernel>(a, raw, nch, f, s);
 }
diff --git a/navtex_amd/csrc/nvx_cascade_main.h b/navtex_amd/csrc/nvx_cascade_main.h
--- /dev/null
+++ b/navtex_amd/csrc/nvx_cascade_main.h
@@ -0,0 +1,327 @@
+#ifndef NVX_CASCADE_MAIN_H
+#define NVX_CASCADE_MAIN_H
+
+#include <hip/hip_runtime.h>
+#include <stdint.h>
+#include <mutex>
+
+#include "nvx_cascade_wave.h"
+
+__device__ __forceinline__ int add_low_halves(unsigned a, unsigned b)
+{
+    int r;
+    asm("v_add_u32_sdwa %0, sext(%1), sext(%2) dst_sel:DWORD dst_unused:UNUSED_PAD src0_sel:WORD_0 src1_sel:WORD_0"
+        : "=v"(r) : "v"(a), "v"(b));
+    return r;
+}
+__device__ __forceinline__ int add_high_halves(unsigned a, unsigned b)
+{
+    int r;
+    asm("v_add_u32_sdwa %0, sext(%1), sext(%2) dst_sel:DWORD dst_unused:UNUSED_PAD src0_sel:WORD_1 src1_sel:WORD_1"
+        : "=v"(r) : "v"(a), "v"(b));
+    return r;
+}
+__device__ __forceinline__ double stage0_component(u32x4 v, bool odd)
+{
+    const int sI = add_low_halves(v.x, v.y) + add_low_halves(v.z, v.w);
+    const int sQ = add_high_halves(v.x, v.y) + add_high_halves(v.z, v.w);
+    int mine = (odd ? sQ : sI) + 4;
+    const int other = odd ? sI : sQ;
+    asm("" : "+v"(mine));
+    const int tot = mine + dpp_swap_pairs(other);
+    return (double)(tot >> 3);
+}
+
+struct Stage0Cic3 {
+    unsigned sel_mine, sel_other;
+    unsigned wa0, wa1, wb0, wb1, wc0, wc1;
+    int c_prev, t_prev;
+    bool last_pair;
+
+    __device__ __forceinline__ void init(int lane)
+    {
+        const bool odd = lane & 1;
+        sel_mine = odd ? 0x07060302u : 0x05040100u;
+        sel_other = odd ? 0x05040100u : 0x07060302u;
+        wa0 = odd ? (10u | 6u << 16) : (36u | 28u << 16);  wa1 = odd ? (3u | 1u << 16) : (21u | 15u << 16);
+        wb0 = odd ? (48u | 48u << 16) : (28u | 36u << 16); wb1 = odd ? (46u | 42u << 16) : (42u | 46u << 16);
+        wc0 = odd ? (6u | 10u << 16) : 0u;                 wc1 = odd ? (15u | 21u << 16) : (1u | 3u << 16);
+        last_pair = lane >= 62;
+        c_prev = 0; t_prev = 0;
+    }
+    __device__ __forceinline__ static int rot1(int v) { return __builtin_amdgcn_mov_dpp(v, 0x13C, 0xF, 0xF, false); }
+    __device__ __forceinline__ static void dot2_first(nvx_short2 a, unsigned wb, unsigned wc, int &b, int &c)
+    {
+        asm("v_dot2_i32_i16 %0, %2, %3, 0\n\t"
+            "v_dot2_i32_i16 %1, %2, %4, 0\n\t"
+            "s_nop 2"
+            : "=&v"(b), "=v"(c) : "v"(a), "v"(wb), "v"(wc));
+    }
+    __device__ __forceinline__ double step(u32x4 v)
+    {
+        const nvx_short2 m01 = as_short2(__builtin_amdgcn_perm(v.y, v.x, sel_mine)), m23 = as_short2(__builtin_amdgcn_perm(v.w, v.z, sel_mine));
+        const nvx_short2 o01 = as_short2(__builtin_amdgcn_perm(v.y, v.x, sel_other)), o23 = as_short2(__builtin_amdgcn_perm(v.w, v.z, sel_other));
+        int oa = __builtin_amdgcn_sdot2(o01, as_short2(wa0), 256, false); oa = __builtin_amdgcn_sdot2(o23, as_short2(wa1), oa, false);
+        int ob, oc;
+        dot2_first(o01, wb0, wc0, ob, oc);
+        ob = __builtin_amdgcn_sdot2(o23, as_short2(wb1), ob, false); oc = __builtin_amdgcn_sdot2(o23, as_short2(wc1), oc, false);
+        int A = dpp_swap_pairs(oa); A = __builtin_amdgcn_sdot2(m01, as_short2(wa0), A, false); A = __builtin_amdgcn_sdot2(m23, as_short2(wa1), A, false);
+        int B = dpp_swap_pairs(ob); B = __builtin_amdgcn_sdot2(m01, as_short2(wb0), B, false); B = __builtin_amdgcn_sdot2(m23, as_short2(wb1), B, false);
+        int C = dpp_swap_pairs(oc); C = __builtin_amdgcn_sdot2(m01, as_short2(wc0), C, false); C = __builtin_amdgcn_sdot2(m23, as_short2(wc1), C, false);
+        const int t = B + rot1(rot1(last_pair ? c_prev : C));
+        const int y = A + rot1(rot1(last_pair ? t_prev : t));
+        c_prev = C; t_prev = t;
+        return (double)(y >> 9);
+    }
+};
+
+template <bool RAW>
+__device__ __forceinline__ void load_pass(u32x4 (&pf)[RAW ? 8 : 1], const u32x4 *src)
+{
+    if (RAW) {
+#pragma unroll
+        for (int j = 0; j < 8; j++) pf[j] = __builtin_nontemporal_load(src + 64 * j);
+    } else {
+        pf[0] = __builtin_nontemporal_load(src);
+    }
+}
+
+#define NVX_SPIN_LIMIT (1 << 22)
+
+template <bool RAW, int NCH, int S0, typename ARGS, bool LIST, bool TABLE_MIX>
+__device__ __forceinline__ void cascade_wave_main(ARGS a, const double2 *tune_tab)
+{
+    __shared__ CascadeLds<NCH> lds;
+    const int lane = threadIdx.x;
+    CascadeWave<NCH, true, TABLE_MIX> cw;
+    cw.init(&lds, lane);
+
+    const size_t pass_words = RAW ? 2048 : 256;
+    const size_t pass_stride = pass_words / 4;
+    constexpr int NPF = RAW ? 8 : 1;
+    const int half = lane >> 1, comp = lane & 1;
+    const bool odd = lane & 1;
+    double *xw = (double *)&lds.X[(half & 7) * XS + XH + (lane >> 4)] + comp;
+    double2 *xw4 = &lds.X[(lane & 1) * 4 * XS + XH + half];
+    static_assert(S0 == 1 || (S0 == 3 && RAW), "the third-order stage 0 belongs to the raw-rate kernels");
+    Stage0Cic3 s0;
+    if (S0 == 3) s0.init(lane);
+    const int n_full = a.n_streams * a.split_from;
+    const int n_units = n_full + 3 * a.n_streams * (a.n_frames - a.split_from);
+
+    for (;;) {
+        int u = 0;
+        if (lane == 0) u = __hip_atomic_fetch_add(a.queue, 1, __ATOMIC_RELAXED, __HIP_MEMORY_SCOPE_AGENT);
+        u = __builtin_amdgcn_readfirstlane(u);
+        if (u >= n_units) break;
+        int tpart, thirds, entry;
+        if (u < n_full) { const int frame = u / a.n_streams; entry = u - frame * a.n_streams; tpart = 3 * frame; thirds = 3; }
+        else { const int v = u - n_full, q = v / a.n_streams; entry = v - q * a.n_streams; tpart = 3 * a.split_from + q; thirds = 1; }
+        const int part = tpart;
+        int stream = entry;
+        const uint8_t *state_rd = a.state[0];
+        uint8_t *state_wr = a.state[1];
+        unsigned third0 = a.third0;
+        if (LIST) {
+            const unsigned long long e = nvx_load_const_u64(a.part + entry);
+            stream = (int)(unsigned)e;
+            if (e >> 32) { state_rd = a.state[1]; state_wr = a.state[0]; }
+            third0 = (unsigned)(nvx_load_const_u64(&a.part[entry].g0) / NVX_THIRD_Y3);
+        }
+        int *const done = a.done + entry;
+        const unsigned mask = a.chain_masks[stream];
+
+        bool preroll = a.independent && part > 0;
+        bool late_publish = false;
+        const u32x4 *unit0 = (const u32x4 *)(a.iq + ((size_t)stream * a.pitch + a.first_sample)) + (size_t)part * NVX_THIRD_PASSES * pass_stride + lane;
+        u32x4 pfA[NPF];
+        if (!preroll) load_pass<RAW>(pfA, unit0);
+
+        if (part > 0 && !a.independent) {
+            int spins = 0, ok = 0;
+            do {
+                int d = 0;
+                if (lane == 0) d = __hip_atomic_load(done, __ATOMIC_RELAXED, __HIP_MEMORY_SCOPE_AGENT);
+                d = __builtin_amdgcn_readfirstlane(d);
+                ok = d >= part;
+                if (!ok && a.dynamic_preroll) break;
+                if (!ok) __builtin_amdgcn_s_sleep(32);
+            } while (!ok && ++spins < NVX_SPIN_LIMIT);
+            if (!ok && a.dynamic_preroll) {
+                preroll = true; late_publish = true;
+                if (lane == 0) __hip_atomic_fetch_add(a.status + 2, 1, __ATOMIC_RELAXED, __HIP_MEMORY_SCOPE_AGENT);
+            } else {
+                if (spins > 0 && lane == 0) {
+                    __hip_atomic_fetch_add(a.status + 1, spins, __ATOMIC_RELAXED, __HIP_MEMORY_SCOPE_AGENT);
+                    __hip_atomic_fetch_add(a.status + 2, 1, __ATOMIC_RELAXED, __HIP_MEMORY_SCOPE_AGENT);
+                }
+                if (!ok) {
+                    if (lane == 0) __hip_atomic_store(a.status, NVX_STATUS_TIMEOUT, __ATOMIC_RELAXED, __HIP_MEMORY_SCOPE_AGENT);
+                    break;
+                }
+                asm volatile("" ::: "memory");
+            }
+        }
+
+        double2 *st = (double2 *)(state_wr + (size_t)stream * NVX_CASCADE_STATE_BYTES);
+        const double2 *st_in = (part == 0) ? (const double2 *)(state_rd + (size_t)stream * NVX_CASCADE_STATE_BYTES) : st;
+#ifdef NVX_INJECT_STALE
+        if (part > 0 && !preroll && (u % NVX_INJECT_STALE) == 0) st_in = (const double2 *)(state_rd + (size_t)stream * NVX_CASCADE_STATE_BYTES);
+#endif
+        cw.set_mask(mask);
+        unsigned long long ct = 0;
+        if (!preroll) {
+            NVX_WAVE_LDS_FENCE();
+            const unsigned long long sealed = seal_load(st_in);
+            unsigned long long fold = cw.state_in(st_in);
+            if (S0 == 3 && s0.last_pair) {
+                ct = __hip_atomic_load((const unsigned long long *)(st_in + NVX_STATE_CIC3) + (lane & 1), __ATOMIC_RELAXED, __HIP_MEMORY_SCOPE_AGENT);
+                fold ^= seal_rotc<37>(ct);
+            }
+            const unsigned third_in = third0 + (unsigned)part;
+            if (third_in != 0 && !seal_ok(sealed, wave_fold64(fold), stream, third_in)) {
+                if (part == 0) {
+                    if (lane == 0) __hip_atomic_store(a.status, NVX_STATUS_INTEGRITY, __ATOMIC_RELAXED, __HIP_MEMORY_SCOPE_AGENT);
+                } else {
+                    preroll = true; ct = 0;
+                    if (lane == 0) __hip_atomic_fetch_add(a.status + 3, 1, __ATOMIC_RELAXED, __HIP_MEMORY_SCOPE_AGENT);
+                }
+            }
+        }
+        const int pre = preroll ? NVX_PREROLL_PASSES : 0;
+        const int n_pass = pre + thirds * NVX_THIRD_PASSES;
+        const u32x4 *src = unit0 - (size_t)pre * pass_stride;
+        if (preroll) load_pass<RAW>(pfA, src);
+        const u32x4 *nxt = src + pass_stride;
+        cw.begin_unit(mask, a.y3, (size_t)(stream * 2) * a.y3_cap + a.y3_base + (size_t)part * NVX_THIRD_Y3, a.y3_cap,
+                      ((part % 3) * (NVX_THIRD_PASSES * 64)) % NVX_MIX_N,
+                      preroll ? NVX_PREROLL_U : 0, preroll ? NVX_PREROLL_Y2 : 0, !preroll);
+        NVX_WAVE_LDS_FENCE();
+        if (preroll) cw.state_zero();
+        NVX_WAVE_LDS_FENCE();
+        if (S0 == 3) { s0.c_prev = (int)(unsigned)ct; s0.t_prev = (int)(unsigned)(ct >> 32); }
+        if constexpr (TABLE_MIX) {
+            const unsigned long long k01 = nvx_load_const_u64(a.tune_k + 2 * stream);
+            int o_first = (part % 3) * (NVX_THIRD_PASSES * 64) - pre * 64;
+            if (o_first < 0) o_first += NVX_PASSES_PER_FRAME * 64;
+            cw.begin_table_mix((int)(unsigned)k01, (int)(unsigned)(k01 >> 32), o_first);
+        }
+
+        auto body = [&](u32x4 (&pf)[NPF], const int pass) {
+            if constexpr (TABLE_MIX) cw.tune_fetch(tune_tab);
+            if (RAW) {
+#pragma unroll
+                for (int j = 0; j < 8; j++) xw[j * 8] = (S0 == 3) ? s0.step(pf[j]) : stage0_component(pf[j], odd);
+            } else {
+                const uint32_t w[4] = { pf[0].x, pf[0].y, pf[0].z, pf[0].w };
+#pragma unroll
+                for (int r = 0; r < 4; r++) {
+                    double2 v;
+                    v.x = (double)(int)(short)(w[r] & 0xffffu);
+                    v.y = (double)((int)w[r] >> 16);
+                    xw4[r * XS] = v;
+                }
+            }
+            if constexpr (TABLE_MIX) cw.tune_ready();
+            if (pass + 1 < n_pass) load_pass<RAW>(pf, nxt);
+            nxt += pass_stride;
+            NVX_WAVE_LDS_FENCE();
+            cw.compute_pass();
+        };
+
+        for (int pass = 0; pass < n_pass; pass++) {
+            if (pass == pre) { cw.emit = true; cw.n3_done = 0; }
+            body(pfA, pass);
+        }
+
+        NVX_WAVE_LDS_FENCE();
+        if (late_publish) {
+            int spins = 0, ok = 0;
+            do {
+                int d = 0;
+                if (lane == 0) d = __hip_atomic_load(done, __ATOMIC_RELAXED, __HIP_MEMORY_SCOPE_AGENT);
+                d = __builtin_amdgcn_readfirstlane(d);
+                ok = d >= part;
+                if (!ok) __builtin_amdgcn_s_sleep(32);
+            } while (!ok && ++spins < NVX_SPIN_LIMIT);
+            if (spins > 0 && lane == 0) __hip_atomic_fetch_add(a.status + 1, spins, __ATOMIC_RELAXED, __HIP_MEMORY_SCOPE_AGENT);
+            if (!ok) {
+                if (lane == 0) __hip_atomic_store(a.status, NVX_STATUS_TIMEOUT, __ATOMIC_RELAXED, __HIP_MEMORY_SCOPE_AGENT);
+                break;
+            }
+            asm volatile("" ::: "memory");
+        }
+        if (!a.independent || part + thirds == 3 * a.n_frames) {
+            unsigned long long fold = cw.state_out(st);
+            if (S0 == 3 && s0.last_pair) {
+                const unsigned long long ct_out = (unsigned long long)(unsigned)s0.c_prev | ((unsigned long long)(unsigned)s0.t_prev << 32);
+                __hip_atomic_store((unsigned long long *)(st + NVX_STATE_CIC3) + (lane & 1), ct_out, __ATOMIC_RELAXED, __HIP_MEMORY_SCOPE_AGENT);
+                fold ^= seal_rotc<37>(ct_out);
+            }
+            fold = wave_fold64(fold);
+            if (lane == 0) seal_store(st, fold, stream, third0 + (unsigned)(part + thirds));
+        }
+        asm volatile("s_waitcnt vmcnt(0)" ::: "memory");
+        if (lane == 0 && !a.independent) __hip_atomic_store(done, part + thirds, __ATOMIC_RELAXED, __HIP_MEMORY_SCOPE_AGENT);
+    }
+}
+
+#define NVX_MAX_DEVICES 64
+template <typename KARGS> KARGS cascade_kernel_args(void (*)(KARGS));
+template <auto FN>
+static hipError_t launch_cascade_fn(const nvx_cascade_args *a, nvx_forms *f, hipStream_t s)
+{
+    static std::mutex mu;
+    static int cus_of[NVX_MAX_DEVICES], fit_of[NVX_MAX_DEVICES];
+    int n_cus = 0, fit_per_cu = 0;
+    {
+        int dev = 0;
+        hipError_t e = hipGetDevice(&dev);
+        if (e != hipSuccess) return e;
+        std::lock_guard<std::mutex> lk(mu);
+        const bool cached = dev >= 0 && dev < NVX_MAX_DEVICES && cus_of[dev] > 0;
+        if (!cached) {
+            int cus = 0, per_cu = 0;
+            e = hipDeviceGetAttribute(&cus, hipDeviceAttributeMultiprocessorCount, dev);
+            if (e == hipSuccess) e = hipOccupancyMaxActiveBlocksPerMultiprocessor(&per_cu, FN, 64, 0);
+            if (e != hipSuccess) return e;
+            n_cus = cus; fit_per_cu = per_cu > 0 ? per_cu : 1;
+            if (dev >= 0 && dev < NVX_MAX_DEVICES) { cus_of[dev] = n_cus; fit_of[dev] = fit_per_cu; }
+        } else {
+            n_cus = cus_of[dev]; fit_per_cu = fit_of[dev];
+        }
+    }
+    int per_cu = fit_per_cu;
+    if (a->max_waves_per_cu > 0 && a->max_waves_per_cu < per_cu) per_cu = a->max_waves_per_cu;
+    if (a->max_waves_per_cu < 0 && per_cu + a->max_waves_per_cu >= 4) per_cu += a->max_waves_per_cu;
+    const int resident = n_cus * per_cu;
+    decltype(cascade_kernel_args(FN)) args = *a;
+    args.independent = f->independent >= 0 ? f->independent : (a->n_streams < resident && a->n_frames > 1);
+    const long long whole_units = (long long)a->n_streams * a->n_frames;
+    const int split_frames = whole_units > resident ? 1 : ((args.independent && 3 * whole_units <= resident) ? a->n_frames : 0);
+    args.split_from = a->n_frames - split_frames;
+    const long long units = (long long)a->n_streams * (args.split_from + 3LL * split_frames);
+    const unsigned grid = (unsigned)(units < resident ? units : resident);
+    args.dynamic_preroll = f->dynamic_preroll != 0;
+    f->independent = args.independent; f->dynamic_preroll = args.dynamic_preroll;
+    hipLaunchKernelGGL(FN, dim3(grid), dim3(64), 0, s, args);
+    return hipGetLastError();
+}
+
+template <template <bool, int, int, bool> class K>
+static hipError_t launch_cascade_family(const nvx_cascade_args *a, int raw, int nch, nvx_forms *f, hipStream_t s)
+{
+    hipError_t e = hipMemsetAsync(a->queue, 0, (size_t)(NVX_CASCADE_CTRL_INTS + a->n_streams) * sizeof(int), s);
+    if (e != hipSuccess) return e;
+    const bool cic3 = raw && a->stage0_order == 3;
+    if (a->part) {
+        if (cic3) return nch == 1 ? launch_cascade_fn<K<true, 1, 3, true>::fn>(a, f, s) : launch_cascade_fn<K<true, 2, 3, true>::fn>(a, f, s);
+        if (raw) return nch == 1 ? launch_cascade_fn<K<true, 1, 1, true>::fn>(a, f, s) : launch_cascade_fn<K<true, 2, 1, true>::fn>(a, f, s);
+        return nch == 1 ? launch_cascade_fn<K<false, 1, 1, true>::fn>(a, f, s) : launch_cascade_fn<K<false, 2, 1, true>::fn>(a, f, s);
+    }
+    if (cic3) return nch == 1 ? launch_cascade_fn<K<true, 1, 3, false>::fn>(a, f, s) : launch_cascade_fn<K<true, 2, 3, false>::fn>(a, f, s);
+    if (raw) return nch == 1 ? launch_cascade_fn<K<true, 1, 1, false>::fn>(a, f, s) : launch_cascade_fn<K<true, 2, 1, false>::fn>(a, f, s);
+    return nch == 1 ? launch_cascade_fn<K<false, 1, 1, false>::fn>(a, f, s) : launch_cascade_fn<K<false, 2, 1, false>::fn>(a, f, s);
+}
+
+#endif
diff --git a/navtex_amd/csrc/nvx_cascade_wave.h b/navtex_amd/csrc/nvx_cascade_wave.h
--- a/navtex_amd/csrc/nvx_cascade_wave.h
+++ b/navtex_amd/csrc/nvx_cascade_wave.h
@@ -128,8 +128,14 @@
     return __builtin_amdgcn_readfirstlane((int)((unsigned)d | (unsigned)(d >> 32))) == 0;
 }
 
-template <int NCH, bool F3IN = true>
-struct CascadeWave {
+template <int NCH, bool TABLE_MIX> struct CascadeTableMix {};
+template <int NCH> struct CascadeTableMix<NCH, true> {
+    int toff[NCH], tk[NCH], tidx[NCH];
+    nvx_d2 tc[NCH];
+};
+
+template <int NCH, bool F3IN = true, bool TABLE_MIX = false>
+struct CascadeWave : CascadeTableMix<NCH, TABLE_MIX> {
     CascadeLds<NCH, F3IN> *lds;
     int lane, half, comp;
     const lds_vdouble *xrv;
@@ -143,15 +149,13 @@
     bool emit;
     double2 *y3; size_t y3_row0, y3_cap;
     double2 *y2_lane; int n2_done;
-    int toff[NCH], tk[NCH], tidx[NCH];
-    nvx_d2 tc[NCH];
 
     __device__ __forceinline__ void init(CascadeLds<NCH, F3IN> *l, int lane_)
     {
         lds = l; lane = lane_; half = lane >> 1; comp = lane & 1;
         xrv = (const lds_vdouble *)((const double *)&lds->X[XH + half] + comp);
         lane_mod9 = (2 * half) % 9;
-        if (!F3IN && lane < 4 * NVX_MIX_N) {
+        if (!TABLE_MIX && lane < 4 * NVX_MIX_N) {
             const int j9 = lane % NVX_MIX_N;
             double cr = 0.0, ci = 0.0;
 #pragma unroll
@@ -175,7 +179,7 @@
         mixrow = (const lds_vd2 *)&lds->mix[(comp ^ (NCH == 1 ? chain_of_slot0 : 0)) ? 0 : 1][lane_mod9];
         y3 = y3_; y3_row0 = row0; y3_cap = cap;
         mixbase = mixbase0; n_u = n_u0; n_y2 = n_y20; n3_done = 0; n2_done = 0; emit = emit0;
-        if (!F3IN) mix_next = mixrow[mixbase];
+        if (!TABLE_MIX) mix_next = mixrow[mixbase];
     }
 
     __device__ __forceinline__ void begin_table_mix(int k0, int k1, int o_first)
@@ -187,25 +191,25 @@
             const int ch = __builtin_amdgcn_readfirstlane((NCH == 1) ? chain_of_slot0 : c);
             const int k = ch ? k1 : k0;
             const bool nominal = k == (ch ? -NVX_TUNE_NOMINAL_K : NVX_TUNE_NOMINAL_K);
-            tk[c] = ((k % NVX_TUNE_TAB_N) + NVX_TUNE_TAB_N) % NVX_TUNE_TAB_N;
-            toff[c] = nominal ? NVX_TUNE_TAB_N * (1 + ch) : 0;
-            tidx[c] = (tk[c] * o) % NVX_TUNE_TAB_N;
+            this->tk[c] = ((k % NVX_TUNE_TAB_N) + NVX_TUNE_TAB_N) % NVX_TUNE_TAB_N;
+            this->toff[c] = nominal ? NVX_TUNE_TAB_N * (1 + ch) : 0;
+            this->tidx[c] = (this->tk[c] * o) % NVX_TUNE_TAB_N;
         }
     }
     __device__ __forceinline__ void tune_fetch(const double2 *tab)
     {
 #pragma unroll
         for (int c = 0; c < NCH; c++) {
-            tc[c] = *(const nvx_d2 *)(tab + toff[c] + tidx[c]);
-            tidx[c] += (64 * tk[c]) % NVX_TUNE_TAB_N;
-            if (tidx[c] >= NVX_TUNE_TAB_N) tidx[c] -= NVX_TUNE_TAB_N;
+            this->tc[c] = *(const nvx_d2 *)(tab + this->toff[c] + this->tidx[c]);
+            this->tidx[c] += (64 * this->tk[c]) % NVX_TUNE_TAB_N;
+            if (this->tidx[c] >= NVX_TUNE_TAB_N) this->tidx[c] -= NVX_TUNE_TAB_N;
         }
     }
 
     __device__ __forceinline__ void tune_ready()
     {
 #pragma unroll
-        for (int c = 0; c < NCH; c++) asm volatile("" :: "v"(tc[c].x), "v"(tc[c].y));
+        for (int c = 0; c < NCH; c++) asm volatile("" :: "v"(this->tc[c].x), "v"(this->tc[c].y));
     }
 
     __device__ __forceinline__ void begin_unit_y2(double2 *y2buf, size_t pitch, int row0, int row1, size_t first)
@@ -272,10 +276,10 @@
         return f;
     }
 
-    __device__ __forceinline__ void compute_pass(const bool table_mix = false)
+    __device__ __forceinline__ void compute_pass()
     {
         nvx_d2 c0 = { 0.0, 0.0 }, c1 = { 0.0, 0.0 };
-        if (!table_mix) { c0 = mix_next; c1 = mixrow[mixbase + 1]; mix_next = c1; }
+        if constexpr (!TABLE_MIX) { c0 = mix_next; c1 = mixrow[mixbase + 1]; mix_next = c1; }
         nvx_d2 tail = { 0.0, 0.0 };
         if (lane < XPH * XH) tail = *(const lds_vd2 *)&lds->X[(lane & 7) * XS + 32 + (lane >> 3)];
         double xs[NVX_T1 + 4];
@@ -298,12 +302,12 @@
                 if (j >= 4) a0 += h1v[NVX_H1_FIRST.first[j - 4]] * xs[j];
             }
         }
-        if (table_mix) {
+        if constexpr (TABLE_MIX) {
             const double o0 = dpp_swap_pairs_f64(a0), o1 = dpp_swap_pairs_f64(a1);
 #pragma unroll
             for (int c = 0; c < NCH; c++) {
-                const nvx_d2 tp = { dpp_swap_pairs_f64(tc[c].x), dpp_swap_pairs_f64(tc[c].y) };
-                const nvx_d2 c0t = comp ? tp : tc[c], c1t = comp ? tc[c] : tp;
+                const nvx_d2 tp = { dpp_swap_pairs_f64(this->tc[c].x), dpp_swap_pairs_f64(this->tc[c].y) };
+                const nvx_d2 c0t = comp ? tp : this->tc[c], c1t = comp ? this->tc[c] : tp;
                 const double A0 = a0 * c0t.x, A1 = a1 * c1t.x;
                 const double B0 = o0 * c0t.y, B1 = o1 * c1t.y;
                 double *uw = (double *)&lds->U[c][46 + n_u + 2 * half] + comp;
@@ -323,7 +327,7 @@
             }
         }
         n_u += 64;
-        if (!table_mix) { mixbase += 1; if (mixbase == NVX_MIX_N) mixbase = 0; }
+        if constexpr (!TABLE_MIX) { mixbase += 1; if (mixbase == NVX_MIX_N) mixbase = 0; }
         NVX_WAVE_LDS_FENCE();
         if (lane < XPH * XH) *(lds_vd2 *)&lds->X[(lane & 7) * XS + (lane >> 3)] = tail;
         NVX_WAVE_LDS_FENCE();
diff --git a/navtex_amd/csrc/nvx_handle.h b/navtex_amd/csrc/nvx_handle.h
--- a/navtex_amd/csrc/nvx_handle.h
+++ b/navtex_amd/csrc/nvx_handle.h
@@ -156,6 +156,7 @@
     unsigned short *d_soft_pos = nullptr;
     nvx_message_fn soft_fn = nullptr; void *soft_user = nullptr;
     std::vector<int> tune_k;
+    int tuned_slots = 0;
     int *d_tune_k = nullptr;
     int *d_afc_k[2] = { nullptr, nullptr };
     nvx_afc_par *d_afc_par = nullptr;
@@ -183,6 +184,7 @@
     int last_n3 = 0;
     nvx_forms forms_req = { -1, -1, -1 }, forms_last = { -1, -1, -1 };
     bool forms_known = false;
+    int mixer_last = 0;
     bool timing = false;
     float ms[5] = { 0.f, 0.f, 0.f, 0.f, 0.f };
     double ms_sum[5] = { 0.0, 0.0, 0.0, 0.0, 0.0 };
diff --git a/navtex_amd/csrc/nvx_kernels.h b/navtex_amd/csrc/nvx_kernels.h
--- a/navtex_amd/csrc/nvx_kernels.h
+++ b/navtex_amd/csrc/nvx_kernels.h
@@ -39,7 +39,7 @@
     int reserved;
 } nvx_part;
 
-typedef struct {
+struct nvx_cascade_core_args {
     const uint32_t *iq;
     size_t pitch;
     size_t first_sample;
@@ -59,8 +59,10 @@
     int dynamic_preroll;
     int split_from;
     unsigned third0;
+};
+struct nvx_cascade_args : nvx_cascade_core_args {
     const int *tune_k;
-} nvx_cascade_args;
+};
 #define NVX_TUNE_NOMINAL_K 4480
 #define NVX_TUNE_TAB_N 20160
 #define NVX_TUNE_TAB_ENTRIES (3 * NVX_TUNE_TAB_N)
@@ -180,6 +182,7 @@
 hipError_t nvx_launch_wideband_fused(const nvx_wideband_args *a, nvx_forms *f, hipStream_t s);
 hipError_t nvx_launch_channelise(const nvx_channelise_args *a, hipStream_t s);
 hipError_t nvx_launch_cascade(const nvx_cascade_args *a, int raw, int nch, nvx_forms *f, hipStream_t s);
+hipError_t nvx_launch_cascade_tuned(const nvx_cascade_args *a, int raw, int nch, nvx_forms *f, hipStream_t s);
 hipError_t nvx_launch_fir3(const nvx_fir3_args *a, hipStream_t s);
 int nvx_front_tile_wgs(const nvx_demod_args *a, int request);
 hipError_t nvx_launch_demod_front(const nvx_demod_args *a, hipStream_t s);
diff --git a/navtex_amd/tune/nvx_cascade_tune.hip b/navtex_amd/tune/nvx_cascade_tune.hip
--- /dev/null
+++ b/navtex_amd/tune/nvx_cascade_tune.hip
@@ -0,0 +1,62 @@
+#include <hip/hip_runtime.h>
+#include <stdint.h>
+#include <stdlib.h>
+#include <mutex>
+
+#include "nvx_cascade_main.h"
+#include "nvx_tune_table.h"
+
+__device__ double2 nvx_tune_tab[NVX_TUNE_TAB_ENTRIES];
+
+template <bool RAW, int NCH>
+__global__ __launch_bounds__(64) void nvx_tuned_cascade(nvx_cascade_args a)
+{
+    if (RAW) cascade_wave_main<RAW, NCH, 1, const nvx_cascade_args &, false, true>(a, nvx_tune_tab);
+    else cascade_wave_main<RAW, NCH, 1, const nvx_cascade_args, false, true>(a, nvx_tune_tab);
+}
+
+__global__ __launch_bounds__(64) __attribute__((amdgpu_waves_per_eu(3, 3))) void nvx_tuned_cascade_cic3_1(nvx_cascade_args a) { cascade_wave_main<true, 1, 3, const nvx_cascade_args &, false, true>(a, nvx_tune_tab); }
+__global__ __launch_bounds__(64) void nvx_tuned_cascade_cic3_2(nvx_cascade_args a) { cascade_wave_main<true, 2, 3, const nvx_cascade_args &, false, true>(a, nvx_tune_tab); }
+
+template <bool RAW, int NCH, int S0>
+__global__ __launch_bounds__(64) void nvx_tuned_cascade_list(nvx_cascade_args a)
+{
+    if (RAW) cascade_wave_main<RAW, NCH, S0, const nvx_cascade_args &, true, true>(a, nvx_tune_tab);
+    else cascade_wave_main<RAW, NCH, S0, const nvx_cascade_args, true, true>(a, nvx_tune_tab);
+}
+
+template <bool RAW, int NCH, int S0, bool LIST> struct TunedKernel { static constexpr auto fn = nvx_tuned_cascade_list<RAW, NCH, S0>; };
+template <bool RAW, int NCH> struct TunedKernel<RAW, NCH, 1, false> { static constexpr auto fn = nvx_tuned_cascade<RAW, NCH>; };
+template <> struct TunedKernel<true, 1, 3, false> { static constexpr auto fn = nvx_tuned_cascade_cic3_1; };
+template <> struct TunedKernel<true, 2, 3, false> { static constexpr auto fn = nvx_tuned_cascade_cic3_2; };
+
+static hipError_t tune_table_ready()
+{
+    static std::mutex mu;
+    static bool done[NVX_MAX_DEVICES];
+    int dev = 0;
+    hipError_t e = hipGetDevice(&dev);
+    if (e != hipSuccess) return e;
+    if (dev < 0 || dev >= NVX_MAX_DEVICES) return hipErrorInvalidDevice;
+    std::lock_guard<std::mutex> lk(mu);
+    if (done[dev]) return hipSuccess;
+    double2 *tab = (double2 *)calloc(NVX_TUNE_TAB_ENTRIES, sizeof(double2));
+    if (!tab) return hipErrorOutOfMemory;
+    for (int j = 0; j < NVX_TUNE_TAB_N; j++) nvx_tune_entry(j, &tab[j].x, &tab[j].y);
+    for (int o = 0; o < NVX_MIX_N; o++) {
+        const int j = (NVX_TUNE_NOMINAL_K * o) % NVX_TUNE_TAB_N;
+        tab[NVX_TUNE_TAB_N + j] = double2{ NVX_MIX_CR[o], NVX_MIX_CI[o] };
+        tab[2 * NVX_TUNE_TAB_N + (NVX_TUNE_TAB_N - j) % NVX_TUNE_TAB_N] = double2{ NVX_MIX_CR[o], -NVX_MIX_CI[o] };
+    }
+    e = hipMemcpyToSymbol(HIP_SYMBOL(nvx_tune_tab), tab, NVX_TUNE_TAB_ENTRIES * sizeof(double2), 0, hipMemcpyHostToDevice);
+    free(tab);
+    if (e == hipSuccess) done[dev] = true;
+    return e;
+}
+
+extern "C" hipError_t nvx_launch_cascade_tuned(const nvx_cascade_args *a, int raw, int nch, nvx_forms *f, hipStream_t s)
+{
+    if (!a->tune_k) return hipErrorInvalidValue;
+    { hipError_t e = tune_table_ready(); if (e != hipSuccess) return e; }
+    return launch_cascade_family<TunedKernel>(a, raw, nch, f, s);
+}
```

Measured after the change: 1.541 million, median of 2. About the same (-0.0%).
